# yhao-wang/DenseRetrievalToolkits

Hardware: AMD Instinct MI355X
Metric: queries/sec@top-1000, 10Mx768 corpus (BASELINE: passages encoded/sec + queries/sec@top-1000, 10Mx768 corpus, 1/2/4/8 GPU) (higher is better)
Workload: dtype bf16

## Files before the change

denseretrievaltoolkits_amd/_native.py:

```python
from __future__ import annotations

import ctypes
import os
import threading

import torch

from .build_native import LIB_PATH

DRT_OK = 0
DRT_EINVAL = -1
ROW_STATS_LEN = 34

_lock = threading.Lock()
_lib = None

c_i32 = ctypes.c_int32
c_i64 = ctypes.c_int64
c_sz = ctypes.c_size_t
c_vp = ctypes.c_void_p
c_f32 = ctypes.c_float
c_u64 = ctypes.c_uint64

_SIGNATURES = [
    ("drt_version", ctypes.c_char_p, []),
    ("drt_ip_topk_workspace", c_sz, [c_i64, c_i64, c_i32, c_i32]),
    ("drt_ip_topk_bf16", c_i32, [c_vp, c_i64, c_vp, c_i64, c_i32, c_i32, c_i64, c_vp, c_vp, c_vp, c_vp, c_sz, c_vp]),
    ("drt_ip_topk_resolve_workspace", c_sz, [c_i64, c_i64, c_i32]),
    ("drt_ip_topk_resolve", c_i32, [c_vp, c_i64, c_vp, c_i64, c_i32, c_i32, c_i64, c_vp, c_vp, c_vp, c_vp, c_sz,
                                    c_vp, c_vp]),
    ("drt_topk_merge", c_i32, [c_vp, c_vp, c_i64, c_i32, c_i32, c_i32, c_vp, c_vp, c_vp]),
    ("drt_ip_topk_sample_rank", c_i32, [c_i32]),
    ("drt_ip_topk_dist_workspace", c_sz, [c_i64, c_i64, c_i64, c_i32, c_i32]),
    ("drt_ip_topk_dist_sample", c_i32, [c_vp, c_i64, c_vp, c_i64, c_i64, c_i32, c_i32, c_vp, c_vp, c_sz, c_vp]),
    ("drt_ip_topk_dist_tau", c_i32, [c_vp, c_i64, c_i32, c_i32, c_vp, c_vp]),
    ("drt_ip_topk_dist_filter", c_i32, [c_vp, c_i64, c_vp, c_i64, c_i64, c_i32, c_i32, c_i64, c_vp, c_vp, c_vp,
                                        c_sz, c_vp]),
    ("drt_ip_topk_dist_filter_chunks", c_i32, [c_vp, c_i64, c_vp, c_i64, c_i64, c_i32, c_i32, c_i64, c_vp, c_vp,
                                               c_vp, c_i32, c_vp, c_sz, c_vp]),
    ("drt_ip_topk_tighten_rank", c_i32, [c_i64, c_i32, c_i32]),
    ("drt_ip_topk_filter_passes_workspace", c_sz, [c_i64, c_i64, c_i64, c_i32, c_i32]),
    ("drt_ip_topk_filter_passes", c_i32, [c_vp, c_i64, c_vp, c_i64, c_i64, c_i32, c_i32, c_i64, c_vp, c_vp,
                                          c_i32, c_i32, c_vp, c_vp, c_vp, c_sz, c_vp]),
    ("drt_ip_topk_dist_filter_lists", c_i32, [c_vp, c_i64, c_vp, c_i64, c_i64, c_i32, c_i32, c_i64, c_vp, c_i32,
                                              c_vp, c_vp, c_vp, c_sz, c_vp]),
    ("drt_ip_topk_dist_filter_lists_at", c_i32, [c_vp, c_i64, c_vp, c_i64, c_i64, c_i32, c_i32, c_i64, c_vp,
                                                 c_i32, c_i64, c_vp, c_vp, c_vp, c_sz, c_vp]),
    ("drt_topk_merge_packed", c_i32, [c_vp, c_i64, c_i32, c_i32, c_i64, c_vp, c_vp, c_vp, c_vp]),
    ("drt_topk_merge_packed_cert", c_i32, [c_vp, c_i64, c_i32, c_i32, c_i32, c_i64, c_vp, c_vp, c_vp, c_vp]),
    ("drt_topk_merge_packed_capped", c_i32, [c_vp, c_i64, c_i32, c_i32, c_i32, c_i32, c_i64, c_vp, c_vp, c_vp,
                                             c_vp]),
    ("drt_row_stats_bf16", c_i32, [c_vp, c_i64, c_i32, c_vp, c_i32, c_vp]),
    ("drt_refine_width", c_i32, [c_i32]),
    ("drt_ip_topk_exact_bf16", c_i32, [c_vp, c_i64, c_vp, c_i64, c_i32, c_i32, c_i64, c_vp, c_vp, c_vp, c_vp, c_vp,
                                       c_sz, c_vp]),
    ("drt_hit_metrics_i8", c_i32, [c_vp, c_i64, c_i64, c_vp, c_i32, c_vp, c_vp]),
    ("drt_answer_match_i32", c_i32, [c_vp, c_i32, c_vp, c_vp, c_i64, c_i64, c_i64, c_vp, c_vp, c_i32, c_i32, c_vp,
                                     c_vp, c_vp]),
    ("drt_ip_topk_resolve_exact", c_i32, [c_vp, c_i64, c_vp, c_i64, c_i32, c_i32, c_i64, c_vp, c_vp, c_vp, c_vp,
                                          c_vp, c_sz, c_vp, c_vp]),
    ("drt_ip_topk_resolve_wide_workspace", c_sz, [c_i64, c_i32]),
    ("drt_ip_topk_resolve_wide", c_i32, [c_vp, c_i64, c_vp, c_i64, c_i32, c_i32, c_i64, c_vp, c_vp, c_vp, c_vp,
                                         c_vp, c_sz, c_vp, c_vp]),
    ("drt_ip_topk_large_workspace", c_sz, [c_i32, c_i32]),
    ("drt_ip_topk_large", c_i32, [c_vp, c_i64, c_vp, c_i64, c_i32, c_i32, c_i64, c_vp, c_vp, c_vp, c_vp, c_vp, c_vp,
                                  c_sz, c_vp]),
    ("drt_ip_topk_large_keys", c_i32, [c_vp, c_i64, c_vp, c_i64, c_i32, c_i32, c_i64, c_vp, c_vp, c_vp, c_vp, c_vp,
                                       c_vp, c_vp, c_sz, c_vp]),
    ("drt_merge_exact", c_i32, [c_vp, c_vp, c_i64, c_i32, c_i32, c_vp, c_vp, c_vp]),
    ("drt_refine_delta_bf16", c_i32, [c_vp, c_i64, c_i32, c_vp, c_i64, c_i64, c_vp, c_vp, c_i32, c_i32, c_vp, c_vp,
                                      c_vp, c_vp, c_vp, c_vp]),
    ("drt_refine_delta_local_bf16", c_i32, [c_vp, c_i64, c_i32, c_vp, c_i64, c_i64, c_vp, c_vp, c_i32, c_i32, c_vp,
                                            c_vp, c_vp, c_vp, c_vp, c_vp]),
    ("drt_refine_sort", c_i32, [c_vp, c_vp, c_vp, c_vp, c_i64, c_i32, c_i32, c_vp, c_vp, c_vp]),
    ("drt_topk_exclude", c_i32, [c_vp, c_vp, c_i64, c_i32, c_vp, c_vp, c_vp, c_i32, c_i32, c_vp, c_vp, c_vp, c_vp]),
    ("drt_pair_scores_bf16", c_i32, [c_vp, c_i64, c_vp, c_i64, c_i32, c_vp, c_vp, c_i64, c_vp, c_vp]),
    ("drt_topk_collapse_workspace", c_sz, [c_i64, c_i32]),
    ("drt_topk_collapse", c_i32, [c_vp, c_vp, c_i64, c_i32, c_vp, c_i64, c_i32, c_vp, c_vp, c_vp, c_vp, c_vp, c_sz,
                                  c_vp]),
    ("drt_gemm_nt_bf16_f32", c_i32, [c_vp, c_vp, c_vp, c_i64, c_i64, c_i32, c_i64, c_vp]),
    ("drt_embed_ln", c_i32, [c_vp, c_vp, c_i64, c_i64, c_vp, c_vp, c_vp, c_vp, c_vp, c_f32, c_i32, c_vp, c_vp]),
    ("drt_linear_bf16", c_i32, [c_vp, c_vp, c_vp, c_vp, c_vp, c_i64, c_i64, c_i64, c_i32, c_vp]),
    ("drt_linear_workspace", c_sz, [c_i64, c_i64, c_i64]),
    ("drt_linear_bf16_ws", c_i32, [c_vp, c_vp, c_vp, c_vp, c_vp, c_i64, c_i64, c_i64, c_i32, c_vp, c_sz, c_vp]),
    ("drt_linear_ln_bf16_ws", c_i32, [c_vp, c_vp, c_vp, c_vp, c_vp, c_vp, c_f32, c_vp, c_vp, c_i64, c_i64, c_i64,
                                      c_vp, c_sz, c_vp]),
    ("drt_layernorm_f32_bf16", c_i32, [c_vp, c_i64, c_i32, c_vp, c_vp, c_f32, c_vp, c_vp]),
    ("drt_attention_fwd_lse_bf16", c_i32, [c_vp, c_vp, c_vp, c_vp, c_i64, c_i64, c_i32, c_i32, c_f32, c_vp]),
    ("drt_layernorm_bwd_workspace", c_sz, [c_i64, c_i32]),
    ("drt_layernorm_bwd_sum_bf16", c_i32, [c_vp, c_vp, c_vp, c_f32, c_i64, c_i32, c_vp, c_vp, c_vp, c_f32, c_u64,
                                           c_u64, c_vp, c_vp, c_vp, c_vp, c_sz, c_vp]),
    ("drt_linear_bf16_ex", c_i32, [c_vp, c_vp, c_vp, c_vp, c_vp, c_vp, c_vp, c_i64, c_i64, c_i64, c_i32, c_f32, c_u64,
                                   c_u64, c_vp, c_sz, c_vp]),
    ("drt_layernorm_bwd_bf16", c_i32, [c_vp, c_vp, c_vp, c_f32, c_i64, c_i32, c_vp, c_vp, c_vp, c_vp, c_vp, c_sz,
                                       c_vp]),
    ("drt_colsum_workspace", c_sz, [c_i64, c_i64]),
    ("drt_colsum_bf16", c_i32, [c_vp, c_i64, c_i64, c_vp, c_vp, c_sz, c_vp]),
    ("drt_colsum_f32", c_i32, [c_vp, c_i64, c_i64, c_vp, c_vp, c_sz, c_vp]),
    ("drt_linear_dgelu_bias_workspace", c_sz, [c_i64, c_i64, c_i64]),
    ("drt_linear_dgelu_bias_bf16", c_i32, [c_vp, c_vp, c_vp, c_vp, c_i64, c_i64, c_i64, c_vp, c_vp, c_sz, c_vp]),
    ("drt_gelu_bwd_bf16", c_i32, [c_vp, c_vp, c_i64, c_vp, c_vp]),
    ("drt_linear_wgrad_workspace", c_sz, [c_i64, c_i64, c_i64]),
    ("drt_linear_wgrad_bf16", c_i32, [c_vp, c_vp, c_vp, c_i64, c_i64, c_i64, c_vp, c_sz, c_vp]),
    ("drt_transpose_bf16", c_i32, [c_vp, c_i64, c_i64, c_vp, c_vp]),
    ("drt_transpose_bf16_ld", c_i32, [c_vp, c_i64, c_i64, c_vp, c_i64, c_vp]),
    ("drt_embed_ln_pre", c_i32, [c_vp, c_vp, c_i64, c_i64, c_vp, c_vp, c_vp, c_vp, c_vp, c_f32, c_i32, c_vp, c_vp,
                                 c_vp]),
    ("drt_gelu_bf16", c_i32, [c_vp, c_i64, c_vp, c_vp]),
    ("drt_embedding_bwd", c_i32, [c_vp, c_vp, c_i32, c_vp, c_i64, c_i64, c_i32, c_i64, c_vp, c_vp, c_vp, c_vp]),
    ("drt_dropout_add_bf16", c_i32, [c_vp, c_vp, c_i64, c_f32, ctypes.c_uint64, ctypes.c_uint64, c_vp, c_vp]),
    ("drt_attention_train_fwd_bits_bf16", c_i32, [c_vp, c_vp, c_vp, c_vp, c_vp, c_i64, c_i64, c_i32, c_i32, c_f32,
                                                  c_f32, c_u64, c_u64, c_vp]),
    ("drt_attention_train_bwd_bits_bf16", c_i32, [c_vp, c_vp, c_vp, c_vp, c_vp, c_vp, c_vp, c_i64, c_i64, c_i32,
                                                  c_i32, c_f32, c_f32, c_u64, c_u64, c_vp]),
    ("drt_attention_train_bwd_bias_workspace", c_sz, [c_i64, c_i32, c_i32]),
    ("drt_attention_train_bwd_bias_bf16", c_i32, [c_vp, c_vp, c_vp, c_vp, c_vp, c_vp, c_vp, c_i64, c_i64, c_i32,
                                                  c_i32, c_f32, c_f32, c_u64, c_u64, c_vp, c_vp, c_sz, c_vp]),
    ("drt_attention_bwd_bf16", c_i32, [c_vp, c_vp, c_vp, c_vp, c_vp, c_vp, c_i64, c_i64, c_i32, c_i32, c_f32, c_vp]),
    ("drt_layernorm_bf16", c_i32, [c_vp, c_i64, c_i32, c_vp, c_vp, c_f32, c_vp, c_vp]),
    ("drt_attention_bf16", c_i32, [c_vp, c_vp, c_vp, c_i64, c_i64, c_i32, c_i32, c_f32, c_vp]),
    ("drt_pool_bf16", c_i32, [c_vp, c_vp, c_i64, c_i64, c_i32, c_i32, c_vp, c_vp, c_vp]),
    ("drt_l2_normalize_f32", c_i32, [c_vp, c_i64, c_i32, c_vp, c_vp]),
    ("drt_t5_embed_bf16", c_i32, [c_vp, c_i64, c_i64, c_vp, c_i32, c_vp, c_vp]),
    ("drt_rmsnorm_bf16", c_i32, [c_vp, c_i64, c_i32, c_vp, c_f32, c_vp, c_vp]),
    ("drt_attention_relbias_bf16", c_i32, [c_vp, c_vp, c_vp, c_vp, c_i64, c_i64, c_i32, c_i32, c_f32, c_vp]),
    ("drt_gated_gelu_new_bf16", c_i32, [c_vp, c_i64, c_i64, c_vp, c_vp]),
    ("drt_attention_relbias_train_fwd_bits_bf16", c_i32, [c_vp, c_vp, c_vp, c_vp, c_vp, c_vp, c_i64, c_i64, c_i32,
                                                          c_i32, c_f32, c_f32, c_u64, c_u64, c_vp]),
    ("drt_attention_relbias_train_bwd_workspace", c_sz, [c_i64, c_i64, c_i32]),
    ("drt_attention_relbias_train_bwd_bf16", c_i32, [c_vp, c_vp, c_vp, c_vp, c_vp, c_vp, c_vp, c_vp, c_i64, c_i64,
                                                     c_i32, c_i32, c_f32, c_f32, c_u64, c_u64, c_vp, c_vp, c_sz,
                                                     c_vp]),
    ("drt_rmsnorm_bwd_workspace", c_sz, [c_i64, c_i32]),
    ("drt_rmsnorm_bwd_bf16", c_i32, [c_vp, c_vp, c_vp, c_f32, c_i64, c_i32, c_vp, c_vp, c_vp, c_vp, c_sz, c_vp]),
    ("drt_gated_gelu_new_bwd_bf16", c_i32, [c_vp, c_vp, c_i64, c_i64, c_f32, c_u64, c_u64, c_vp, c_vp]),
    ("drt_relu_bwd_bf16", c_i32, [c_vp, c_vp, c_i64, c_f32, c_u64, c_u64, c_vp, c_vp]),
    ("drt_t5_embedding_bwd", c_i32, [c_vp, c_vp, c_i64, c_i64, c_i32, c_i64, c_vp, c_vp]),
    ("drt_t5_head_expand_bf16",c_i32, [c_vp, c_vp, c_vp, c_i64, c_i32, c_i32, c_vp]),
    ("drt_t5_cross_pool_bf16", c_i32, [c_vp, c_vp, c_vp, c_vp, c_i64, c_i64, c_i32, c_i32, c_vp]),
    ("drt_t5_head_reduce_bf16", c_i32, [c_vp, c_vp, c_vp, c_i64, c_i32, c_i32, c_vp]),
    ("drt_gemm_nt_f32", c_i32, [c_vp, c_vp, c_vp, c_i64, c_i64, c_i64, c_i64, c_i64, c_i64, c_vp]),
    ("drt_gemm_f32", c_i32, [c_vp, c_vp, c_vp, c_i64, c_i64, c_i64, c_i64, c_i64, c_i64, c_i32, c_i32, c_i32, c_vp, c_vp]),
    ("drt_ce_fwd", c_i32, [c_vp, c_i64, c_i64, c_i64, c_f32, c_vp, c_vp, c_vp, c_vp]),
    ("drt_ce_bwd", c_i32, [c_vp, c_vp, c_i64, c_i64, c_i64, c_vp, c_f32, c_vp, c_vp]),
    ("drt_score_ce_workspace", c_sz, [c_i64, c_i64, c_i32]),
    ("drt_score_ce_fwd", c_i32, [c_vp, c_vp, c_i64, c_i64, c_i32, c_i64, c_f32, c_vp, c_vp, c_vp, c_vp, c_sz, c_vp]),
    ("drt_score_ce_bwd", c_i32, [c_vp, c_vp, c_vp, c_vp, c_i64, c_i64, c_i32, c_i64, c_vp, c_f32, c_vp, c_vp, c_vp,
                                 c_sz, c_vp]),
    ("drt_kd_fwd", c_i32, [c_vp, c_vp, c_i64, c_i64, c_i64, c_f32, c_f32, c_f32, c_f32, c_vp, c_vp, c_vp, c_vp, c_vp]),
    ("drt_kd_bwd", c_i32, [c_vp, c_vp, c_vp, c_vp, c_i64, c_i64, c_i64, c_f32, c_f32, c_f32, c_vp, c_f32, c_vp, c_vp]),
    ("drt_score_kd_workspace", c_sz, [c_i64, c_i64, c_i32]),
    ("drt_score_kd_fwd", c_i32, [c_vp, c_vp, c_vp, c_i64, c_i64, c_i32, c_i64, c_f32, c_f32, c_f32, c_f32, c_vp, c_vp,
                                 c_vp, c_vp, c_vp, c_sz, c_vp]),
    ("drt_score_kd_bwd", c_i32, [c_vp, c_vp, c_vp, c_vp, c_vp, c_vp, c_i64, c_i64, c_i32, c_i64, c_f32, c_f32, c_f32,
                                 c_vp, c_f32, c_vp, c_vp, c_vp, c_sz, c_vp]),
    ("drt_transpose_f32", c_i32, [c_vp, c_i64, c_i64, c_vp, c_vp]),
    ("drt_profile_enable", c_i32, [c_i32, c_i32]),
    ("drt_profile_read", c_i32, [c_i32, c_vp, c_vp]),
    ("drt_profile_read_each", c_i32, [c_i32, c_vp, c_i64, c_vp]),
]

PROF_SCAN, PROF_SAMPLE, PROF_SELECT, PROF_MERGE, PROF_GEMM = range(5)

EXPORTED = [n for n, _, _ in _SIGNATURES]


def lib_path() -> str:
    return os.environ.get("DRT_LIB", LIB_PATH)


def load():
    global _lib
    if _lib is not None:
        return _lib
    with _lock:
        if _lib is not None:
            return _lib
        path = lib_path()
        if not os.path.exists(path):
            raise RuntimeError(
                f"DRT native library not found at {path}; build it with "
                "`python -m denseretrievaltoolkits_amd.build_native` (no CPU fallback exists)")
        lib = ctypes.CDLL(path, mode=ctypes.RTLD_LOCAL)
        for name, res, args in _SIGNATURES:
            fn = getattr(lib, name)
            fn.restype = res
            fn.argtypes = args
        _lib = lib
    return _lib


def check(rc: int, what: str) -> None:
    if rc != DRT_OK:
        if rc == DRT_EINVAL:
            raise ValueError(f"{what}: invalid argument (DRT_EINVAL)")
        raise RuntimeError(f"{what}: HIP error {rc}")
# ... 5 lines not shown
```

denseretrievaltoolkits_amd/csrc/search.hip:

```cpp
#include <cmath>
#include <type_traits>

#include "profile.h"
#include "search_internal.h"

namespace drt {

constexpr int kHitCap = 1024;
constexpr int kTopRL = 4;

__host__ __device__ __forceinline__ int pass_tiles(int ntiles, int npass, int pass) {
  return npass <= 1 ? ntiles : (pass < ntiles ? (ntiles - 1 - pass) / npass + 1 : 0);
}

__device__ __forceinline__ void glds16(const void* gsrc, uint32_t lds_addr) {
  uint32_t keep;
  asm volatile(
      "s_mov_b32 %0, m0\n\t"
      "s_mov_b32 m0, %2\n\t"
      "s_nop 0\n\t"
      "global_load_lds_dwordx4 %1, off\n\t"
      "s_mov_b32 m0, %0"
      : "=&s"(keep)
      : "v"(gsrc), "s"(lds_addr)
// ... 1180 lines not shown
  rc = launch_scan(filter_scan_args(Q, nq, P, d, n, tau, cnt, w + p.off_keys, p.cap), d, SCAN_FILTER, s, PROF_SCAN);
  if (rc) return rc;

  sa.in = w + p.off_keys;
  sa.in_stride = p.cap;
  sa.counts = cnt;
  sa.cap = p.cap;
  sa.n_total = n;
  rc = launch_select(sa, SEL_KEYS64, SEL_TOPK, s);
  if (rc || !refine) return rc;
  ra.tau = tau;
  return launch_refine(ra, s);
}

int drt_ip_topk_bf16(const void* Q, int64_t nq, const void* P, int64_t n, int32_t d, int32_t k,
                     int64_t id_offset, float* out_scores, int64_t* out_ids, int32_t* status,
                     void* ws, size_t ws_bytes, void* stream) {
  return ip_topk_impl(Q, nq, P, n, d, k, id_offset, out_scores, out_ids, status, ws, ws_bytes, nullptr,
                      (hipStream_t)stream);
}

int drt_ip_topk_exact_bf16(const void* Q, int64_t nq, const void* P, int64_t n, int32_t d, int32_t k,
                           int64_t id_offset, const float* stats, float* out_scores, int64_t* out_ids,
                           int32_t* status, void* ws, size_t ws_bytes, void* stream) {
  DRT_REQUIRE(stats != nullptr);
  return ip_topk_impl(Q, nq, P, n, d, k, id_offset, out_scores, out_ids, status, ws, ws_bytes, stats,
                      (hipStream_t)stream);
}

static int64_t resolve_chunk(int64_t nbad, int64_t n) {
  const int64_t width = resolve_width(n);
  int64_t chunk = std::max<int64_t>(1, std::min<int64_t>(nbad, (2ll << 30) / (width * 4)));
  return std::min<int64_t>(chunk, kQueriesPerWG);
}

size_t drt_ip_topk_resolve_workspace(int64_t nbad, int64_t n, int32_t d) {
  if (nbad <= 0 || n < 0 || d <= 0 || d % 64 || d > 1024) return 0;
  return resolve_layout(resolve_chunk(nbad, n), n, d).total;
}

static int resolve_impl(const void* Q, int64_t nq, const void* P, int64_t n, int32_t d, int32_t k, int64_t id_offset,
                        float* out_scores, int64_t* out_ids, int32_t* status, void* ws, size_t ws_bytes,
                        int64_t* n_resolved, const float* stats, hipStream_t s) {
  DRT_REQUIRE(valid_dims(nq, n, d, k));
  if (n_resolved) *n_resolved = 0;
  if (nq == 0 || status == nullptr) return DRT_OK;
  std::vector<int32_t> bad;
  int rc = flagged_queries(status, nq, 1, 1, s, bad);
  if (rc || bad.empty()) return rc;
  if (n_resolved) *n_resolved = (int64_t)bad.size();

  const int64_t width = resolve_width(n);
  int64_t chunk = resolve_chunk((int64_t)bad.size(), n);
  while (chunk > 1 && resolve_layout(chunk, n, d).total > ws_bytes) chunk >>= 1;
  const bool refine = stats != nullptr && n > 0;
  const int64_t kc = refine_width(k);
  const ResolveLayout l = resolve_layout(chunk, n, d, kc);
  DRT_REQUIRE(ws != nullptr && l.total <= ws_bytes);
  char* wp = (char*)ws;
  void* qbuf = wp + l.qbuf;
  void* sbuf = wp + l.scores;
  void* mbuf = wp + l.qmap;
  float* rcs = (float*)(wp + l.cand_s);
  int64_t* rci = (int64_t*)(wp + l.cand_i);
  float* rdl = (float*)(wp + l.delta);
  int32_t* rcn = (int32_t*)(wp + l.cnt);
  for (size_t b0 = 0; b0 < bad.size(); b0 += chunk) {
    const int64_t nb = std::min<int64_t>(chunk, (int64_t)bad.size() - (int64_t)b0);
    if ((rc = gather_queries(Q, d, bad.data() + b0, nb, qbuf, mbuf, s))) return rc;
    ScanArgs a = scan_args(qbuf, nb, P, d);
    a.nrows = n;
    a.out = sbuf;
    a.cap = width;
    if ((rc = launch_scan(a, d, SCAN_DENSE, s, -1))) return rc;
    SelectArgs sa{};
    sa.in = sbuf;
    sa.in_stride = width;
    sa.n_in = n;
    sa.n_total = n;
    sa.k = k;
    sa.nq = nb;
    sa.out_scores = out_scores;
    sa.out_ids = out_ids;
    sa.ldo = k;
    sa.id_offset = id_offset;
    sa.status = status;
    sa.qmap = (const int32_t*)mbuf;
    if (refine) {
      sa.k = (int)kc;
      sa.k_cert = k;
      sa.out_scores = rcs;
      sa.out_ids = rci;
      sa.ldo = kc;
      sa.status = nullptr;
      sa.qmap = nullptr;
    }
    if ((rc = launch_select(sa, SEL_DENSE32, SEL_TOPK, s))) return rc;
    if (refine) {
      RefineArgs ra{};
      ra.Q = (const __bf16*)qbuf;
      ra.nq = nb;
      ra.d = d;
      ra.P = (const __bf16*)P;
      ra.n_local = n;
      ra.row_offset = id_offset;
      ra.cs = rcs;
      ra.ci = rci;
      ra.kc = (int32_t)kc;
      ra.k = k;
      ra.stats = stats;
      ra.tau = nullptr;
      ra.delta = rdl;
      ra.cnt = rcn;
      ra.status = status;
      ra.qmap = (const int32_t*)mbuf;
      ra.set_status = true;
      ra.out_s = out_scores;
      ra.out_i = out_ids;
      if ((rc = launch_refine(ra, s))) return rc;
    }
    DRT_CHECK_HIP(hipStreamSynchronize(s));
  }
  return DRT_OK;
}

int drt_ip_topk_resolve(const void* Q, int64_t nq, const void* P, int64_t n, int32_t d, int32_t k,
                        int64_t id_offset, float* out_scores, int64_t* out_ids, int32_t* status,
                        void* ws, size_t ws_bytes, int64_t* n_resolved, void* stream) {
  return resolve_impl(Q, nq, P, n, d, k, id_offset, out_scores, out_ids, status, ws, ws_bytes, n_resolved, nullptr,
                      (hipStream_t)stream);
}

int drt_ip_topk_resolve_exact(const void* Q, int64_t nq, const void* P, int64_t n, int32_t d, int32_t k,
                              int64_t id_offset, const float* stats, float* out_scores, int64_t* out_ids,
                              int32_t* status, void* ws, size_t ws_bytes, int64_t* n_resolved, void* stream) {
  DRT_REQUIRE(stats != nullptr);
  return resolve_impl(Q, nq, P, n, d, k, id_offset, out_scores, out_ids, status, ws, ws_bytes, n_resolved, stats,
                      (hipStream_t)stream);
}

int32_t drt_ip_topk_sample_rank(int32_t k) {
  if (k < 1 || k > kSelMaxK) return -1;
  const TopkPlan p = make_plan(1, (int64_t)0xFFFFFFFEll, k);
  return (int32_t)p.r;
}

size_t drt_ip_topk_dist_workspace(int64_t nq, int64_t n_local, int64_t n_global, int32_t d, int32_t k) {
  if (!valid_dist_dims(nq, n_local, n_global, d, k)) return 0;
  return make_dist_plan(nq, n_local, n_global, k).total;
}

int drt_ip_topk_dist_sample(const void* Q, int64_t nq, const void* P, int64_t n_local, int64_t n_global, int32_t d,
                            int32_t k, uint32_t* best, void* ws, size_t ws_bytes, void* stream) {
  DRT_REQUIRE(valid_dist_dims(nq, n_local, n_global, d, k));
  if (nq == 0) return DRT_OK;
  DRT_REQUIRE(Q && best && ws);
  const TopkPlan p = make_dist_plan(nq, n_local, n_global, k);
  DRT_REQUIRE(ws_bytes >= p.total);
  const int64_t r = drt_ip_topk_sample_rank(k);
  hipStream_t s = (hipStream_t)stream;
  if (!p.sample || n_local == 0) {
    DRT_CHECK_HIP(hipMemsetAsync(best, 0xFF, (size_t)nq * r * 4, s));
    return DRT_OK;
  }
  DRT_REQUIRE(P != nullptr);
  char* w = (char*)ws;
  ScanArgs a = scan_args(Q, nq, P, d);
  a.row0 = p.stride / 2;
  a.nrows = p.m;
  a.rstride = p.stride;
  a.out = w + p.off_sample;
  const int64_t nlists = 4 * (int64_t)scan16_grid(nq, p.m).x;
  if (nlists * kTopRL <= kKthChunk && nlists * kTopRL <= align_up(p.m, 4)) {
    a.cap = nlists * kTopRL;
    DRT_CHECK_HIP(hipMemsetAsync(a.out, 0xFF, (size_t)nq * a.cap * 4, s));
    int rc = launch_scan(a, d, SCAN_TOPR, s, PROF_SAMPLE);
    if (rc) return rc;
    const ProfPair pp = prof_begin(PROF_SELECT, s);
    launch_kth_final(nq, (const uint32_t*)a.out, (int)nlists, (int)r, (int64_t)kTopRL, (int64_t)a.cap, nullptr, best,
                     nullptr, kTopRL, s);
    prof_end(pp, s);
    return hip_status(hipGetLastError());
  }
  a.cap = align_up(p.m, 4);
  int rc = launch_scan(a, d, SCAN_DENSE, s, PROF_SAMPLE);
  if (rc) return rc;
  const ProfPair pp = prof_begin(PROF_SELECT, s);
  launch_kth_partial(p.nchunk, nq, (const uint32_t*)(w + p.off_sample), (int64_t)align_up(p.m, 4), p.m, (int)r,
                     (uint32_t*)(w + p.off_part), s);
  launch_kth_final(nq, (const uint32_t*)(w + p.off_part), (int)p.nchunk, (int)r, (int64_t)r, (int64_t)(p.nchunk * r),
                   nullptr, best, nullptr, (int)r, s);
  prof_end(pp, s);
  return hip_status(hipGetLastError());
}

int drt_ip_topk_dist_tau(const uint32_t* lists, int64_t nq, int32_t nlists, int32_t k, float* tau, void* stream) {
  const int32_t r = drt_ip_topk_sample_rank(k);
  DRT_REQUIRE(r > 0 && nq >= 0 && nlists >= 1 && (int64_t)nlists * r <= kKthChunk);
  if (nq == 0) return DRT_OK;
  DRT_REQUIRE(lists && tau);
  launch_kth_final(nq, lists, (int)nlists, (int)r, (int64_t)nq * r, (int64_t)r, tau, nullptr, nullptr, (int)r,
                   (hipStream_t)stream);
  return hip_status(hipGetLastError());
}

struct FilterRun {
  TopkPlan p;
  hipStream_t s;
  char* w;
  uint32_t* cnt;
  SelectArgs sel;
  ScanArgs scan;
};

static int filter_setup(FilterRun& f, const void* Q, int64_t nq, const void* P, int64_t n_local, int64_t n_global,
                        int32_t d, int32_t k, int64_t id_offset, const void* thr, uint64_t* packed, void* ws,
                        size_t ws_bytes, void* stream) {
  DRT_REQUIRE(valid_dist_dims(nq, n_local, n_global, d, k));
  DRT_REQUIRE(id_offset >= 0 && id_offset + n_local <= n_global);
  if (nq == 0) return DRT_OK;
  DRT_REQUIRE(Q && thr && packed && ws);
  f.p = make_dist_plan(nq, n_local, n_global, k);
  DRT_REQUIRE(ws_bytes >= f.p.total);
  f.s = (hipStream_t)stream;
  f.w = (char*)ws;
  f.cnt = (uint32_t*)(f.w + f.p.off_cnt);
  f.sel = SelectArgs{};
  f.sel.in = f.w + f.p.off_keys;
  f.sel.in_stride = f.p.cap;
  f.sel.k = k;
  f.sel.nq = nq;
  f.sel.id_offset = id_offset;
  f.sel.out_packed = packed;
  f.sel.global_tau = true;
  f.scan = filter_scan_args(Q, nq, P, d, n_local, nullptr, f.cnt, f.w + f.p.off_keys, f.p.cap);
  return DRT_OK;
}

static int filter_begin(const FilterRun& f, bool zero_counts) {
  DRT_REQUIRE(f.scan.P != nullptr);
  if (zero_counts) DRT_CHECK_HIP(hipMemsetAsync(f.cnt, 0, f.p.nq_pad * 4 * kCntStride, f.s));
  return DRT_OK;
}

static int filter_select(FilterRun& f) {
  if (f.p.n == 0) return launch_select(f.sel, SEL_DENSE32, SEL_TOPK, f.s);
  f.sel.counts = f.cnt;
  f.sel.cap = f.p.cap;
  f.sel.n_total = f.p.n;
  return launch_select(f.sel, SEL_KEYS64, SEL_TOPK, f.s);
}

int drt_ip_topk_dist_filter(const void* Q, int64_t nq, const void* P, int64_t n_local, int64_t n_global, int32_t d,
                            int32_t k, int64_t id_offset, const float* tau, uint64_t* packed, void* ws,
                            size_t ws_bytes, void* stream) {
  FilterRun f;
  int rc = filter_setup(f, Q, nq, P, n_local, n_global, d, k, id_offset, tau, packed, ws, ws_bytes, stream);
  if (rc || nq == 0) return rc;
  if (n_local > 0) {
    if ((rc = filter_begin(f, true))) return rc;
    ScanArgs a = f.scan;
    a.tau = tau;
    a.exp_hits = rows_exp_hits(f.p, n_local, n_global);
    if ((rc = launch_scan(a, d, SCAN_FILTER, f.s, PROF_SCAN))) return rc;
  }
  return filter_select(f);
}

int drt_ip_topk_dist_filter_chunks(const void* Q, int64_t nq, const void* P, int64_t n_local, int64_t n_global,
                                   int32_t d, int32_t k, int64_t id_offset, const float* tau, uint64_t* packed,
                                   const int64_t* starts, int32_t nchunks, void* ws, size_t ws_bytes, void* stream) {
  DRT_REQUIRE(d <= 768 && n_local < ((int64_t)1 << 32));
  DRT_REQUIRE(starts != nullptr && nchunks >= 1 && starts[0] == 0 && starts[nchunks] == n_local);
  for (int c = 0; c < nchunks; ++c) DRT_REQUIRE(starts[c] <= starts[c + 1]);
  FilterRun f;
  int rc = filter_setup(f, Q, nq, P, n_local, n_global, d, k, id_offset, tau, packed, ws, ws_bytes, stream);
  if (rc || nq == 0) return rc;
  if (n_local > 0) {
    if ((rc = filter_begin(f, true))) return rc;
    for (int c = 0; c < nchunks; ++c) {
      const int64_t r0 = starts[c], rows = starts[c + 1] - starts[c];
      if (rows == 0) continue;
      ScanArgs a = f.scan;
      a.P += r0 * d;
      a.nrows = rows;
      a.row_base = (uint32_t)r0;
      a.tau = tau;
      a.exp_hits = rows_exp_hits(f.p, rows, n_global);
      if ((rc = launch_scan(a, d, SCAN_FILTER, f.s, PROF_SCAN))) return rc;
    }
  }
  return filter_select(f);
}

int32_t drt_ip_topk_tighten_rank(int64_t n_local, int32_t npasses, int32_t k) {
  if (n_local <= 0 || npasses <= 1 || k < 1) return 0;
  const int64_t tall = (n_local + kT16 - 1) / kT16;
  const int64_t t0 = (tall + npasses - 1) / npasses;
  if (t0 >= tall) return 0;
  const double C = (double)tall / (double)t0;
  for (int64_t r = 1; r < ((int64_t)1 << 24); ++r) {
    const double sigma = std::sqrt(C * (C - 1.0) * (double)r + (C - 1.0) * (double)r);
    if (C * (double)r - 5.0 * sigma >= (double)k) return (int32_t)r;
  }
  return 0;
}

size_t drt_ip_topk_filter_passes_workspace(int64_t nq, int64_t n_local, int64_t n_global, int32_t d, int32_t k) {
  if (!valid_dist_dims(nq, n_local, n_global, d, k)) return 0;
  const TopkPlan p = make_dist_plan(nq, n_local, n_global, k);
  return passes_layout(p.total, p.nq_pad).total;
}

int drt_ip_topk_filter_passes(const void* Q, int64_t nq, const void* P, int64_t n_local, int64_t n_global,
                              int32_t d, int32_t k, int64_t id_offset, const float* tau, uint64_t* packed,
                              int32_t npasses, int32_t r, float* tau1_out, uint32_t* pass0_out, void* ws,
                              size_t ws_bytes, void* stream) {
  DRT_REQUIRE(d <= 768 && n_local < ((int64_t)1 << 32) && npasses >= 1 && npasses <= 1024);
  FilterRun f;
  int rc = filter_setup(f, Q, nq, P, n_local, n_global, d, k, id_offset, tau, packed, ws, ws_bytes, stream);
  if (rc || nq == 0) return rc;
  const PassesLayout pl = passes_layout(f.p.total, f.p.nq_pad);
  DRT_REQUIRE(ws_bytes >= pl.total);
  if (r < 0) r = drt_ip_topk_tighten_rank(n_local, npasses, k);
  const int tall = (int)((n_local + kT16 - 1) / kT16);
  const bool tighten = r > 0 && n_local > 0 && pass_tiles(tall, npasses, 0) < tall;
  if (!tighten) {
    if (tau1_out) DRT_CHECK_HIP(hipMemcpyAsync(tau1_out, tau, (size_t)nq * 4, hipMemcpyDeviceToDevice, f.s));
    if (pass0_out) DRT_CHECK_HIP(hipMemsetAsync(pass0_out, 0, (size_t)nq * 16, f.s));
  }
  float* tau1 = tau1_out ? tau1_out : (float*)(f.w + f.p.off_tau);
  uint32_t* pass0 = pass0_out ? pass0_out : (uint32_t*)(f.w + pl.off_pass0);
  if (n_local > 0) {
    if ((rc = filter_begin(f, true))) return rc;
    for (int ps = 0; ps < npasses; ++ps) {
      if (pass_tiles(tall, npasses, ps) == 0) continue;
      ScanArgs a = f.scan;
      a.npass = npasses;
      a.pass = ps;
      a.tau = (tighten && ps > 0) ? tau1 : tau;
      a.exp_hits = pass_exp_hits(f.p, npasses, n_global);
      if ((rc = launch_scan(a, d, SCAN_FILTER, f.s, PROF_SCAN))) return rc;
      if (tighten && ps == 0) {
        const ProfPair pp = prof_begin(PROF_SELECT, f.s);
        launch_tighten(nq, (const uint64_t*)f.scan.out, f.p.cap, f.cnt, tau, (int)r, tau1, pass0, f.s);
        prof_end(pp, f.s);
        DRT_CHECK_HIP(hipGetLastError());
      }
    }
  }
  f.sel.pass0 = tighten ? pass0 : nullptr;
  return filter_select(f);
}

int drt_ip_topk_dist_filter_lists(const void* Q, int64_t nq, const void* P, int64_t n_local, int64_t n_global,
                                  int32_t d, int32_t k, int64_t id_offset, const uint32_t* lists, int32_t nlists,
                                  float* tau_out, uint64_t* packed, void* ws, size_t ws_bytes, void* stream) {
  const int32_t r = drt_ip_topk_sample_rank(k);
  return drt_ip_topk_dist_filter_lists_at(Q, nq, P, n_local, n_global, d, k, id_offset, lists, nlists,
                                          r > 0 ? nq * r : 0, tau_out, packed, ws, ws_bytes, stream);
}

int drt_ip_topk_dist_filter_lists_at(const void* Q, int64_t nq, const void* P, int64_t n_local, int64_t n_global,
                                     int32_t d, int32_t k, int64_t id_offset, const uint32_t* lists, int32_t nlists,
                                     int64_t lists_stride, float* tau_out, uint64_t* packed, void* ws,
                                     size_t ws_bytes, void* stream) {
  const int32_t r = drt_ip_topk_sample_rank(k);
  DRT_REQUIRE(r > 0 && nlists >= 1 && (int64_t)nlists * r <= kKthChunk);
  DRT_REQUIRE(nlists == 1 || lists_stride >= nq * r);
  FilterRun f;
  int rc = filter_setup(f, Q, nq, P, n_local, n_global, d, k, id_offset, lists, packed, ws, ws_bytes, stream);
  if (rc || nq == 0) return rc;
  float* tau = tau_out ? tau_out : (float*)(f.w + f.p.off_tau);
  launch_kth_final(nq, lists, (int)nlists, (int)r, lists_stride, (int64_t)r, tau, nullptr,
                   n_local > 0 ? f.cnt : nullptr, (int)r, f.s);
  DRT_CHECK_HIP(hipGetLastError());
  if (n_local > 0) {
    if ((rc = filter_begin(f, false))) return rc;
    ScanArgs a = f.scan;
    a.tau = tau;
    a.exp_hits = rows_exp_hits(f.p, n_local, n_global);
    if ((rc = launch_scan(a, d, SCAN_FILTER, f.s, PROF_SCAN))) return rc;
  }
  return filter_select(f);
}

}
```

denseretrievaltoolkits_amd/csrc/search_internal.h:

```cpp
#pragma once

#include <algorithm>
#include <vector>

#include "drt_common.h"

#define DRT_INTERNAL __attribute__((visibility("hidden")))

namespace drt {

constexpr int kQueriesPerWG = 128;
constexpr int kCntStride = 32;
constexpr int kSelMaxK = 2048;
constexpr int kKthChunk = 4096;
constexpr int64_t kWideCap = 65536;

enum { SEL_KEYS64 = 0, SEL_DENSE32 = 1 };
enum { SEL_TOPK = 0, SEL_KTH = 1 };

struct SelectArgs {
  const void* in;
  int64_t in_stride;
  const uint32_t* counts;
  int64_t n_in;
  int64_t cap;
  int64_t n_total;
  int k;
  int64_t nq;
  float* out_scores;
  int64_t* out_ids;
  int64_t ldo;
  int64_t id_offset;
  int32_t* status;
  const int32_t* qmap;
  float* tau;
  uint64_t* out_packed;
  bool global_tau;
  int k_cert;
  const uint32_t* pass0;
};

DRT_INTERNAL int launch_select(const SelectArgs& a, int input, int output, hipStream_t s);
DRT_INTERNAL bool kth_rank_fits(int64_t m, int64_t r);
DRT_INTERNAL void launch_kth_rank(int64_t nq, const uint32_t* in, int64_t stride, int64_t n, int r, float* tau,
                                  uint32_t* zero, hipStream_t s);
DRT_INTERNAL void launch_kth_partial(int64_t nchunk, int64_t nq, const uint32_t* in, int64_t stride, int64_t n, int r,
                                     uint32_t* part, hipStream_t s);
DRT_INTERNAL void launch_kth_final(int64_t nq, const uint32_t* part, int nlists, int r, int64_t lstride,
                                   int64_t qstride, float* tau, uint32_t* best, uint32_t* zero, int len,
                                   hipStream_t s);
DRT_INTERNAL void launch_tighten(int64_t nq, const uint64_t* keys, int64_t cap, const uint32_t* counts,
                                 const float* tau0, int r, float* tau1, uint32_t* pass0, hipStream_t s);

enum { SCAN_FILTER = 0, SCAN_DENSE = 1, SCAN_TOPR = 2 };

struct ScanArgs {
  const __bf16* Q;
  int64_t nq;
  int64_t ldq;
  const __bf16* P;
  int64_t ldp;
  int64_t row0;
  int64_t nrows;
  int64_t rstride;
  const float* tau;
  uint32_t* counts;
  void* out;
  int64_t cap;
  int64_t exp_hits;
  uint32_t row_base;
  int32_t npass;
  int32_t pass;
};

static inline ScanArgs scan_args(const void* Q, int64_t nq, const void* P, int32_t d) {
  ScanArgs a{};
  a.Q = (const __bf16*)Q;
  a.nq = nq;
  a.ldq = d;
  a.P = (const __bf16*)P;
  a.ldp = d;
  a.row0 = 0;
  a.rstride = 1;
  return a;
}

static inline ScanArgs filter_scan_args(const void* Q, int64_t nq, const void* P, int32_t d, int64_t n,
                                        const float* tau, uint32_t* counts, void* out, int64_t cap) {
  ScanArgs a = scan_args(Q, nq, P, d);
  a.nrows = n;
  a.tau = tau;
  a.counts = counts;
  a.out = out;
  a.cap = cap;
  return a;
}

DRT_INTERNAL int launch_scan(const ScanArgs& a, int d, int mode, hipStream_t s, int family);

struct RefineArgs {
  const __bf16* Q;
  int64_t nq;
  int32_t d;
  const __bf16* P;
  int64_t n_local;
  int64_t row_offset;
  const float* cs;
  const int64_t* ci;
  int32_t kc, k;
  const float* stats;
  const float* tau;
  float* delta;
  int32_t* cnt;
  int32_t* status;
  const int32_t* qmap;
  bool set_status;
  int32_t slice;
  float* out_s;
  int64_t* out_i;
};

DRT_INTERNAL int launch_refine(RefineArgs& ra, hipStream_t s);
DRT_INTERNAL int flagged_queries(const int32_t* status, int64_t nq, int32_t mask, int32_t want, hipStream_t s,
                                 std::vector<int32_t>& out);
DRT_INTERNAL int gather_queries(const void* Q, int32_t d, const int32_t* idx, int64_t nb, void* qbuf, void* qmap,
                                hipStream_t s);

static inline size_t align_up(size_t x, size_t a) { return (x + a - 1) / a * a; }

static inline int64_t hit_target(int64_t k) { return std::max<int64_t>(4096, 4 * k); }

static inline int64_t refine_width(int64_t k) {
  return std::min<int64_t>(kSelMaxK, k + std::max<int64_t>(256, k / 4));
}

static inline bool valid_dims(int64_t nq, int64_t n, int32_t d, int32_t k) {
  return nq >= 0 && n >= 0 && d > 0 && d % 64 == 0 && d <= 1024 && k >= 1 && k <= kSelMaxK &&
         n < (int64_t)0xFFFFFFFFll;
}


struct WsBump {
  size_t o = 0;
  size_t take(size_t bytes) {
    const size_t at = o;
    o = align_up(o + bytes, 256);
    return at;
  }
};

struct PlanHead {
  size_t off_tau, off_cnt, off_keys, off_sample, off_part, head_end;
};
static inline PlanHead plan_head_layout(int64_t nq_pad, int64_t cap, int key_bytes, int64_t m, int64_t part_keys) {
  WsBump b;
  PlanHead h;
  h.off_tau = b.take((size_t)nq_pad * 4);
  h.off_cnt = b.take((size_t)nq_pad * 4 * kCntStride);
  h.off_keys = b.take((size_t)nq_pad * cap * key_bytes);
  h.off_sample = b.take((size_t)nq_pad * align_up(m, 4) * 4);
  h.off_part = b.take((size_t)nq_pad * part_keys * 4);
  h.head_end = b.o;
  return h;
}

struct PassesLayout {
  size_t off_pass0, total;
};
static inline PassesLayout passes_layout(size_t plan_total, int64_t nq_pad) {
  WsBump b;
  b.take(plan_total);
  PassesLayout l;
  l.off_pass0 = b.take((size_t)nq_pad * 16);
  l.total = b.o;
  return l;
}

static inline int64_t resolve_width(int64_t n) { return align_up(std::max<int64_t>(n, 4), 4); }

struct ResolveLayout {
  size_t qbuf, scores, qmap, cand_s, cand_i, delta, cnt, total;
};
static inline ResolveLayout resolve_layout(int64_t chunk, int64_t n, int32_t d, int64_t kc = kSelMaxK) {
  WsBump b;
  ResolveLayout l;
  l.qbuf = b.take((size_t)chunk * d * 2);
  l.scores = b.take((size_t)chunk * resolve_width(n) * 4);
  l.qmap = b.take((size_t)chunk * 4);
  l.cand_s = b.take((size_t)chunk * kSelMaxK * 16 + chunk * 8);
  l.cand_i = l.cand_s + (size_t)chunk * kc * 4;
  l.delta = l.cand_s + (size_t)chunk * kc * 12;
  l.cnt = l.cand_s + (size_t)chunk * kc * 16;
// ... 41 lines not shown
```

denseretrievaltoolkits_amd/csrc/select.hip:

```cpp
#include "profile.h"
#include "search_internal.h"

namespace drt {

constexpr int kSelThreads = 512;
constexpr int kSelWaves = kSelThreads / 64;
constexpr int kSelBins = 1024;
constexpr int kSelBuf = 4096;
constexpr int kSelKPT = 16;
constexpr int kSelRegCap = kSelKPT * kSelThreads;

template <int INPUT>
__device__ __forceinline__ uint64_t sel_load(const SelectArgs& a, int64_t q, int64_t j) {
  if (INPUT == SEL_KEYS64) return ((const uint64_t*)a.in)[q * a.in_stride + j];
  const uint32_t v = ((const uint32_t*)a.in)[q * a.in_stride + j];
  return ((uint64_t)v << 32) | (uint64_t)(uint32_t)j;
}

__device__ __forceinline__ float key_score(uint64_t x) { return desc_key_to_score((uint32_t)(x >> 32)); }

__device__ __forceinline__ int score_bin(float s, float smin, float scale) {
  if (scale == 0.0f) return 0;
  return hist_bin((s - smin) * scale, kSelBins, __builtin_signbit(s) ? 0 : kSelBins - 1);
}

template <typename T, typename Op>
__device__ __forceinline__ T block_reduce(T v, T* scratch, Op op) {
#pragma unroll
  for (int o = 32; o > 0; o >>= 1) v = op(v, __shfl_xor(v, o, 64));
  const int w = threadIdx.x >> 6;
  __syncthreads();
  if ((threadIdx.x & 63) == 0) scratch[w] = v;
  __syncthreads();
  T r = scratch[0];
#pragma unroll
  for (int i = 1; i < kSelWaves; ++i) r = op(r, scratch[i]);
  return r;
}

template <typename T, int NT, int E, int US>
__device__ __forceinline__ void sort_inthread(T (&v)[E], int size, int tid) {
#pragma unroll
  for (int u = 0; u < E; ++u) {
    if ((u & US) == 0 && (u | US) < E) {
      const int i = u * NT + tid;
      const bool up = (i & size) == 0;
      const T a = v[u], b = v[u | US];
      v[u] = up ? (a < b ? a : b) : (a < b ? b : a);
      v[u | US] = up ? (a < b ? b : a) : (a < b ? a : b);
    }
  }
}

template <typename T, int NT, int N>
__device__ __forceinline__ void block_sort_fixed(T* buf, int n) {
  constexpr int E = N / NT;
  const int tid = threadIdx.x;
  const T kMax = ~(T)0;
  T v[E];
#pragma unroll
  for (int u = 0; u < E; ++u) {
    const int i = u * NT + tid;
    v[u] = i < n ? buf[i] : kMax;
  }
  __syncthreads();
#pragma unroll
  for (int size = 2; size <= N; size <<= 1) {
#pragma unroll
    for (int stride = size >> 1; stride > 0; stride >>= 1) {
      if (stride >= NT) {
        if (E >= 2 && stride == NT) sort_inthread<T, NT, E, 1>(v, size, tid);
        else if (E >= 4 && stride == 2 * NT) sort_inthread<T, NT, E, 2>(v, size, tid);
        else if (E >= 8) sort_inthread<T, NT, E, 4>(v, size, tid);
      } else {
        T p[E];
        if (stride >= 64) {
#pragma unroll
          for (int u = 0; u < E; ++u) buf[u * NT + tid] = v[u];
          __syncthreads();
#pragma unroll
          for (int u = 0; u < E; ++u) p[u] = buf[(u * NT + tid) ^ stride];
          __syncthreads();
        } else {
#pragma unroll
          for (int u = 0; u < E; ++u) p[u] = __shfl_xor(v[u], stride, 64);
        }
#pragma unroll
        for (int u = 0; u < E; ++u) {
          const int i = u * NT + tid;
          const bool keep_min = ((i & stride) == 0) == ((i & size) == 0);
          const T a = v[u], b = p[u];
          v[u] = keep_min ? (a < b ? a : b) : (a < b ? b : a);
        }
      }
    }
  }
#pragma unroll
  for (int u = 0; u < E; ++u) {
    const int i = u * NT + tid;
    if (i < n) buf[i] = v[u];
  }
  __syncthreads();
}

template <typename T, int NT>
__device__ __forceinline__ void block_sort(T* buf, int n) {
  if (n <= 1) {
    __syncthreads();
    return;
  }
  if (n <= NT) block_sort_fixed<T, NT, NT>(buf, n);
  else if (n <= 2 * NT) block_sort_fixed<T, NT, 2 * NT>(buf, n);
  else if (n <= 4 * NT) block_sort_fixed<T, NT, 4 * NT>(buf, n);
  else block_sort_fixed<T, NT, 8 * NT>(buf, n);
}

__device__ __forceinline__ void block_bitonic(uint64_t* buf, int n2) { block_sort<uint64_t, kSelThreads>(buf, n2); }

template <int INPUT, int OUTPUT>
__global__ __launch_bounds__(kSelThreads) void select_kernel(SelectArgs a) {
  __shared__ uint32_t hist[kSelWaves][kSelBins];
  __shared__ uint32_t suffix[kSelBins];
  __shared__ float fscr[kSelWaves];
  __shared__ uint64_t uscr[kSelWaves];
  __shared__ uint64_t sh_prefix, sh_mask;
  __shared__ int64_t sh_kk;
  __shared__ int sh_done, sh_bin;
  __shared__ uint32_t sh_nsel, sh_nside;
  __shared__ __attribute__((aligned(16))) uint64_t buf[kSelBuf];

  const int tid = threadIdx.x;
  const int wave = tid >> 6;
  const int64_t q = blockIdx.x;
  int64_t c_raw, c;
  if (INPUT == SEL_KEYS64) {
    c_raw = a.counts[q * kCntStride];
    c = c_raw < a.cap ? c_raw : a.cap;
  } else {
    c_raw = a.n_in;
    c = a.n_in;
  }
  const int64_t kk_total = (int64_t)a.k < c ? (int64_t)a.k : c;

  if (OUTPUT == SEL_KTH && (c < (int64_t)a.k || c == 0)) {
    if (tid == 0) a.tau[q] = -__builtin_inff();
    return;
  }

  bool fast_done = false;
  int nsel = 0;
  if (c > (int64_t)a.k && c <= kSelRegCap) {
    uint64_t kr[kSelKPT];
    float sc[kSelKPT];
#pragma unroll
    for (int u = 0; u < kSelKPT; ++u) {
      const int64_t j = (int64_t)u * kSelThreads + tid;
      const uint64_t x = sel_load<INPUT>(a, q, j < c ? j : 0);
      kr[u] = j < c ? x : ~0ull;
    }
    float lo = __builtin_inff(), hi = -__builtin_inff();
#pragma unroll
    for (int u = 0; u < kSelKPT; ++u) {
      sc[u] = key_score(kr[u]);
      if ((int64_t)u * kSelThreads + tid < c) {
        lo = fminf(lo, sc[u]);
        hi = fmaxf(hi, sc[u]);
      }
    }
    lo = block_reduce(lo, fscr, [](float x, float y) { return fminf(x, y); });
    hi = block_reduce(hi, fscr, [](float x, float y) { return fmaxf(x, y); });
    const float range = hi - lo;
    const float scale = hist_scale((float)kSelBins, range);
    for (int i = tid; i < kSelWaves * kSelBins; i += kSelThreads) (&hist[0][0])[i] = 0;
    __syncthreads();
    int bn[kSelKPT];
#pragma unroll
    for (int u = 0; u < kSelKPT; ++u) {
      bn[u] = -1;
      if ((int64_t)u * kSelThreads + tid < c) {
        bn[u] = score_bin(sc[u], lo, scale);
        atomicAdd(&hist[wave][bn[u]], 1u);
      }
    }
    __syncthreads();
    for (int i = tid; i < kSelBins; i += kSelThreads) {
      uint32_t t = 0;
#pragma unroll
      for (int w = 0; w < kSelWaves; ++w) t += hist[w][i];
      suffix[i] = t;
    }
    __syncthreads();
    for (int off = 1; off < kSelBins; off <<= 1) {
      uint32_t v[kSelBins / kSelThreads];
#pragma unroll
      for (int u = 0; u < kSelBins / kSelThreads; ++u) {
        const int i = tid + u * kSelThreads;
        v[u] = suffix[i] + (i + off < kSelBins ? suffix[i + off] : 0u);
      }
      __syncthreads();
#pragma unroll
      for (int u = 0; u < kSelBins / kSelThreads; ++u) suffix[tid + u * kSelThreads] = v[u];
      __syncthreads();
    }
    if (tid == 0) sh_bin = 0;
    __syncthreads();
    for (int i = tid; i < kSelBins; i += kSelThreads) {
      const bool ok = (int64_t)suffix[i] >= kk_total;
      const bool next_ok = (i + 1 < kSelBins) && (int64_t)suffix[i + 1] >= kk_total;
      if (ok && !next_ok) sh_bin = i;
    }
    __syncthreads();
    const int b = sh_bin;
    if (OUTPUT == SEL_KTH) {
      float t = __builtin_inff();
#pragma unroll
      for (int u = 0; u < kSelKPT; ++u)
        if (bn[u] >= b) t = fminf(t, sc[u]);
      t = block_reduce(t, fscr, [](float x, float y) { return fminf(x, y); });
      if (tid == 0) a.tau[q] = t;
      return;
    }
    const uint32_t cnt_sel = suffix[b];
    const uint32_t c_above = (b + 1 < kSelBins) ? suffix[b + 1] : 0u;
    const uint32_t cnt_b = cnt_sel - c_above;
    if (cnt_b <= (uint32_t)(kSelBuf / 2) && kk_total <= kSelBuf / 2) {
      uint64_t* side = buf + kSelBuf / 2;
      if (tid == 0) {
        sh_nsel = 0;
        sh_nside = 0;
      }
      __syncthreads();
#pragma unroll
      for (int u = 0; u < kSelKPT; ++u) {
        if (bn[u] > b) buf[atomicAdd(&sh_nsel, 1u)] = kr[u];
        else if (bn[u] == b) side[atomicAdd(&sh_nside, 1u)] = kr[u];
      }
      __syncthreads();
      const int ns = (int)sh_nside;
      int m2 = 1;
      while (m2 < ns) m2 <<= 1;
      for (int i = ns + tid; i < m2; i += kSelThreads) side[i] = ~0ull;
      __syncthreads();
      block_bitonic(side, m2);
      const int need = (int)kk_total - (int)c_above;
      for (int i = tid; i < need; i += kSelThreads) buf[c_above + i] = side[i];
      __syncthreads();
      nsel = (int)kk_total;
      fast_done = true;
    } else if (cnt_sel <= (uint32_t)kSelBuf) {
      if (tid == 0) sh_nsel = 0;
      __syncthreads();
#pragma unroll
      for (int u = 0; u < kSelKPT; ++u)
        if (bn[u] >= b) buf[atomicAdd(&sh_nsel, 1u)] = kr[u];
      __syncthreads();
      nsel = (int)sh_nsel;
      fast_done = true;
    }
  } else if (c > (int64_t)a.k) {
    float lo = __builtin_inff(), hi = -__builtin_inff();
    for (int64_t j = tid; j < c; j += kSelThreads) {
      const float s = key_score(sel_load<INPUT>(a, q, j));
      lo = fminf(lo, s);
      hi = fmaxf(hi, s);
    }
    lo = block_reduce(lo, fscr, [](float x, float y) { return fminf(x, y); });
    hi = block_reduce(hi, fscr, [](float x, float y) { return fmaxf(x, y); });
    const float range = hi - lo;
    const float scale = hist_scale((float)kSelBins, range);
    for (int i = tid; i < kSelWaves * kSelBins; i += kSelThreads) (&hist[0][0])[i] = 0;
    __syncthreads();
    for (int64_t j = tid; j < c; j += kSelThreads) {
      const float s = key_score(sel_load<INPUT>(a, q, j));
      atomicAdd(&hist[wave][score_bin(s, lo, scale)], 1u);
    }
    __syncthreads();
    for (int i = tid; i < kSelBins; i += kSelThreads) {
      uint32_t t = 0;
#pragma unroll
      for (int w = 0; w < kSelWaves; ++w) t += hist[w][i];
      suffix[i] = t;
    }
    __syncthreads();
    for (int off = 1; off < kSelBins; off <<= 1) {
      uint32_t v[kSelBins / kSelThreads];
#pragma unroll
      for (int u = 0; u < kSelBins / kSelThreads; ++u) {
        const int i = tid + u * kSelThreads;
        v[u] = suffix[i] + (i + off < kSelBins ? suffix[i + off] : 0u);
      }
      __syncthreads();
#pragma unroll
      for (int u = 0; u < kSelBins / kSelThreads; ++u) suffix[tid + u * kSelThreads] = v[u];
      __syncthreads();
    }
    if (tid == 0) sh_bin = 0;
    __syncthreads();
    for (int i = tid; i < kSelBins; i += kSelThreads) {
      const bool ok = (int64_t)suffix[i] >= kk_total;
      const bool next_ok = (i + 1 < kSelBins) && (int64_t)suffix[i + 1] >= kk_total;
      if (ok && !next_ok) sh_bin = i;
    }
    __syncthreads();
    const int b = sh_bin;
    const uint32_t cnt_sel = suffix[b];
    if (OUTPUT == SEL_KTH) {
      float t = __builtin_inff();
      for (int64_t j = tid; j < c; j += kSelThreads) {
        const float s = key_score(sel_load<INPUT>(a, q, j));
        if (score_bin(s, lo, scale) >= b) t = fminf(t, s);
      }
      t = block_reduce(t, fscr, [](float x, float y) { return fminf(x, y); });
      if (tid == 0) a.tau[q] = t;
      return;
    }
    const uint32_t c_above = (b + 1 < kSelBins) ? suffix[b + 1] : 0u;
    const uint32_t cnt_b = cnt_sel - c_above;
    if (cnt_b <= (uint32_t)(kSelBuf / 2) && kk_total <= kSelBuf / 2) {
      uint64_t* side = buf + kSelBuf / 2;
      if (tid == 0) {
        sh_nsel = 0;
        sh_nside = 0;
      }
      __syncthreads();
      for (int64_t j = tid; j < c; j += kSelThreads) {
        const uint64_t x = sel_load<INPUT>(a, q, j);
        const int bx = score_bin(key_score(x), lo, scale);
        if (bx > b) buf[atomicAdd(&sh_nsel, 1u)] = x;
        else if (bx == b) side[atomicAdd(&sh_nside, 1u)] = x;
      }
      __syncthreads();
      const int ns = (int)sh_nside;
      int m2 = 1;
      while (m2 < ns) m2 <<= 1;
      for (int i = ns + tid; i < m2; i += kSelThreads) side[i] = ~0ull;
      __syncthreads();
      block_bitonic(side, m2);
      const int need = (int)kk_total - (int)c_above;
      for (int i = tid; i < need; i += kSelThreads) buf[c_above + i] = side[i];
      __syncthreads();
      nsel = (int)kk_total;
      fast_done = true;
    } else if (cnt_sel <= (uint32_t)kSelBuf) {
      if (tid == 0) sh_nsel = 0;
      __syncthreads();
      for (int64_t j = tid; j < c; j += kSelThreads) {
        const uint64_t x = sel_load<INPUT>(a, q, j);
        if (score_bin(key_score(x), lo, scale) >= b) {
          const uint32_t p = atomicAdd(&sh_nsel, 1u);
          if (p < (uint32_t)kSelBuf) buf[p] = x;
        }
      }
      __syncthreads();
      nsel = (int)sh_nsel;
      fast_done = true;
    }
  }

  if (!fast_done) {
    if (tid == 0) {
      sh_prefix = 0;
      sh_mask = 0;
      sh_kk = kk_total;
      sh_done = (c <= (int64_t)a.k) ? 1 : 0;
      if (c <= (int64_t)a.k) {
        sh_prefix = ~0ull;
        sh_mask = ~0ull;
      }
    }
    __syncthreads();
    uint32_t* h0 = &hist[0][0];
    for (int shift = 56; shift >= 0 && !sh_done; shift -= 8) {
      for (int i = tid; i < 256; i += kSelThreads) h0[i] = 0;
      __syncthreads();
      const uint64_t prefix = sh_prefix, mask = sh_mask;
      for (int64_t j = tid; j < c; j += kSelThreads) {
        const uint64_t x = sel_load<INPUT>(a, q, j);
        if ((x & mask) == prefix) atomicAdd(&h0[(x >> shift) & 255], 1u);
      }
      __syncthreads();
      if (tid < 64) {
        const uint32_t b0 = h0[4 * tid], b1 = h0[4 * tid + 1], b2 = h0[4 * tid + 2], b3 = h0[4 * tid + 3];
        const uint32_t s4 = b0 + b1 + b2 + b3;
        uint32_t incl = s4;
#pragma unroll
        for (int o = 1; o < 64; o <<= 1) {
          const uint32_t v = __shfl_up(incl, o, 64);
          if (tid >= o) incl += v;
        }
        const uint32_t excl = incl - s4;
        const int64_t kk = sh_kk;
        if ((int64_t)excl < kk && kk <= (int64_t)incl) {
          uint32_t run = excl;
          const uint32_t bb[4] = {b0, b1, b2, b3};
          int d = 0;
          uint32_t cnt = 0;
#pragma unroll
          for (int t = 0; t < 4; ++t) {
            if ((int64_t)(run + bb[t]) >= kk) {
              d = 4 * tid + t;
              cnt = bb[t];
              break;
            }
            run += bb[t];
          }
          const int64_t rem = kk - run;
          sh_prefix = prefix | ((uint64_t)d << shift);
          sh_mask = mask | (255ull << shift);
          sh_kk = rem;
          if ((int64_t)cnt == rem) sh_done = 1;
        }
      }
      __syncthreads();
    }
    const uint64_t thr = sh_prefix | ~sh_mask;
    if (tid == 0) sh_nsel = 0;
    __syncthreads();
    for (int64_t j = tid; j < c; j += kSelThreads) {
      const uint64_t x = sel_load<INPUT>(a, q, j);
      if (x <= thr) {
        const uint32_t p = atomicAdd(&sh_nsel, 1u);
        if (p < (uint32_t)kSelBuf) buf[p] = x;
      }
    }
    __syncthreads();
    nsel = (int)sh_nsel;
  }

  nsel = nsel < kSelBuf ? nsel : kSelBuf;
  int n2 = 1;
  while (n2 < nsel) n2 <<= 1;
  for (int i = nsel + tid; i < n2; i += kSelThreads) buf[i] = ~0ull;
  __syncthreads();
  block_bitonic(buf, n2);

  const int64_t orow = a.qmap ? (int64_t)a.qmap[q] : q;
  if (a.out_packed) {
    uint64_t* op = a.out_packed + orow * (int64_t)(a.k + 1);
    for (int j = tid; j < a.k; j += kSelThreads) {
      if (j < kk_total) {
        const uint64_t x = buf[j];
        op[j] = (x & 0xFFFFFFFF00000000ull) | (uint64_t)(uint32_t)(a.id_offset + (int64_t)(x & 0xFFFFFFFFull));
      } else {
        op[j] = ~0ull;
      }
    }
    if (tid == 0) {
      const uint64_t nval = (uint64_t)(kk_total < a.k ? kk_total : a.k);
      bool bad = INPUT == SEL_KEYS64 && c_raw > a.cap;
      if (INPUT == SEL_KEYS64 && a.pass0) {
        const uint32_t* t = a.pass0 + q * 4;
        if (t[2] && (int64_t)t[1] + (c_raw - (int64_t)t[0]) < (int64_t)a.k) bad = true;
      }
      op[a.k] = (nval << 32) | (bad ? 1ull : 0ull) | (c_raw > (int64_t)a.k ? 2ull : 0ull);
    }
    return;
  }
  float* os = a.out_scores + orow * a.ldo;
  int64_t* oi = a.out_ids + orow * a.ldo;
  for (int j = tid; j < a.k; j += kSelThreads) {
    if (j < kk_total) {
      const uint64_t x = buf[j];
      os[j] = key_score(x);
      oi[j] = a.id_offset + (int64_t)(x & 0xFFFFFFFFull);
    } else {
      os[j] = kPadScore;
      oi[j] = -1;
    }
  }
  if (a.status && tid == 0) {
    int st = 0;
    if (INPUT == SEL_KEYS64) {
      if (c_raw > a.cap) st = 1;
      const int64_t kq = a.k_cert > 0 ? a.k_cert : a.k;
      if (!a.global_tau && c_raw < kq && c_raw < a.n_total) st = 1;
    }
    a.status[orow] = st;
  }
}

constexpr int kTightThreads = 256;

__global__ __launch_bounds__(kTightThreads) void tighten_kernel(const uint64_t* keys, int64_t cap,
                                                                const uint32_t* counts, const float* tau0, int r,
                                                                float* tau1, uint32_t* pass0) {
  __shared__ uint32_t hist[256];
  __shared__ uint32_t sh_prefix, sh_rem;
  __shared__ uint32_t red[kTightThreads / 64];
  const int tid = threadIdx.x;
  const int64_t q = blockIdx.x;
  const uint32_t c = counts[q * kCntStride];
  const float t0 = tau0[q];
  if (!((int64_t)c <= cap && c >= (uint32_t)r && t0 == t0)) {
    if (tid == 0) {
      tau1[q] = t0;
      pass0[q * 4 + 0] = c;
      pass0[q * 4 + 1] = c;
      pass0[q * 4 + 2] = 0;
      pass0[q * 4 + 3] = 0;
    }
    return;
  }
  const uint64_t* kq = keys + q * cap;
  uint32_t prefix = 0, mask = 0, rem = (uint32_t)r;
  for (int shift = 24; shift >= 0; shift -= 8) {
    hist[tid] = 0;
    __syncthreads();
    for (uint32_t j = tid; j < c; j += kTightThreads) {
      const uint32_t key = (uint32_t)(kq[j] >> 32);
      if ((key & mask) == prefix) atomicAdd(&hist[(key >> shift) & 255], 1u);
    }
    __syncthreads();
    if (tid < 64) {
      const uint32_t bb[4] = {hist[4 * tid], hist[4 * tid + 1], hist[4 * tid + 2], hist[4 * tid + 3]};
      const uint32_t s4 = bb[0] + bb[1] + bb[2] + bb[3];
      uint32_t incl = s4;
#pragma unroll
      for (int o = 1; o < 64; o <<= 1) {
        const uint32_t v = __shfl_up(incl, o, 64);
        if (tid >= o) incl += v;
      }
      uint32_t run = incl - s4;
      if (run < rem && rem <= incl) {
        int dgt = 4 * tid;
#pragma unroll
        for (int t = 0; t < 3; ++t) {
          if (dgt == 4 * tid + t && run + bb[t] < rem) {
            run += bb[t];
            ++dgt;
          }
        }
        sh_prefix = prefix | ((uint32_t)dgt << shift);
        sh_rem = rem - run;
      }
    }
    __syncthreads();
    prefix = sh_prefix;
    rem = sh_rem;
    mask |= 255u << shift;
  }
  const float t1 = desc_key_to_score(prefix);
  uint32_t n = 0;
  for (uint32_t j = tid; j < c; j += kTightThreads) n += key_score(kq[j]) >= t1 ? 1u : 0u;
#pragma unroll
  for (int o = 32; o > 0; o >>= 1) n += __shfl_xor(n, o, 64);
  if ((tid & 63) == 0) red[tid >> 6] = n;
  __syncthreads();
  if (tid == 0) {
    uint32_t tot = 0;
    for (int w = 0; w < kTightThreads / 64; ++w) tot += red[w];
    tau1[q] = t1;
    pass0[q * 4 + 0] = c;
    pass0[q * 4 + 1] = tot;
    pass0[q * 4 + 2] = t1 > t0 ? 1u : 0u;
    pass0[q * 4 + 3] = 0;
  }
}

constexpr int kKthThreads = 512;

__device__ __forceinline__ void block_bitonic_u32(uint32_t* buf, int n2) { block_sort<uint32_t, kKthThreads>(buf, n2); }

constexpr int kKthPer = kKthChunk / kKthThreads;
constexpr int kKthBins = 256;
constexpr int kKthSel = 1024;

__global__ __launch_bounds__(kKthThreads) void kth_partial_kernel(const uint32_t* in, int64_t stride, int64_t n,
                                                                  int r, uint32_t* part) {
  __shared__ __attribute__((aligned(16))) uint32_t buf[kKthChunk];
  __shared__ uint32_t hist[kKthThreads / 64][kKthBins];
  __shared__ float red[2][kKthThreads / 64];
  __shared__ uint32_t sh_n;
  __shared__ int sh_bin;
  const int tid = threadIdx.x, wave = tid >> 6, lane = tid & 63;
  const int64_t q = blockIdx.y;
  const int nchunk = gridDim.x;
  const int64_t j0 = (int64_t)blockIdx.x * kKthChunk;
  const int cnt = (int)(n - j0 < kKthChunk ? n - j0 : kKthChunk);
  const uint32_t* src = in + q * stride + j0;

  uint32_t key[kKthPer];
#pragma unroll
  for (int v = 0; v < 2; ++v) {
    const int base = v * (kKthChunk / 2) + 4 * tid;
    if (base + 3 < cnt) {
      const u32x4 x = *(const u32x4*)(src + base);
#pragma unroll
      for (int u = 0; u < 4; ++u) key[4 * v + u] = x[u];
    } else {
#pragma unroll
      for (int u = 0; u < 4; ++u) key[4 * v + u] = base + u < cnt ? src[base + u] : 0xFFFFFFFFu;
    }
  }
  float hi = -__builtin_inff(), lo = __builtin_inff();
#pragma unroll
  for (int e = 0; e < kKthPer; ++e) {
    if (key[e] != 0xFFFFFFFFu) {
      const float sc = desc_key_to_score(key[e]);
      hi = fmaxf(hi, sc);
      lo = fminf(lo, sc);
    }
  }
#pragma unroll
  for (int o = 32; o > 0; o >>= 1) {
    hi = fmaxf(hi, __shfl_xor(hi, o, 64));
    lo = fminf(lo, __shfl_xor(lo, o, 64));
  }
  if (lane == 0) {
    red[0][wave] = hi;
    red[1][wave] = lo;
  }
  for (int i = tid; i < (kKthThreads / 64) * kKthBins; i += kKthThreads) (&hist[0][0])[i] = 0;
  __syncthreads();
#pragma unroll
  for (int w = 0; w < kKthThreads / 64; ++w) {
    hi = fmaxf(hi, red[0][w]);
    lo = fminf(lo, red[1][w]);
  }
  const float range = hi - lo;
  const float scale = hist_scale((float)kKthBins, range);
  int bins[kKthPer];
#pragma unroll
  for (int e = 0; e < kKthPer; ++e) {
    int bb = kKthBins;
    if (key[e] != 0xFFFFFFFFu) {
// ... 300 lines not shown
```

denseretrievaltoolkits_amd/csrc/torch_ops.cpp:

```cpp
#include <vector>

#include <torch/library.h>
#include <ATen/ATen.h>
#include <c10/core/DeviceGuard.h>
#include <ATen/hip/impl/HIPStreamMasqueradingAsCUDA.h>

#include "drt.h"

namespace {

using at::Tensor;

void* stream_of(const Tensor& t) {
  return (void*)at::hip::getCurrentHIPStreamMasqueradingAsCUDA(t.device().index()).stream();
}

void check_rc(int rc, const char* what) {
  TORCH_CHECK_VALUE(rc != DRT_EINVAL, what, ": invalid argument (DRT_EINVAL)");
  TORCH_CHECK(rc == DRT_OK, what, ": HIP error ", rc);
}

void need_gpu(const Tensor& t, const char* name) {
  TORCH_CHECK(t.is_cuda(), "drt ops run on the GPU only (", name, " is on ", t.device(),
              "; no CPU fallback exists)");
// ... 144 lines not shown
  TORCH_CHECK_VALUE(wsb > 0, "unsupported ip_topk_large shape d=", d, " k=", k, " (d % 64 == 0, d <= 1024, k <= 32768)");
  const float* sp = stats_ptr(stats, q);
  Tensor scores = at::empty({nq, k}, q.options().dtype(at::kFloat));
  Tensor ids = at::empty({nq, k}, q.options().dtype(at::kLong));
  Tensor status = at::empty({nq}, q.options().dtype(at::kInt));
  Tensor keys = at::empty({want_keys ? nq : 0, k}, q.options().dtype(at::kLong));
  if (nq == 0) return {scores, ids, status, keys};
  Tensor ws = workspace(q, wsb);
  check_rc(drt_ip_topk_large_keys(q.data_ptr(), nq, n ? p.data_ptr() : nullptr, n, (int32_t)d, (int32_t)k, id_offset,
                                  sp, tau.data_ptr<float>(), scores.data_ptr<float>(), ids.data_ptr<int64_t>(),
                                  want_keys ? (uint64_t*)keys.data_ptr<int64_t>() : nullptr,
                                  status.data_ptr<int32_t>(), ws.data_ptr(), wsb, stream_of(q)),
           "drt_ip_topk_large_keys");
  return {scores, ids, status, keys};
}

std::tuple<Tensor, Tensor, Tensor> ip_topk_large(const Tensor& q, const Tensor& p, int64_t k, int64_t id_offset,
                                                 const Tensor& stats, const Tensor& tau) {
  auto r = ip_topk_large_impl(q, p, k, id_offset, stats, tau, false);
  return {std::get<0>(r), std::get<1>(r), std::get<2>(r)};
}

std::tuple<Tensor, Tensor, Tensor, Tensor> ip_topk_large_keys(const Tensor& q, const Tensor& p, int64_t k,
                                                              int64_t id_offset, const Tensor& stats,
                                                              const Tensor& tau) {
  return ip_topk_large_impl(q, p, k, id_offset, stats, tau, true);
}

std::tuple<Tensor, Tensor> merge_exact(const Tensor& keys_, const Tensor& ids_, int64_t k) {
  need(keys_, "keys", at::kLong, 3);
  need(ids_, "ids", at::kLong, 3);
  TORCH_CHECK_VALUE(keys_.sizes() == ids_.sizes() && keys_.device() == ids_.device(),
                    "merge_exact: keys and ids differ in shape or device");
  TORCH_CHECK_VALUE(keys_.size(2) == k, "merge_exact: lists of ", keys_.size(2), " entries, k = ", k);
  const c10::DeviceGuard g(keys_.device());
  const Tensor keys = keys_.contiguous(), ids = ids_.contiguous();
  const int64_t nq = keys.size(1);
  Tensor s = at::empty({nq, k}, keys.options().dtype(at::kFloat));
  Tensor i = at::empty({nq, k}, keys.options().dtype(at::kLong));
  check_rc(drt_merge_exact((const uint64_t*)keys.data_ptr<int64_t>(), ids.data_ptr<int64_t>(), nq,
                           (int32_t)keys.size(0), (int32_t)k, s.data_ptr<float>(), i.data_ptr<int64_t>(),
                           stream_of(keys)),
           "drt_merge_exact");
  return {s, i};
}

Tensor row_stats(const Tensor& p_, const c10::optional<Tensor>& prev) {
  need(p_, "p", at::kBFloat16, 2);
  const c10::DeviceGuard g(p_.device());
  const Tensor p = p_.contiguous();
  Tensor st;
  if (prev.has_value()) {
    stats_ptr(prev, p);
    st = prev->clone();
  } else {
    st = at::empty({DRT_ROW_STATS_LEN}, p.options().dtype(at::kFloat));
  }
  check_rc(drt_row_stats_bf16(p.size(0) ? p.data_ptr() : nullptr, p.size(0), (int32_t)p.size(1),
                              st.data_ptr<float>(), prev.has_value() ? 1 : 0, stream_of(p)),
           "drt_row_stats_bf16");
  return st;
}

std::tuple<Tensor, Tensor> refine_delta(const Tensor& q_, const Tensor& p_, int64_t row_offset, const Tensor& cs_,
                                        const Tensor& ci_, int64_t k, const Tensor& stats,
                                        const c10::optional<Tensor>& tau_, Tensor& status, bool local) {
  need(q_, "q", at::kBFloat16, 2);
  need(p_, "p", at::kBFloat16, 2);
  need(cs_, "cand_scores", at::kFloat, 2);
  need(ci_, "cand_ids", at::kLong, 2);
  need(status, "status", at::kInt, 1);
  const c10::DeviceGuard g(q_.device());
  const Tensor q = q_.contiguous(), p = p_.contiguous(), cs = cs_.contiguous(), ci = ci_.contiguous();
  const int64_t nq = q.size(0), kc = cs.size(1);
  TORCH_CHECK_VALUE(ci.sizes() == cs.sizes() && cs.size(0) == nq, "candidates must be [nq, kc] like q");
  TORCH_CHECK_VALUE(status.is_contiguous() && status.size(0) == nq, "status must be a contiguous [nq] tensor");
  Tensor tau;
  if (tau_.has_value()) {
    need(*tau_, "tau", at::kFloat, 1);
    tau = tau_->contiguous();
    TORCH_CHECK_VALUE(tau.size(0) == nq, "tau must hold one threshold per query");
  }
  Tensor delta = at::empty({nq, kc}, cs.options());
  Tensor cnt = at::empty({nq, 2}, cs.options().dtype(at::kInt));
  check_rc((local ? drt_refine_delta_local_bf16 : drt_refine_delta_bf16)(
               q.data_ptr(), nq, (int32_t)q.size(1), p.size(0) ? p.data_ptr() : nullptr, p.size(0), row_offset,
               cs.data_ptr<float>(), ci.data_ptr<int64_t>(), (int32_t)kc, (int32_t)k, stats_ptr(stats, q),
               tau.defined() ? tau.data_ptr<float>() : nullptr, delta.data_ptr<float>(), cnt.data_ptr<int32_t>(),
               status.data_ptr<int32_t>(), stream_of(q)),
           "drt_refine_delta_bf16");
  return {delta, cnt};
}

std::tuple<Tensor, Tensor> refine_sort(const Tensor& cs_, const Tensor& ci_, const Tensor& delta_, const Tensor& cnt_,
                                       int64_t k) {
  need(cs_, "cand_scores", at::kFloat, 2);
  need(ci_, "cand_ids", at::kLong, 2);
  need(delta_, "delta", at::kFloat, 2);
  need(cnt_, "cnt", at::kInt, 2);
  const c10::DeviceGuard g(cs_.device());
  const Tensor cs = cs_.contiguous(), ci = ci_.contiguous(), delta = delta_.contiguous(), cnt = cnt_.contiguous();
  const int64_t nq = cs.size(0), kc = cs.size(1);
  TORCH_CHECK_VALUE(ci.sizes() == cs.sizes() && delta.sizes() == cs.sizes() && cnt.size(0) == nq,
                    "refine_sort: candidate, delta and cnt shapes disagree");
  Tensor os = at::empty({nq, k}, cs.options());
  Tensor oi = at::empty({nq, k}, ci.options());
  check_rc(drt_refine_sort(cs.data_ptr<float>(), ci.data_ptr<int64_t>(), delta.data_ptr<float>(),
                           cnt.data_ptr<int32_t>(), nq, (int32_t)kc, (int32_t)k, os.data_ptr<float>(),
                           oi.data_ptr<int64_t>(), stream_of(cs)),
           "drt_refine_sort");
  return {os, oi};
}

std::tuple<Tensor, Tensor> topk_merge(const Tensor& scores_, const Tensor& ids_, int64_t k_out) {
  need(scores_, "scores", at::kFloat, 3);
  need(ids_, "ids", at::kLong, 3);
  TORCH_CHECK_VALUE(scores_.sizes() == ids_.sizes(), "topk_merge: scores and ids differ in shape");
  const c10::DeviceGuard g(scores_.device());
  const Tensor s = scores_.contiguous(), i = ids_.contiguous();
  const int64_t nparts = s.size(0), nq = s.size(1), k_in = s.size(2);
  Tensor os = at::empty({nq, k_out}, s.options());
  Tensor oi = at::empty({nq, k_out}, i.options());
  check_rc(drt_topk_merge(s.data_ptr<float>(), i.data_ptr<int64_t>(), nq, (int32_t)nparts, (int32_t)k_in,
                          (int32_t)k_out, os.data_ptr<float>(), oi.data_ptr<int64_t>(), stream_of(s)),
           "drt_topk_merge");
  return {os, oi};
}

Tensor dist_ws(const Tensor& q, int64_t n_local, int64_t n_global, int64_t k, size_t* wsb, bool passes = false) {
  *wsb = (passes ? drt_ip_topk_filter_passes_workspace
                 : drt_ip_topk_dist_workspace)(q.size(0), n_local, n_global, (int32_t)q.size(1), (int32_t)k);
  TORCH_CHECK_VALUE(*wsb > 0 || q.size(0) == 0, "unsupported dist shape nq=", q.size(0), " n_local=", n_local,
              " n_global=", n_global, " d=", q.size(1), " k=", k);
  return workspace(q, *wsb);
}

Tensor dist_sample(const Tensor& q_, const Tensor& p_, int64_t n_global, int64_t k) {
  need(q_, "q", at::kBFloat16, 2);
  need(p_, "p", at::kBFloat16, 2);
  const c10::DeviceGuard g(q_.device());
  const Tensor q = q_.contiguous(), p = p_.contiguous();
  const int32_t r = drt_ip_topk_sample_rank((int32_t)k);
  TORCH_CHECK_VALUE(r > 0, "unsupported k=", k);
  Tensor best = at::empty({q.size(0), r}, q.options().dtype(at::kInt));
  size_t wsb = 0;
  Tensor ws = dist_ws(q, p.size(0), n_global, k, &wsb);
  check_rc(drt_ip_topk_dist_sample(q.data_ptr(), q.size(0), p.size(0) ? p.data_ptr() : nullptr, p.size(0), n_global,
                                   (int32_t)q.size(1), (int32_t)k, (uint32_t*)best.data_ptr<int32_t>(), ws.data_ptr(),
                                   wsb, stream_of(q)),
           "drt_ip_topk_dist_sample");
  return best;
}

Tensor dist_tau(const Tensor& lists_, int64_t k) {
  need(lists_, "lists", at::kInt, 3);
  const c10::DeviceGuard g(lists_.device());
  const Tensor lists = lists_.contiguous();
  Tensor tau = at::empty({lists.size(1)}, lists.options().dtype(at::kFloat));
  check_rc(drt_ip_topk_dist_tau((const uint32_t*)lists.data_ptr<int32_t>(), lists.size(1), (int32_t)lists.size(0),
                                (int32_t)k, tau.data_ptr<float>(), stream_of(lists)),
           "drt_ip_topk_dist_tau");
  return tau;
}

struct FilterPrelude {
  c10::OptionalDeviceGuard guard;
  Tensor q, p, thr, ws;
  size_t wsb = 0;
  int64_t n_global, k;

  FilterPrelude(const Tensor& q_, const Tensor& p_, const Tensor& thr_, bool thr_is_lists, const Tensor& packed,
                int64_t n_global_, int64_t k_, bool passes_ws = false)
      : n_global(n_global_), k(k_) {
    need(q_, "q", at::kBFloat16, 2);
    need(p_, "p", at::kBFloat16, 2);
    if (thr_is_lists) need(thr_, "lists", at::kInt, 3);
    else need(thr_, "tau", at::kFloat, 1);
    need(packed, "packed", at::kLong, 2);
    guard.reset_device(q_.device());
    q = q_.contiguous();
    p = p_.contiguous();
    thr = thr_is_lists ? thr_ : thr_.contiguous();
    TORCH_CHECK_VALUE(thr_is_lists || thr.size(0) == q.size(0), "tau must hold one threshold per query");
    TORCH_CHECK_VALUE(packed.is_contiguous() && packed.size(0) == q.size(0) && packed.size(1) == k + 1,
                      "packed must be a contiguous [nq, k + 1] tensor");
    ws = dist_ws(q, p.size(0), n_global, k, &wsb, passes_ws);
  }
  template <class Fn, class... Mid>
  void call(Fn fn, const char* what, int64_t id_offset, Mid... mid) const {
    check_rc(fn(q.data_ptr(), q.size(0), p.size(0) ? p.data_ptr() : nullptr, p.size(0), n_global, (int32_t)q.size(1),
                (int32_t)k, id_offset, mid..., ws.data_ptr(), wsb, stream_of(q)),
             what);
  }
};

void dist_filter_into(const Tensor& q_, const Tensor& p_, int64_t n_global, int64_t k, int64_t id_offset,
                      const Tensor& tau_, Tensor& packed) {
  const FilterPrelude f(q_, p_, tau_, false, packed, n_global, k);
  f.call(drt_ip_topk_dist_filter, "drt_ip_topk_dist_filter", id_offset, f.thr.data_ptr<float>(),
         (uint64_t*)packed.data_ptr<int64_t>());
}

Tensor dist_filter(const Tensor& q, const Tensor& p, int64_t n_global, int64_t k, int64_t id_offset,
                   const Tensor& tau) {
  need(q, "q", at::kBFloat16, 2);
  Tensor packed = at::empty({q.size(0), k + 1}, q.options().dtype(at::kLong));
  dist_filter_into(q, p, n_global, k, id_offset, tau, packed);
  return packed;
}

void dist_filter_chunks_into(const Tensor& q_, const Tensor& p_, int64_t n_global, int64_t k, int64_t id_offset,
                             const Tensor& tau_, at::IntArrayRef starts, Tensor& packed) {
  const FilterPrelude f(q_, p_, tau_, false, packed, n_global, k);
  TORCH_CHECK_VALUE(starts.size() >= 2 && starts.front() == 0 && starts.back() == f.p.size(0),
                    "starts must run from 0 to the shard's row count");
  for (size_t c = 1; c < starts.size(); ++c) TORCH_CHECK_VALUE(starts[c - 1] <= starts[c], "starts must not decrease");
  TORCH_CHECK_VALUE(f.q.size(1) <= 768, "chunked filtering takes d <= 768");
  const std::vector<int64_t> st(starts.begin(), starts.end());
  f.call(drt_ip_topk_dist_filter_chunks, "drt_ip_topk_dist_filter_chunks", id_offset, f.thr.data_ptr<float>(),
         (uint64_t*)packed.data_ptr<int64_t>(), st.data(), (int32_t)st.size() - 1);
}

void filter_passes_into(const Tensor& q_, const Tensor& p_, int64_t n_global, int64_t k, int64_t id_offset,
                        const Tensor& tau_, int64_t npasses, int64_t r, Tensor& packed,
                        const c10::optional<Tensor>& tau1, const c10::optional<Tensor>& pass0) {
  const FilterPrelude f(q_, p_, tau_, false, packed, n_global, k, true);
  TORCH_CHECK_VALUE(f.q.size(1) <= 768, "interleaved filter passes take d <= 768");
  TORCH_CHECK_VALUE(npasses >= 1 && npasses <= 1024, "npasses must be in [1, 1024]");
  if (tau1.has_value()) {
    need(*tau1, "tau1", at::kFloat, 1);
    TORCH_CHECK_VALUE(tau1->is_contiguous() && tau1->size(0) == f.q.size(0), "tau1 must be a contiguous [nq] tensor");
  }
  if (pass0.has_value()) {
    need(*pass0, "pass0", at::kInt, 2);
    TORCH_CHECK_VALUE(pass0->is_contiguous() && pass0->size(0) == f.q.size(0) && pass0->size(1) == 4,
                      "pass0 must be a contiguous [nq, 4] tensor");
  }
  f.call(drt_ip_topk_filter_passes, "drt_ip_topk_filter_passes", id_offset, f.thr.data_ptr<float>(),
         (uint64_t*)packed.data_ptr<int64_t>(), (int32_t)npasses, (int32_t)r,
         tau1.has_value() ? tau1->data_ptr<float>() : nullptr,
         pass0.has_value() ? (uint32_t*)pass0->data_ptr<int32_t>() : nullptr);
}

void filter_lists_into(const Tensor& q_, const Tensor& p_, int64_t n_global, int64_t k, int64_t id_offset,
                       const Tensor& lists, int64_t q0, Tensor& packed, const char* what) {
  const FilterPrelude f(q_, p_, lists, true, packed, n_global, k);
  TORCH_CHECK_VALUE(lists.is_contiguous(), "lists must be a contiguous [nlists, NQ, r] tensor");
  TORCH_CHECK_VALUE(q0 >= 0 && q0 + f.q.size(0) <= lists.size(1), "query rows [", q0, ", ", q0 + f.q.size(0),
                    ") outside the lists' ", lists.size(1), " rows");
  const int64_t r = lists.size(2);
  TORCH_CHECK_VALUE(r == drt_ip_topk_sample_rank((int32_t)k), "lists hold ", r, " keys per query, k=", k, " needs ",
                    drt_ip_topk_sample_rank((int32_t)k));
  f.call(drt_ip_topk_dist_filter_lists_at, what, id_offset, (const uint32_t*)lists.data_ptr<int32_t>() + q0 * r,
         (int32_t)lists.size(0), lists.size(1) * r, (float*)nullptr, (uint64_t*)packed.data_ptr<int64_t>());
}

void dist_filter_lists_into(const Tensor& q, const Tensor& p, int64_t n_global, int64_t k, int64_t id_offset,
                            const Tensor& lists, int64_t q0, Tensor& packed) {
  filter_lists_into(q, p, n_global, k, id_offset, lists, q0, packed, "drt_ip_topk_dist_filter_lists_at");
}

Tensor dist_filter_lists(const Tensor& q, const Tensor& p, int64_t n_global, int64_t k, int64_t id_offset,
                         const Tensor& lists_) {
  need(q, "q", at::kBFloat16, 2);
  need(p, "p", at::kBFloat16, 2);
  need(lists_, "lists", at::kInt, 3);
  TORCH_CHECK_VALUE(lists_.size(1) == q.size(0), "lists must be [nlists, nq, r]");
  Tensor packed = at::empty({q.size(0), k + 1}, q.options().dtype(at::kLong));
  filter_lists_into(q, p, n_global, k, id_offset, lists_.contiguous(), 0, packed, "drt_ip_topk_dist_filter_lists");
  return packed;
}

std::tuple<Tensor, Tensor, Tensor> merge_packed(const Tensor& parts_, int64_t k, int64_t n_global, int64_t k_cert) {
  need(parts_, "parts", at::kLong, 3);
  TORCH_CHECK_VALUE(parts_.size(2) >= 2 && parts_.size(2) <= k + 1,
                    "merge_packed expects [nparts, nq, lcap + 1] lists with lcap <= k");
  const c10::DeviceGuard g(parts_.device());
  const Tensor parts = parts_.contiguous();
  const int64_t nq = parts.size(1), lcap = parts.size(2) - 1;
  Tensor s = at::empty({nq, k}, parts.options().dtype(at::kFloat));
  Tensor i = at::empty({nq, k}, parts.options().dtype(at::kLong));
  Tensor st = at::empty({nq}, parts.options().dtype(at::kInt));
  if (lcap < k) {
    check_rc(drt_topk_merge_packed_capped((const uint64_t*)parts.data_ptr<int64_t>(), nq, (int32_t)parts.size(0),
                                          (int32_t)lcap, (int32_t)k, (int32_t)(k_cert > 0 ? k_cert : k), n_global,
                                          s.data_ptr<float>(), i.data_ptr<int64_t>(), st.data_ptr<int32_t>(),
                                          stream_of(parts)),
             "drt_topk_merge_packed_capped");
    return {s, i, st};
  }
  check_rc(drt_topk_merge_packed_cert((const uint64_t*)parts.data_ptr<int64_t>(), nq, (int32_t)parts.size(0),
                                      (int32_t)k, (int32_t)(k_cert > 0 ? k_cert : k), n_global, s.data_ptr<float>(),
                                      i.data_ptr<int64_t>(), st.data_ptr<int32_t>(), stream_of(parts)),
           "drt_topk_merge_packed_cert");
  return {s, i, st};
}

std::tuple<Tensor, Tensor, Tensor> topk_exclude(const Tensor& scores_, const Tensor& ids_, const Tensor& excl_,
                                                const Tensor& excl_off_, const c10::optional<Tensor>& ceiling_,
                                                int64_t skip, int64_t k_out) {
  need(scores_, "scores", at::kFloat, 2);
  need(ids_, "ids", at::kLong, 2);
  need(excl_, "excl", at::kLong, 1);
  need(excl_off_, "excl_off", at::kLong, 1);
  TORCH_CHECK_VALUE(scores_.sizes() == ids_.sizes(), "topk_exclude: scores ", scores_.sizes(), " and ids ",
                    ids_.sizes(), " differ in shape");
  TORCH_CHECK_VALUE(ids_.device() == scores_.device() && excl_.device() == scores_.device() &&
                        excl_off_.device() == scores_.device(),
                    "topk_exclude: every tensor must be on the scores' device ", scores_.device());
  const int64_t nq = scores_.size(0), k_in = scores_.size(1);
  TORCH_CHECK_VALUE(excl_off_.numel() == nq + 1, "excl_off: expected ", nq + 1, " offsets (nq + 1), got ",
                    excl_off_.numel());
  TORCH_CHECK_VALUE(k_out >= 1 && skip >= 0 && skip <= 0x7FFFFFFF && k_out <= 0x7FFFFFFF,
                    "topk_exclude: unsupported skip=", skip, " k_out=", k_out, " (skip >= 0, k_out >= 1)");
  TORCH_CHECK_VALUE(k_in >= 1 && k_in <= 32768, "topk_exclude: unsupported list length k_in=", k_in,
                    " (1 <= k_in <= 32768)");
  const c10::DeviceGuard g(scores_.device());
  const Tensor scores = scores_.contiguous(), ids = ids_.contiguous(), excl = excl_.contiguous(),
               excl_off = excl_off_.contiguous();
  Tensor ceiling;
  if (ceiling_.has_value()) {
    need(*ceiling_, "ceiling", at::kFloat, 1);
    TORCH_CHECK_VALUE(ceiling_->device() == scores.device() && ceiling_->numel() == nq,
                      "ceiling: expected a float [", nq, "] tensor on ", scores.device());
    ceiling = ceiling_->contiguous();
  }
  Tensor os = at::empty({nq, k_out}, scores.options());
  Tensor oi = at::empty({nq, k_out}, ids.options());
  Tensor cnt = at::empty({nq}, scores.options().dtype(at::kInt));
  if (nq == 0) return {os, oi, cnt};
  check_rc(drt_topk_exclude(scores.data_ptr<float>(), ids.data_ptr<int64_t>(), nq, (int32_t)k_in,
                            excl.numel() ? excl.data_ptr<int64_t>() : nullptr, excl_off.data_ptr<int64_t>(),
                            ceiling.defined() ? ceiling.data_ptr<float>() : nullptr, (int32_t)skip, (int32_t)k_out,
                            os.data_ptr<float>(), oi.data_ptr<int64_t>(), cnt.data_ptr<int32_t>(), stream_of(scores)),
           "drt_topk_exclude");
  return {os, oi, cnt};
}

Tensor pair_scores(const Tensor& q_, const Tensor& p_, const Tensor& qidx_, const Tensor& rows_) {
  need(q_, "q", at::kBFloat16, 2);
  need(p_, "p", at::kBFloat16, 2);
  need(qidx_, "qidx", at::kInt, 1);
  need(rows_, "rows", at::kLong, 1);
  TORCH_CHECK_VALUE(q_.size(1) == p_.size(1), "q and p differ in dimension: ", q_.sizes(), " vs ", p_.sizes());
  TORCH_CHECK_VALUE(p_.device() == q_.device() && qidx_.device() == q_.device() && rows_.device() == q_.device(),
                    "pair_scores: every tensor must be on the queries' device ", q_.device());
  TORCH_CHECK_VALUE(qidx_.numel() == rows_.numel(), "pair_scores: ", qidx_.numel(), " query indices for ",
                    rows_.numel(), " rows");
  const int64_t d = q_.size(1);
  TORCH_CHECK_VALUE(d >= 8 && d % 8 == 0 && d <= 1024, "pair_scores: unsupported d=", d, " (d % 8 == 0, d <= 1024)");
  const c10::DeviceGuard g(q_.device());
  const Tensor q = q_.contiguous(), p = p_.contiguous(), qidx = qidx_.contiguous(), rows = rows_.contiguous();
  const int64_t npairs = rows.numel();
  Tensor out = at::empty({npairs}, q.options().dtype(at::kFloat));
  if (npairs == 0) return out;
  check_rc(drt_pair_scores_bf16(q.size(0) ? q.data_ptr() : nullptr, q.size(0), p.size(0) ? p.data_ptr() : nullptr,
                                p.size(0), (int32_t)d, qidx.data_ptr<int32_t>(), rows.data_ptr<int64_t>(), npairs,
                                out.data_ptr<float>(), stream_of(q)),
           "drt_pair_scores_bf16");
  return out;
}

std::tuple<Tensor, Tensor, Tensor, Tensor> topk_collapse(const Tensor& scores_, const Tensor& ids_,
                                                         const Tensor& groups_, int64_t k_out) {
  need(scores_, "scores", at::kFloat, 2);
  need(ids_, "ids", at::kLong, 2);
  need(groups_, "groups", at::kInt, 1);
  TORCH_CHECK_VALUE(scores_.sizes() == ids_.sizes(), "topk_collapse: scores ", scores_.sizes(), " and ids ",
                    ids_.sizes(), " differ in shape");
  TORCH_CHECK_VALUE(ids_.device() == scores_.device() && groups_.device() == scores_.device(),
                    "topk_collapse: every tensor must be on the scores' device ", scores_.device());
  const int64_t nq = scores_.size(0), k_in = scores_.size(1);
  TORCH_CHECK_VALUE(k_out >= 1 && k_out <= 0x7FFFFFFF, "topk_collapse: unsupported k_out=", k_out, " (k_out >= 1)");
  TORCH_CHECK_VALUE(k_in >= 1 && k_in <= 32768, "topk_collapse: unsupported list length k_in=", k_in,
                    " (1 <= k_in <= 32768)");
  const c10::DeviceGuard g(scores_.device());
  const Tensor scores = scores_.contiguous(), ids = ids_.contiguous(), groups = groups_.contiguous();
  Tensor os = at::empty({nq, k_out}, scores.options());
  Tensor og = at::empty({nq, k_out}, groups.options());
  Tensor oi = at::empty({nq, k_out}, ids.options());
  Tensor cnt = at::empty({nq}, scores.options().dtype(at::kInt));
  if (nq == 0) return {os, og, oi, cnt};
  const size_t wsb = drt_topk_collapse_workspace(nq, (int32_t)k_in);
  TORCH_CHECK_VALUE(wsb > 0, "unsupported topk_collapse shape nq=", nq, " k_in=", k_in);
  Tensor ws = workspace(scores, wsb);
  check_rc(drt_topk_collapse(scores.data_ptr<float>(), ids.data_ptr<int64_t>(), nq, (int32_t)k_in,
                             groups.numel() ? groups.data_ptr<int32_t>() : nullptr, groups.numel(), (int32_t)k_out,
                             os.data_ptr<float>(), og.data_ptr<int32_t>(), oi.data_ptr<int64_t>(),
                             cnt.data_ptr<int32_t>(), ws.data_ptr(), wsb, stream_of(scores)),
           "drt_topk_collapse");
  return {os, og, oi, cnt};
}

std::tuple<Tensor, Tensor, Tensor> score_ce_fwd(const Tensor& q_, const Tensor& p_, int64_t target_stride,
// ... 69 lines not shown
}

std::tuple<Tensor, Tensor> score_kd_bwd(const Tensor& grad_, const Tensor& q_, const Tensor& p_,
                                        const Tensor& teacher_, const Tensor& S_, const Tensor& lse_,
                                        const Tensor& aux_, int64_t group, double temperature, double w_ce,
                                        double w_kd, double scale) {
  need_kd(q_, p_, teacher_, group);
  need(S_, "scores", at::kFloat, 2);
  need(lse_, "lse", at::kFloat, 1);
  need(aux_, "aux", at::kFloat, 2);
  const int64_t m = q_.size(0), n = p_.size(0), d = q_.size(1);
  TORCH_CHECK_VALUE(S_.size(0) == m && S_.size(1) == n && lse_.size(0) == m && aux_.size(0) == m && aux_.size(1) == 2,
                    "scores ", S_.sizes(), ", lse ", lse_.sizes(), ", aux ", aux_.sizes(), ": expected [", m, ", ", n,
                    "], [", m, "], [", m, ", 2]");
  const c10::DeviceGuard g(q_.device());
  const Tensor q = q_.contiguous(), p = p_.contiguous(), teacher = teacher_.contiguous(), S = S_.contiguous(),
               lse = lse_.contiguous(), aux = aux_.contiguous();
  const Tensor grad = grad_.to(at::kFloat).contiguous().reshape({1});
  Tensor dq = at::empty({m, d}, q.options());
  Tensor dp = at::empty({n, d}, q.options());
  const size_t wsb = drt_score_kd_workspace(m, n, (int32_t)d);
  Tensor ws = workspace(q, wsb);
  check_rc(drt_score_kd_bwd(q.data_ptr<float>(), p.data_ptr<float>(), teacher.data_ptr<float>(), S.data_ptr<float>(),
                            lse.data_ptr<float>(), aux.data_ptr<float>(), m, n, (int32_t)d, group, (float)temperature,
                            (float)w_ce, (float)w_kd, grad.data_ptr<float>(), (float)scale, dq.data_ptr<float>(),
                            dp.data_ptr<float>(), ws.data_ptr(), wsb, stream_of(q)),
           "drt_score_kd_bwd");
  return {dq, dp};
}

Tensor embed_ln(const Tensor& ids_, const c10::optional<Tensor>& type_ids, const Tensor& word, const Tensor& pos,
                const Tensor& type, const Tensor& gamma, const Tensor& beta, double eps) {
  need(ids_, "input_ids", at::kLong, 2);
  const c10::DeviceGuard g(ids_.device());
  const Tensor ids = ids_.contiguous();
  const int64_t B = ids.size(0), L = ids.size(1), H = word.size(1);
  TORCH_CHECK(L <= pos.size(0), "sequence length ", L, " exceeds max_position_embeddings ", pos.size(0));
  c10::optional<Tensor> tt;
  if (type_ids.has_value()) tt = type_ids->contiguous();
  Tensor out = at::empty({B, L, H}, ids.options().dtype(at::kBFloat16));
  check_rc(drt_embed_ln(ids.data_ptr<int64_t>(), tt.has_value() ? tt->data_ptr<int64_t>() : nullptr, B, L,
                        word.data_ptr<float>(), pos.data_ptr<float>(), type.data_ptr<float>(), gamma.data_ptr<float>(),
                        beta.data_ptr<float>(), (float)eps, (int32_t)H, out.data_ptr(), stream_of(ids)),
           "drt_embed_ln");
  return out;
}

Tensor linear(const Tensor& x_, const Tensor& w_, const c10::optional<Tensor>& bias,
              const c10::optional<Tensor>& residual, bool gelu, bool fp32_out) {
  need(x_, "x", at::kBFloat16, 2);
  need(w_, "w", at::kBFloat16, 2);
  TORCH_CHECK(x_.size(1) == w_.size(1), "linear: x ", x_.sizes(), " and w ", w_.sizes(), " differ in K");
  const c10::DeviceGuard g(x_.device());
  const Tensor x = x_.contiguous(), w = w_.contiguous();
  const int64_t M = x.size(0), K = x.size(1), N = w.size(0);
  if (bias.has_value()) TORCH_CHECK(bias->scalar_type() == at::kFloat && bias->numel() == N, "bias: float [N]");
  c10::optional<Tensor> res;
  if (residual.has_value()) {
    TORCH_CHECK(residual->scalar_type() == at::kBFloat16 && residual->numel() == M * N, "residual: bf16 [M, N]");
    res = residual->contiguous();
  }
  Tensor y = at::empty({M, N}, x.options().dtype(fp32_out ? at::kFloat : at::kBFloat16));
  const int32_t flags = (gelu ? 1 : 0) | (fp32_out ? 2 : 0);
  const size_t wsb = drt_linear_workspace(M, N, K);
  Tensor ws = workspace(x, wsb);
  check_rc(drt_linear_bf16_ws(x.data_ptr(), w.data_ptr(), bias.has_value() ? bias->data_ptr<float>() : nullptr,
                              res.has_value() ? res->data_ptr() : nullptr, y.data_ptr(), M, N, K, flags,
                              wsb ? ws.data_ptr() : nullptr, wsb, stream_of(x)),
           "drt_linear_bf16_ws");
  return y;
}

Tensor attention(const Tensor& qkv_, const c10::optional<Tensor>& mask, int64_t B, int64_t heads, double scale) {
  need(qkv_, "qkv", at::kBFloat16, 2);
  const c10::DeviceGuard g(qkv_.device());
  const Tensor qkv = qkv_.contiguous();
  const int64_t T = qkv.size(0), H3 = qkv.size(1);
  TORCH_CHECK(B > 0 && T % B == 0 && H3 % (3 * heads) == 0, "attention: qkv must be [B*L, 3*heads*64]");
  const int64_t L = T / B, hd = H3 / (3 * heads);
  c10::optional<Tensor> m;
  if (mask.has_value()) {
    TORCH_CHECK(mask->numel() == B * L, "attention: mask must be [B, L]");
    m = mask->to(at::kLong).contiguous();
  }
  Tensor ctx = at::empty({T, heads * hd}, qkv.options());
  check_rc(drt_attention_bf16(qkv.data_ptr(), m.has_value() ? m->data_ptr<int64_t>() : nullptr, ctx.data_ptr(), B, L,
                              (int32_t)heads, (int32_t)hd, (float)scale, stream_of(qkv)),
           "drt_attention_bf16");
  return ctx;
}

Tensor layernorm(const Tensor& x_, const Tensor& gamma, const Tensor& beta, double eps) {
  need_gpu(x_, "x");
  const c10::DeviceGuard g(x_.device());
  const Tensor x = x_.contiguous();
  const int64_t H = x.size(-1), M = x.numel() / H;
  Tensor out = at::empty(x.sizes(), x.options().dtype(at::kBFloat16));
  int rc;
  if (x.scalar_type() == at::kFloat)
    rc = drt_layernorm_f32_bf16(x.data_ptr<float>(), M, (int32_t)H, gamma.data_ptr<float>(), beta.data_ptr<float>(),
                                (float)eps, out.data_ptr(), stream_of(x));
  else {
    TORCH_CHECK(x.scalar_type() == at::kBFloat16, "layernorm: x must be float or bfloat16");
    rc = drt_layernorm_bf16(x.data_ptr(), M, (int32_t)H, gamma.data_ptr<float>(), beta.data_ptr<float>(), (float)eps,
                            out.data_ptr(), stream_of(x));
  }
  check_rc(rc, "drt_layernorm");
  return out;
}

Tensor pool(const Tensor& hidden_, const c10::optional<Tensor>& mask, int64_t mode) {
  need(hidden_, "hidden", at::kBFloat16, 3);
  const c10::DeviceGuard g(hidden_.device());
  const Tensor hidden = hidden_.contiguous();
  const int64_t B = hidden.size(0), L = hidden.size(1), H = hidden.size(2);
  c10::optional<Tensor> m;
  if (mask.has_value()) m = mask->to(at::kLong).contiguous();
  Tensor reps = at::empty({B, H}, hidden.options().dtype(at::kFloat));
  check_rc(drt_pool_bf16(hidden.data_ptr(), m.has_value() ? m->data_ptr<int64_t>() : nullptr, B, L, (int32_t)H,
                         (int32_t)mode, reps.data_ptr<float>(), nullptr, stream_of(hidden)),
           "drt_pool_bf16");
  return reps;
}

Tensor l2_normalize(const Tensor& x_) {
  need(x_, "x", at::kFloat, 2);
  const c10::DeviceGuard g(x_.device());
  Tensor x = x_.clone(at::MemoryFormat::Contiguous);
  check_rc(drt_l2_normalize_f32(x.data_ptr<float>(), x.size(0), (int32_t)x.size(1), nullptr, stream_of(x)),
           "drt_l2_normalize_f32");
  return x;
}

}

TORCH_LIBRARY(drt, m) {
  m.def("ip_topk(Tensor q, Tensor p, int k, int id_offset=0, Tensor? stats=None) -> (Tensor, Tensor, Tensor)");
  m.def("ip_topk.out(Tensor q, Tensor p, int k, int id_offset, Tensor? stats=None, *, Tensor(a!) scores, "
        "Tensor(b!) ids, Tensor(c!) status) -> ()");
  m.def("ip_topk_resolve(Tensor q, Tensor p, int k, int id_offset, Tensor(a!) scores, Tensor(b!) ids, "
        "Tensor(c!) status, Tensor? stats=None) -> int");
  m.def("ip_topk_resolve_wide(Tensor q, Tensor p, int k, int id_offset, Tensor(a!) scores, Tensor(b!) ids, "
        "Tensor(c!) status, Tensor stats) -> int");
  m.def("ip_topk_large(Tensor q, Tensor p, int k, int id_offset, Tensor stats, Tensor tau) -> (Tensor, Tensor, Tensor)");
  m.def("ip_topk_large_keys(Tensor q, Tensor p, int k, int id_offset, Tensor stats, Tensor tau) -> "
        "(Tensor, Tensor, Tensor, Tensor)");
  m.def("merge_exact(Tensor keys, Tensor ids, int k) -> (Tensor, Tensor)");
  m.def("row_stats(Tensor p, Tensor? prev=None) -> Tensor");
  m.def("refine_delta(Tensor q, Tensor p, int row_offset, Tensor cand_scores, Tensor cand_ids, int k, Tensor stats, "
        "Tensor? tau, Tensor(a!) status, bool local=False) -> (Tensor, Tensor)");
  m.def("refine_sort(Tensor cand_scores, Tensor cand_ids, Tensor delta, Tensor cnt, int k) -> (Tensor, Tensor)");
  m.def("topk_merge(Tensor scores, Tensor ids, int k_out) -> (Tensor, Tensor)");
  m.def("dist_sample(Tensor q, Tensor p, int n_global, int k) -> Tensor");
  m.def("dist_tau(Tensor lists, int k) -> Tensor");
  m.def("dist_filter(Tensor q, Tensor p, int n_global, int k, int id_offset, Tensor tau) -> Tensor");
  m.def("dist_filter_lists(Tensor q, Tensor p, int n_global, int k, int id_offset, Tensor lists) -> Tensor");
  m.def("dist_filter_lists_into(Tensor q, Tensor p, int n_global, int k, int id_offset, Tensor lists, int q0, "
        "Tensor(a!) packed) -> ()");
  m.def("dist_filter_into(Tensor q, Tensor p, int n_global, int k, int id_offset, Tensor tau, Tensor(a!) packed) -> ()");
  m.def("dist_filter_chunks_into(Tensor q, Tensor p, int n_global, int k, int id_offset, Tensor tau, int[] starts, "
        "Tensor(a!) packed) -> ()");
  m.def("filter_passes_into(Tensor q, Tensor p, int n_global, int k, int id_offset, Tensor tau, int npasses, int r, "
        "Tensor(a!) packed, Tensor(b!)? tau1=None, Tensor(c!)? pass0=None) -> ()");
  m.def("merge_packed(Tensor parts, int k, int n_global, int k_cert=-1) -> (Tensor, Tensor, Tensor)");
  m.def("topk_exclude(Tensor scores, Tensor ids, Tensor excl, Tensor excl_off, Tensor? ceiling, int skip, int k_out) -> "
        "(Tensor, Tensor, Tensor)");
  m.def("pair_scores(Tensor q, Tensor p, Tensor qidx, Tensor rows) -> Tensor");
  m.def("topk_collapse(Tensor scores, Tensor ids, Tensor groups, int k_out) -> (Tensor, Tensor, Tensor, Tensor)");
  m.def("score_ce_fwd(Tensor q, Tensor p, int target_stride, float scale) -> (Tensor, Tensor, Tensor)");
  m.def("score_ce_bwd(Tensor grad, Tensor q, Tensor p, Tensor scores, Tensor lse, int target_stride, "
        "float scale) -> (Tensor, Tensor)");
  m.def("score_kd_fwd(Tensor q, Tensor p, Tensor teacher, int group, float temperature, float w_ce, float w_kd, "
        "float scale) -> (Tensor, Tensor, Tensor, Tensor)");
  m.def("score_kd_bwd(Tensor grad, Tensor q, Tensor p, Tensor teacher, Tensor scores, Tensor lse, Tensor aux, "
        "int group, float temperature, float w_ce, float w_kd, float scale) -> (Tensor, Tensor)");
  m.def("embed_ln(Tensor input_ids, Tensor? token_type_ids, Tensor word, Tensor pos, Tensor type, Tensor gamma, "
        "Tensor beta, float eps) -> Tensor");
  m.def("linear(Tensor x, Tensor w, Tensor? bias, Tensor? residual, bool gelu=False, bool fp32_out=False) -> Tensor");
  m.def("attention(Tensor qkv, Tensor? mask, int batch, int heads, float scale) -> Tensor");
  m.def("layernorm(Tensor x, Tensor gamma, Tensor beta, float eps) -> Tensor");
  m.def("pool(Tensor hidden, Tensor? mask, int mode) -> Tensor");
  m.def("l2_normalize(Tensor x) -> Tensor");
}

TORCH_LIBRARY_IMPL(drt, CUDA, m) {
  m.impl("ip_topk", &ip_topk);
  m.impl("ip_topk.out", &ip_topk_out);
  m.impl("dist_filter_chunks_into", &dist_filter_chunks_into);
  m.impl("filter_passes_into", &filter_passes_into);
  m.impl("ip_topk_resolve", &ip_topk_resolve);
  m.impl("ip_topk_resolve_wide", &ip_topk_resolve_wide);
  m.impl("ip_topk_large", &ip_topk_large);
  m.impl("ip_topk_large_keys", &ip_topk_large_keys);
  m.impl("merge_exact", &merge_exact);
  m.impl("row_stats", &row_stats);
  m.impl("refine_delta", &refine_delta);
  m.impl("refine_sort", &refine_sort);
  m.impl("topk_merge", &topk_merge);
  m.impl("dist_sample", &dist_sample);
  m.impl("dist_tau", &dist_tau);
  m.impl("dist_filter", &dist_filter);
  m.impl("dist_filter_lists", &dist_filter_lists);
  m.impl("dist_filter_lists_into", &dist_filter_lists_into);
  m.impl("dist_filter_into", &dist_filter_into);
  m.impl("merge_packed", &merge_packed);
  m.impl("topk_exclude", &topk_exclude);
  m.impl("pair_scores", &pair_scores);
  m.impl("topk_collapse", &topk_collapse);
  m.impl("score_ce_fwd", &score_ce_fwd);
  m.impl("score_ce_bwd", &score_ce_bwd);
  m.impl("score_kd_fwd", &score_kd_fwd);
  m.impl("score_kd_bwd", &score_kd_bwd);
  m.impl("embed_ln", &embed_ln);
  m.impl("linear", &linear);
  m.impl("attention", &attention);
  m.impl("layernorm", &layernorm);
  m.impl("pool", &pool);
  m.impl("l2_normalize", &l2_normalize);
}
```

denseretrievaltoolkits_amd/kernels.py:

```python
from __future__ import annotations

from typing import Optional, Tuple

import torch

from . import _native, ops


def _require_device(*ts: torch.Tensor) -> None:
    for t in ts:
        if not t.is_cuda:
            raise ValueError("DRT kernels run on the GPU only (got a CPU tensor; no CPU fallback exists)")


def ip_topk_workspace_bytes(nq: int, n: int, d: int, k: int) -> int:
    return int(_native.load().drt_ip_topk_workspace(nq, n, d, k))


def ip_topk(q: torch.Tensor, p: torch.Tensor, k: int, id_offset: int = 0, resolve: bool = True,
            out: Optional[Tuple[torch.Tensor, torch.Tensor]] = None,
            status: Optional[torch.Tensor] = None,
            stats: Optional[torch.Tensor] = None) -> Tuple[torch.Tensor, torch.Tensor, torch.Tensor]:
    drt = ops.load()
    _require_device(q, p)
# ... 62 lines not shown
        st.index_copy_(0, bad, st2)
        if keys is not None:
            keys.index_copy_(0, bad, k2)
        still = torch.nonzero(st2 != 0).flatten()
        if still.numel():
            qs = qb.index_select(0, still).contiguous()
            s3, i3, k3 = exact_by_ranges(qs, p, k, id_offset, stats, want_keys=True)
            rows = bad.index_select(0, still)
            scores.index_copy_(0, rows, s3)
            ids.index_copy_(0, rows, i3)
            st.index_fill_(0, rows, 0)
            if keys is not None:
                keys.index_copy_(0, rows, k3)
    if out is not None:
        out[0].copy_(scores)
        out[1].copy_(ids)
        scores, ids = out
    if status is not None:
        status.copy_(st)
        st = status
    if want_keys:
        return scores, ids, st, keys
    return scores, ids, st


def ip_topk_exact_keys(q: torch.Tensor, p: torch.Tensor, k: int, id_offset: int = 0,
                       stats: Optional[torch.Tensor] = None) -> Tuple[torch.Tensor, torch.Tensor]:
    drt = ops.load()
    _require_device(q, p)
    if k > MAX_K_LARGE or k < 1:
        raise ValueError(f"unsupported k={k} (1 <= k <= {MAX_K_LARGE})")
    if q.shape[0] == 0:
        z = torch.empty((0, k), dtype=torch.int64, device=q.device)
        return z, z.clone()
    _, ids, _, keys = _ip_topk_large(q, p, k, id_offset, None, None, stats, want_keys=True)
    return keys, ids


def merge_exact(keys: torch.Tensor, ids: torch.Tensor, k: int) -> Tuple[torch.Tensor, torch.Tensor]:
    _require_device(keys, ids)
    if keys.dim() != 3 or keys.shape != ids.shape:
        raise ValueError("merge_exact expects [nparts, nq, k] keys and ids")
    return ops.load().merge_exact(keys, ids, k)


def exact_by_ranges(q: torch.Tensor, p: torch.Tensor, k: int, id_offset: int = 0,
                    stats: Optional[torch.Tensor] = None, want_keys: bool = False):
    drt = ops.load()
    _require_device(q, p)
    nq, n = q.shape[0], p.shape[0]
    if k > MAX_K_LARGE or k < 1:
        raise ValueError(f"unsupported k={k} (1 <= k <= {MAX_K_LARGE})")
    ranges = [(a, min(n, a + _WIDE_CAP)) for a in range(0, n, _WIDE_CAP)] or [(0, 0)]
    if len(ranges) > 1024:
        raise ValueError(f"exact_by_ranges: {n} rows exceed 1024 ranges of {_WIDE_CAP}")
    if stats is None:
        stats = row_stats(p)
    tau = torch.full((nq,), float("-inf"), dtype=torch.float32, device=q.device)
    keys = torch.full((len(ranges), nq, k), -1, dtype=torch.int64, device=q.device)
    ids = torch.full((len(ranges), nq, k), -1, dtype=torch.int64, device=q.device)
    for r, (a, b) in enumerate(ranges):
        kk = min(k, b - a)
        if kk <= 0:
            continue
        _, i_, st_, k_ = drt.ip_topk_large_keys(q, p[a:b], kk, id_offset + a, stats, tau)
        if bool((st_ != 0).any()):
            raise RuntimeError("exact_by_ranges: a range of at most _WIDE_CAP rows overflowed")
        keys[r, :, :kk] = k_
        ids[r, :, :kk] = i_
    so, io = merge_exact(keys, ids, k)
    if not want_keys:
        return so, io
    cid = ids.permute(1, 0, 2).reshape(nq, -1)
    ckey = keys.permute(1, 0, 2).reshape(nq, -1)
    sid, order = torch.sort(cid, dim=1)
    pos = torch.searchsorted(sid, io.contiguous()).clamp_(max=sid.shape[1] - 1)
    ko = torch.gather(ckey, 1, torch.gather(order, 1, pos))
    ko = torch.where(io >= 0, ko, torch.full_like(ko, -1))
    return so, io, ko


_KTH_ROWS = 1 << 20


def _kth_bound(q: torch.Tensor, p: torch.Tensor, k: int, stats: torch.Tensor) -> torch.Tensor:
    nq, d = q.shape
    best = None
    for a in range(0, p.shape[0], _KTH_ROWS):
        g = gemm_nt_f32(q, p[a: a + _KTH_ROWS])
        cand = g if best is None else torch.cat([best, g], dim=1)
        best = torch.topk(cand, min(k, cand.shape[1]), dim=1, sorted=False).values
        del g, cand
    gk = best.min(dim=1).values if best.shape[1] >= k else torch.full((nq,), float("-inf"), device=q.device)
    qn = q.float().pow(2).sum(1).sqrt()
    eps = 1.1 * d * 2.0 ** -24 * qn * stats[0].clamp_min(0).sqrt()
    return (gk - eps).contiguous()


def resolve_failed(q, p, k, id_offset, scores, ids, status, n_failed: Optional[int] = None,
                   stats: Optional[torch.Tensor] = None) -> int:
    if n_failed == 0 or q.shape[0] == 0:
        return 0
    return int(ops.load().ip_topk_resolve(q, p, k, id_offset, scores, ids, status, stats))


def resolve_wide(q, p, k, id_offset, scores, ids, status, stats: torch.Tensor, n_wide: Optional[int] = None) -> int:
    if n_wide == 0 or q.shape[0] == 0:
        return 0
    _require_device(q, p, stats)
    return int(ops.load().ip_topk_resolve_wide(q, p, k, id_offset, scores, ids, status, stats))


def row_stats(p: torch.Tensor, prev: Optional[torch.Tensor] = None) -> torch.Tensor:
    _require_device(p)
    return ops.load().row_stats(p, prev)


def refine_width(k: int) -> int:
    w = int(_native.load().drt_refine_width(k))
    if w <= 0:
        raise ValueError(f"unsupported k={k}")
    return w


def refine(q: torch.Tensor, p: torch.Tensor, row_offset: int, cand_s: torch.Tensor, cand_i: torch.Tensor, k: int,
           stats: torch.Tensor, tau: Optional[torch.Tensor], status: torch.Tensor, all_reduce_sum=None):
    _require_device(q, p, cand_s, cand_i, stats, status)
    drt = ops.load()
    delta, cnt = drt.refine_delta(q, p, row_offset, cand_s, cand_i, k, stats, tau, status, all_reduce_sum is None)
    if all_reduce_sum is not None:
        all_reduce_sum(delta)
    return drt.refine_sort(cand_s, cand_i, delta, cnt, k)


def topk_merge(scores: torch.Tensor, ids: torch.Tensor, k_out: int) -> Tuple[torch.Tensor, torch.Tensor]:
    _require_device(scores, ids)
    if scores.dim() != 3 or scores.shape != ids.shape:
        raise ValueError("topk_merge expects [nparts, nq, k] scores and ids")
    return ops.load().topk_merge(scores.float(), ids.long(), k_out)


def sample_rank(k: int) -> int:
    r = int(_native.load().drt_ip_topk_sample_rank(k))
    if r <= 0:
        raise ValueError(f"unsupported k={k}")
    return r


def dist_sample(q: torch.Tensor, p: torch.Tensor, n_global: int, k: int) -> torch.Tensor:
    _require_device(q, p)
    return ops.load().dist_sample(q, p, n_global, k)


def dist_tau(lists: torch.Tensor, k: int) -> torch.Tensor:
    _require_device(lists)
    return ops.load().dist_tau(lists, k)


def dist_filter(q: torch.Tensor, p: torch.Tensor, n_global: int, k: int, id_offset: int,
                tau: torch.Tensor) -> torch.Tensor:
    _require_device(q, p, tau)
    return ops.load().dist_filter(q, p, n_global, k, id_offset, tau)


def dist_filter_lists(q: torch.Tensor, p: torch.Tensor, n_global: int, k: int, id_offset: int,
                      lists: torch.Tensor) -> torch.Tensor:
    _require_device(q, p, lists)
    return ops.load().dist_filter_lists(q, p, n_global, k, id_offset, lists)


def dist_filter_into(q: torch.Tensor, p: torch.Tensor, n_global: int, k: int, id_offset: int, tau: torch.Tensor,
                     packed: torch.Tensor) -> None:
    _require_device(q, p, tau, packed)
    ops.load().dist_filter_into(q, p, n_global, k, id_offset, tau, packed)


def dist_filter_chunks_into(q: torch.Tensor, p: torch.Tensor, n_global: int, k: int, id_offset: int,
                            tau: torch.Tensor, starts, packed: torch.Tensor) -> None:
    _require_device(q, p, tau, packed)
    ops.load().dist_filter_chunks_into(q, p, n_global, k, id_offset, tau, [int(x) for x in starts], packed)


def tighten_rank(n_local: int, npasses: int, k: int) -> int:
    return int(_native.load().drt_ip_topk_tighten_rank(n_local, npasses, k))


def filter_passes_into(q: torch.Tensor, p: torch.Tensor, n_global: int, k: int, id_offset: int, tau: torch.Tensor,
                       npasses: int, packed: torch.Tensor, r: int = -1, tau1: Optional[torch.Tensor] = None,
                       pass0: Optional[torch.Tensor] = None) -> None:
    _require_device(q, p, tau, packed)
    ops.load().filter_passes_into(q, p, n_global, k, id_offset, tau, npasses, r, packed, tau1, pass0)


def dist_filter_lists_into(q: torch.Tensor, p: torch.Tensor, n_global: int, k: int, id_offset: int,
                           lists: torch.Tensor, q0: int, packed: torch.Tensor) -> None:
    _require_device(q, p, lists, packed)
    ops.load().dist_filter_lists_into(q, p, n_global, k, id_offset, lists, q0, packed)


def merge_packed(parts: torch.Tensor, k: int, n_global: int, k_cert: int = -1):
    _require_device(parts)
    if parts.dim() != 3 or not 2 <= parts.shape[2] <= k + 1:
        raise ValueError("merge_packed expects [nparts, nq, lcap + 1] with lcap <= k")
    return ops.load().merge_packed(parts, k, n_global, k_cert)


def exchange_cap(kc: int, nparts: int) -> int:
    if nparts <= 1 or nparts > 8:
        return kc
    cap = -(-5 * kc // (4 * nparts)) + 32
    cap = -(-cap // 64) * 64
    return kc if cap * 10 >= kc * 9 else cap


def filtered_depth(k: int, skip: int, max_excluded: int) -> int:
    if k < 1 or skip < 0 or max_excluded < 0:
        raise ValueError(f"filtered search needs k >= 1, skip >= 0 (k={k}, skip={skip})")
    depth = skip + k + max_excluded
    if depth > MAX_K_LARGE:
        raise ValueError(f"filtered search depth skip + k + max exclusions = {skip} + {k} + {max_excluded} = {depth} "
                         f"exceeds the limit {MAX_K_LARGE} (MAX_K_LARGE)")
    return depth


def topk_exclude(scores: torch.Tensor, ids: torch.Tensor, excl: torch.Tensor, excl_off: torch.Tensor,
                 k_out: int, skip: int = 0,
                 ceiling: Optional[torch.Tensor] = None) -> Tuple[torch.Tensor, torch.Tensor, torch.Tensor]:
    _require_device(scores, ids, excl, excl_off)
    if ceiling is not None:
        _require_device(ceiling)
    if scores.dim() != 2 or scores.shape != ids.shape:
        raise ValueError("topk_exclude expects [nq, k_in] scores and ids")
    return ops.load().topk_exclude(scores, ids, excl, excl_off, ceiling, skip, k_out)


def pair_scores(q: torch.Tensor, p: torch.Tensor, qidx: torch.Tensor, rows: torch.Tensor) -> torch.Tensor:
    _require_device(q, p, qidx, rows)
    if q.dtype != torch.bfloat16 or p.dtype != torch.bfloat16:
        raise ValueError("pair_scores expects bf16 queries and corpus")
    return ops.load().pair_scores(q, p, qidx.to(torch.int32), rows.to(torch.int64))


COLLAPSE_LDS_K = 2048
COLLAPSE_LDS_GROUPS = 1024
COLLAPSE_REGIONS = 128


def grouped_depths(k: int, p_max: int, ntotal: int) -> Tuple[int, Optional[int]]:
    if k < 1 or p_max < 1 or ntotal < 0:
        raise ValueError(f"grouped search needs k >= 1, p_max >= 1, ntotal >= 0 (k={k}, p_max={p_max}, "
                         f"ntotal={ntotal})")
    full = max(1, min(k * p_max, int(ntotal)))
    d1 = max(1, min(full, MAX_K))
    d2 = max(1, min(full, MAX_K_LARGE)) if full > d1 else None
    return d1, d2


def topk_collapse(scores: torch.Tensor, ids: torch.Tensor, groups: torch.Tensor,
                  k_out: int) -> Tuple[torch.Tensor, torch.Tensor, torch.Tensor, torch.Tensor]:
    _require_device(scores, ids, groups)
    if scores.dim() != 2 or scores.shape != ids.shape:
        raise ValueError("topk_collapse expects [nq, k_in] scores and ids")
    return ops.load().topk_collapse(scores, ids, groups, k_out)


def gemm_nt_f32(a: torch.Tensor, b: torch.Tensor, out: Optional[torch.Tensor] = None) -> torch.Tensor:
    lib = _native.load()
    _require_device(a, b)
    if a.dtype != torch.bfloat16 or b.dtype != torch.bfloat16:
        raise ValueError("gemm_nt_f32 expects bf16 operands")
    a = a.contiguous()
    b = b.contiguous()
    m, d = a.shape
    n = b.shape[0]
    if out is None:
        out = torch.empty((m, n), dtype=torch.float32, device=a.device)
    _native.check(lib.drt_gemm_nt_bf16_f32(a.data_ptr(), b.data_ptr(), out.data_ptr(), m, n, d, out.stride(0),
                                           _native.stream_ptr(a.device)), "drt_gemm_nt_bf16_f32")
    return out
```

denseretrievaltoolkits_amd/ops.py:

```python
from __future__ import annotations

import os
import threading

import torch

from . import _native
from ._native import ROW_STATS_LEN
from .build_native import OPS_LIB_PATH

_lock = threading.Lock()
_loaded = False


def load():
    global _loaded
    if _loaded:
        return torch.ops.drt
    with _lock:
        if _loaded:
            return torch.ops.drt
        _native.load()
        if not os.path.exists(OPS_LIB_PATH):
            raise RuntimeError(f"torch custom-op library not found at {OPS_LIB_PATH}; build it with "
                               "`python -m denseretrievaltoolkits_amd.build_native` (no CPU fallback exists)")
        torch.ops.load_library(OPS_LIB_PATH)
        _register_python_parts()
        _loaded = True
    return torch.ops.drt


def _register_python_parts():
    lib = torch.library

    @lib.register_fake("drt::ip_topk")
    def _(q, p, k, id_offset=0, stats=None):
        nq = q.shape[0]
        return (q.new_empty((nq, k), dtype=torch.float32), q.new_empty((nq, k), dtype=torch.int64),
                q.new_empty((nq,), dtype=torch.int32))

    @lib.register_fake("drt::ip_topk.out")
    def _(q, p, k, id_offset, stats=None, *, scores, ids, status):
        return None

    @lib.register_fake("drt::ip_topk_resolve")
    def _(q, p, k, id_offset, scores, ids, status, stats=None):
        return torch.library.get_ctx().new_dynamic_size()

    @lib.register_fake("drt::ip_topk_resolve_wide")
    def _(q, p, k, id_offset, scores, ids, status, stats):
        return torch.library.get_ctx().new_dynamic_size()

    @lib.register_fake("drt::ip_topk_large")
    def _(q, p, k, id_offset, stats, tau):
        nq = q.shape[0]
        return (q.new_empty((nq, k), dtype=torch.float32), q.new_empty((nq, k), dtype=torch.int64),
                q.new_empty((nq,), dtype=torch.int32))

    @lib.register_fake("drt::ip_topk_large_keys")
    def _(q, p, k, id_offset, stats, tau):
        nq = q.shape[0]
        return (q.new_empty((nq, k), dtype=torch.float32), q.new_empty((nq, k), dtype=torch.int64),
                q.new_empty((nq,), dtype=torch.int32), q.new_empty((nq, k), dtype=torch.int64))

    @lib.register_fake("drt::merge_exact")
    def _(keys, ids, k):
        nq = keys.shape[1]
        return keys.new_empty((nq, k), dtype=torch.float32), ids.new_empty((nq, k))

    @lib.register_fake("drt::row_stats")
    def _(p, prev=None):
        return p.new_empty((ROW_STATS_LEN,), dtype=torch.float32)

    @lib.register_fake("drt::refine_delta")
    def _(q, p, row_offset, cand_scores, cand_ids, k, stats, tau, status, local=False):
        return cand_scores.new_empty(cand_scores.shape), cand_scores.new_empty((cand_scores.shape[0], 2),
                                                                                 dtype=torch.int32)

    @lib.register_fake("drt::refine_sort")
    def _(cand_scores, cand_ids, delta, cnt, k):
        nq = cand_scores.shape[0]
        return cand_scores.new_empty((nq, k)), cand_ids.new_empty((nq, k))

    @lib.register_fake("drt::topk_merge")
    def _(scores, ids, k_out):
        nq = scores.shape[1]
        return scores.new_empty((nq, k_out)), ids.new_empty((nq, k_out))

    @lib.register_fake("drt::dist_sample")
    def _(q, p, n_global, k):
        r = int(_native.load().drt_ip_topk_sample_rank(k))
        return q.new_empty((q.shape[0], r), dtype=torch.int32)

    @lib.register_fake("drt::dist_tau")
    def _(lists, k):
        return lists.new_empty((lists.shape[1],), dtype=torch.float32)

    @lib.register_fake("drt::dist_filter")
    def _(q, p, n_global, k, id_offset, tau):
        return q.new_empty((q.shape[0], k + 1), dtype=torch.int64)

    @lib.register_fake("drt::dist_filter_lists")
    def _(q, p, n_global, k, id_offset, lists):
        return q.new_empty((q.shape[0], k + 1), dtype=torch.int64)

    @lib.register_fake("drt::dist_filter_into")
    def _(q, p, n_global, k, id_offset, tau, packed):
        return None

    @lib.register_fake("drt::dist_filter_chunks_into")
    def _(q, p, n_global, k, id_offset, tau, starts, packed):
        return None

    @lib.register_fake("drt::filter_passes_into")
    def _(q, p, n_global, k, id_offset, tau, npasses, r, packed, tau1=None, pass0=None):
        return None

    @lib.register_fake("drt::dist_filter_lists_into")
    def _(q, p, n_global, k, id_offset, lists, q0, packed):
        return None

    @lib.register_fake("drt::merge_packed")
    def _(parts, k, n_global, k_cert=-1):
        nq = parts.shape[1]
        return (parts.new_empty((nq, k), dtype=torch.float32), parts.new_empty((nq, k), dtype=torch.int64),
                parts.new_empty((nq,), dtype=torch.int32))

    @lib.register_fake("drt::topk_exclude")
    def _(scores, ids, excl, excl_off, ceiling, skip, k_out):
        nq = scores.shape[0]
        return (scores.new_empty((nq, k_out), dtype=torch.float32), ids.new_empty((nq, k_out), dtype=torch.int64),
                scores.new_empty((nq,), dtype=torch.int32))

    @lib.register_fake("drt::pair_scores")
    def _(q, p, qidx, rows):
        return q.new_empty((rows.shape[0],), dtype=torch.float32)

    @lib.register_fake("drt::topk_collapse")
    def _(scores, ids, groups, k_out):
        nq = scores.shape[0]
        return (scores.new_empty((nq, k_out), dtype=torch.float32), groups.new_empty((nq, k_out), dtype=torch.int32),
                ids.new_empty((nq, k_out), dtype=torch.int64), scores.new_empty((nq,), dtype=torch.int32))

    @lib.register_fake("drt::score_ce_fwd")
    def _(q, p, target_stride, scale):
        return q.new_empty(()), q.new_empty((q.shape[0], p.shape[0])), q.new_empty((q.shape[0],))

    @lib.register_fake("drt::score_ce_bwd")
    def _(grad, q, p, scores, lse, target_stride, scale):
        return q.new_empty(q.shape), p.new_empty(p.shape)

    @lib.register_fake("drt::score_kd_fwd")
    def _(q, p, teacher, group, temperature, w_ce, w_kd, scale):
        m = q.shape[0]
        return q.new_empty(()), q.new_empty((m, p.shape[0])), q.new_empty((m,)), q.new_empty((m, 2))

    @lib.register_fake("drt::score_kd_bwd")
    def _(grad, q, p, teacher, scores, lse, aux, group, temperature, w_ce, w_kd, scale):
        return q.new_empty(q.shape), p.new_empty(p.shape)

    @lib.register_fake("drt::embed_ln")
    def _(input_ids, token_type_ids, word, pos, type, gamma, beta, eps):
        return input_ids.new_empty(tuple(input_ids.shape) + (word.shape[1],), dtype=torch.bfloat16)

    @lib.register_fake("drt::linear")
    def _(x, w, bias, residual, gelu=False, fp32_out=False):
        return x.new_empty((x.shape[0], w.shape[0]), dtype=torch.float32 if fp32_out else torch.bfloat16)

    @lib.register_fake("drt::attention")
    def _(qkv, mask, batch, heads, scale):
        return qkv.new_empty((qkv.shape[0], qkv.shape[1] // 3))

    @lib.register_fake("drt::layernorm")
    def _(x, gamma, beta, eps):
        return x.new_empty(x.shape, dtype=torch.bfloat16)

    @lib.register_fake("drt::pool")
    def _(hidden, mask, mode):
        return hidden.new_empty((hidden.shape[0], hidden.shape[2]), dtype=torch.float32)

    @lib.register_fake("drt::l2_normalize")
    def _(x):
        return x.new_empty(x.shape)

    def setup_context(ctx, inputs, output):
        q, p, target_stride, scale = inputs
        _, scores, lse = output
        ctx.save_for_backward(q, p, scores, lse)
        ctx.target_stride = int(target_stride)
        ctx.scale = float(scale)
        ctx.mark_non_differentiable(scores, lse)

    def backward(ctx, g_loss, g_scores, g_lse):
        q, p, scores, lse = ctx.saved_tensors
        dq, dp = torch.ops.drt.score_ce_bwd(g_loss, q, p, scores, lse, ctx.target_stride, ctx.scale)
        return dq, dp, None, None

    lib.register_autograd("drt::score_ce_fwd", backward, setup_context=setup_context)

    def kd_setup_context(ctx, inputs, output):
        q, p, teacher, group, temperature, w_ce, w_kd, scale = inputs
        _, scores, lse, aux = output
        ctx.save_for_backward(q, p, teacher, scores, lse, aux)
        ctx.kd_args = (int(group), float(temperature), float(w_ce), float(w_kd), float(scale))
        ctx.mark_non_differentiable(scores, lse, aux)

    def kd_backward(ctx, g_loss, g_scores, g_lse, g_aux):
        q, p, teacher, scores, lse, aux = ctx.saved_tensors
        dq, dp = torch.ops.drt.score_kd_bwd(g_loss, q, p, teacher, scores, lse, aux, *ctx.kd_args)
        return dq, dp, None, None, None, None, None, None

    lib.register_autograd("drt::score_kd_fwd", kd_backward, setup_context=kd_setup_context)
```

denseretrievaltoolkits_amd/search.py:

```python
from __future__ import annotations

from typing import Optional, Tuple

import numpy as np
import torch

from . import _native, comm, kernels, shards


def _as_device_bf16(x, device) -> torch.Tensor:
    if isinstance(x, np.ndarray):
        x = torch.from_numpy(np.ascontiguousarray(x))
    if not isinstance(x, torch.Tensor):
        raise TypeError(f"expected np.ndarray or torch.Tensor, got {type(x)}")
    return x.detach().to(device=device, dtype=torch.bfloat16).contiguous()


def _stage_host(*ts: torch.Tensor):
    dev = ts[0].device
    hs = [torch.empty(t.shape, dtype=t.dtype, pin_memory=True) for t in ts]
    with torch.cuda.device(dev):
        stream = torch.cuda.current_stream(dev)
        for h, t in zip(hs, ts):
            h.copy_(t, non_blocking=True)
        ev = torch.cuda.Event()
        ev.record(stream)
    return hs, ev


def _stage_status(st: torch.Tensor):
    if not st.is_cuda:
        return st, None
    (h,), ev = _stage_host(st)
    return h, ev


def _status_failed(h: torch.Tensor, ev) -> int:
    if ev is not None:
        ev.synchronize()
    return int(((h & 1) != 0).sum().item())


def _order_uncertified(h: torch.Tensor) -> int:
    return int(((h & 2) != 0).sum().item())


EXACT_ORDER = True


class _HostResult:
    __slots__ = ("hs", "ev")

    def __init__(self, s: torch.Tensor, i: torch.Tensor):
        self.hs, self.ev = _stage_host(s, i)

    def get(self, s: torch.Tensor, i: torch.Tensor, redone: bool):
        if redone:
            return s.cpu().numpy(), i.cpu().numpy()
        self.ev.synchronize()
        return self.hs[0].numpy(), self.hs[1].numpy()


def _pipeline(batches, enqueue, finish):
    pend = None
    for j, q in enumerate(batches):
        cur = enqueue(j, q)
        if pend is not None:
            yield finish(pend)
        pend = cur
    if pend is not None:
        yield finish(pend)


GROUP_QUERIES = 2048
GROUP_MIN_ROWS = 500_000
GROUP_CHUNK_ROWS = 1_250_000
TIGHTEN_AFTER_FIRST_PASS = True


def group_chunks(nrows: int, chunk_rows: int = None, nch: int = None):
    chunk_rows = GROUP_CHUNK_ROWS if chunk_rows is None else chunk_rows
    if nch is None:
        if chunk_rows <= 0 or nrows <= chunk_rows:
            return [(0, nrows)]
        nch = -(-nrows // chunk_rows)
    if nch <= 1:
        return [(0, nrows)]
    per = -(-nrows // nch)
    return [(min(nrows, c * per), min(nrows, (c + 1) * per)) for c in range(nch)]


def _groups(batches, cap=None):
    cap = GROUP_QUERIES if cap is None else cap
    grp, n = [], 0
    for q in batches:
        if grp and n + q.shape[0] > cap:
            yield grp
            grp, n = [], 0
        grp.append(q)
        n += q.shape[0]
    if grp:
        yield grp


def _reserve_group_memory(local, k: int, n_global: int, chunks=None):
    key = (k, n_global, GROUP_QUERIES)
    if getattr(local, "_group_reserved", None) == key or local.ntotal == 0:
        return
    kc = kernels.refine_width(k)
    nq = GROUP_QUERIES
    ws = int(_native.load().drt_ip_topk_dist_workspace(nq, local.ntotal, n_global, local.dp, kc))
    nparts = max(1, len(chunks or [0]))
    lists = nq * (kc + 1) * 8 * (nparts + 1)
    outs = nq * kc * (4 + 8 + 4) + nq * k * (4 + 8) * 2
    need = ws + lists + outs + (64 << 20)
    with torch.cuda.device(local.device):
        blk = torch.empty(need, dtype=torch.uint8, device=local.device)
        del blk
    local._group_reserved = key


class _SideChannel:
    __slots__ = ("stream", "group")

    def __init__(self, stream, group):
        self.stream, self.group = stream, group

    def gather(self, t: torch.Tensor) -> torch.Tensor:
        return comm.all_gather_stacked(t, self.group)

    def all_reduce_sum(self, t: torch.Tensor) -> torch.Tensor:
        return comm.all_reduce_sum_(t, self.group)


def _gtau_enqueue_group(local, qs, k: int, n_global: int, offset: int, gather, to_host: bool = False,
                        stats=None, all_reduce_sum=None, id_shift: int = 0, chunks=None, world: int = 1,
                        side: _SideChannel = None):
    sizes = [q.shape[0] for q in qs]
    qg = qs[0] if len(qs) == 1 else torch.cat(qs)
    best = local.dist_sample(qg, n_global, k)
    lists = gather(best).contiguous()
    tau = kernels.dist_tau(lists, k)
    kc = kernels.refine_width(k) if stats is not None else k
    lc = kernels.exchange_cap(kc, world) if world > 1 and getattr(local, "exchange_capped", True) else kc
    if chunks is not None and len(chunks) > 1 and qg.shape[1] <= 768:
        lists = torch.empty((qg.shape[0], lc + 1), dtype=torch.int64, device=qg.device)
        if TIGHTEN_AFTER_FIRST_PASS and world == 1 and offset == 0 and n_global == local.rows.shape[0]:
            kernels.filter_passes_into(qg, local.rows, n_global, lc, offset, tau, len(chunks), lists)
        else:
            starts = [a for a, _ in chunks] + [chunks[-1][1]]
            kernels.dist_filter_chunks_into(qg, local.rows, n_global, lc, offset, tau, starts, lists)
    elif chunks is not None and len(chunks) > 1:
        lists = torch.empty((len(chunks), qg.shape[0], kc + 1), dtype=torch.int64, device=qg.device)
        for c, (a, b) in enumerate(chunks):
            kernels.dist_filter_into(qg, local.rows[a:b], n_global, kc, offset + a, tau, lists[c])
    else:
        lists = torch.empty((qg.shape[0], lc + 1), dtype=torch.int64, device=qg.device)
        kernels.dist_filter_into(qg, local.rows, n_global, lc, offset, tau, lists)

    def exchange(gather, all_reduce_sum):
        allp = gather(lists)
        if lists.dim() == 3:
            allp = allp.reshape(-1, qg.shape[0], kc + 1)
        s, i, st = kernels.merge_packed(allp, kc, n_global, k_cert=k)
        if stats is not None:
            s, i = kernels.refine(qg, local.rows, offset, s, i, k, stats, tau, st, all_reduce_sum)
        if id_shift:
            i = torch.where(i >= 0, i + id_shift, i)
        h, ev = _stage_status(st)
        host = _HostResult(s, i) if to_host else None
        return s, i, st, h, ev, host

    if side is None:
        return (qs, sizes) + exchange(gather, all_reduce_sum)
    compute = torch.cuda.current_stream(qg.device)
    scanned = torch.cuda.Event()
    scanned.record(compute)
    with torch.cuda.stream(side.stream):
        side.stream.wait_event(scanned)
        for t in (lists, qg, tau):
            t.record_stream(side.stream)
        s, i, st, h, ev, host = exchange(side.gather, side.all_reduce_sum)
    for t in (s, i, st):
        t.record_stream(compute)
    return qs, sizes, s, i, st, h, ev, host


def _gtau_finish_group(pend, redo, wide=None):
    qs, sizes, s, i, st, h, ev, host = pend
    if ev is not None:
        ev.synchronize()
    bad = (h & 1) != 0
    wid = (h & 3) == 2
    res, o, nredo, nunc = [], 0, 0, 0
    hs = hi = None
    for q, nb in zip(qs, sizes):
        nw = int(wid[o:o + nb].sum()) if not bool(bad[o:o + nb].any()) else 0
        if nw and wide is not None:
            nunc += nw - wide(q, s[o:o + nb], i[o:o + nb], st[o:o + nb])
            res.append((s[o:o + nb].cpu().numpy(), i[o:o + nb].cpu().numpy()) if host is not None
                       else (s[o:o + nb], i[o:o + nb]))
        elif bool(bad[o:o + nb].any()):
            rs, ri = redo(q)
            res.append((rs.cpu().numpy(), ri.cpu().numpy()) if host is not None else (rs, ri))
            nredo += 1
        elif host is not None:
            nunc += nw
            if hs is None:
                hs, hi = host.get(s, i, False)
            res.append((hs[o:o + nb], hi[o:o + nb]))
        else:
            nunc += nw
            res.append((s[o:o + nb], i[o:o + nb]))
        o += nb
    return res, nredo, nunc


def filtered_depth(k: int, skip: int, excl_off: torch.Tensor, ntotal: int, depth: Optional[int] = None) -> int:
    if excl_off.dim() != 1 or excl_off.numel() < 1:
        raise ValueError("excl_off must be a 1-d tensor of nq + 1 offsets")
    longest = int((excl_off[1:] - excl_off[:-1]).max().item()) if excl_off.numel() > 1 else 0
    need = kernels.filtered_depth(k, skip, max(0, longest))
    if depth is not None:
        if depth > kernels.MAX_K_LARGE:
            raise ValueError(f"filtered search depth {depth} exceeds the limit {kernels.MAX_K_LARGE} (MAX_K_LARGE)")
        need = max(need, int(depth))
    return max(1, min(need, int(ntotal)))


def _filtered_iter(index, batches, k: int, excl: torch.Tensor, excl_off: torch.Tensor, skip: int, ceiling,
                   to_host: bool, depth):
    batches = list(batches)
    nq = sum(int(q.shape[0]) for q in batches)
    if excl_off.numel() != nq + 1:
        raise ValueError(f"excl_off holds {excl_off.numel()} offsets for {nq} queries (expected nq + 1)")
    if ceiling is not None and ceiling.numel() != nq:
        raise ValueError(f"ceiling holds {ceiling.numel()} values for {nq} queries")
    if not batches:
        return
    K = filtered_depth(k, skip, excl_off, index.ntotal, depth)
    o = 0
    for s, i in index.search_batches_iter(batches, K):
        b = s.shape[0]
        fs, fi, cnt = kernels.topk_exclude(s, i, excl, excl_off[o: o + b + 1], k, skip=skip,
                                           ceiling=None if ceiling is None else ceiling[o: o + b])
        o += b
        yield (fs.cpu().numpy(), fi.cpu().numpy(), cnt.cpu().numpy()) if to_host else (fs, fi, cnt)


def prepare_groups(groups, device) -> Tuple[torch.Tensor, int]:
    g = groups if isinstance(groups, torch.Tensor) else torch.as_tensor(np.asarray(groups))
    if g.dim() != 1 or g.dtype not in (torch.int8, torch.int16, torch.int32, torch.int64, torch.uint8):
        raise ValueError(f"groups must be a 1-d integer array (got {tuple(g.shape)} {g.dtype})")
    g = g.to(device)
    if g.numel():
        lo, hi = int(g.min().item()), int(g.max().item())
        if lo < 0 or hi >= 2 ** 31:
            raise ValueError(f"group ids must lie in [0, 2^31) (got {lo} .. {hi})")
    g = g.to(torch.int32).contiguous()
    p_max = int(torch.unique(g, return_counts=True)[1].max().item()) if g.numel() else 1
    return g, p_max


def _grouped_iter(index, prep, batches, k: int, groups: Optional[torch.Tensor], p_max: int, to_host: bool):
    batches = list(batches)
    if groups is None:
        raise ValueError("grouped search needs a row -> group map: call set_groups first")
    if groups.numel() != index.ntotal:
        raise ValueError(f"groups maps {groups.numel()} rows, the index holds {index.ntotal} (set_groups again "
                         "after adding rows)")
    d1, d2 = kernels.grouped_depths(k, p_max, index.ntotal)
    full = max(1, min(k * p_max, int(index.ntotal)))
    batches = [prep(q) for q in batches]
    for q, (s, i) in zip(batches, index.search_batches_iter(batches, d1)):
        gs, gg, gi, cnt = kernels.topk_collapse(s, i, groups, k)
        if d2 is not None:
            short = torch.nonzero((cnt < k) & (i[:, -1] >= 0)).flatten()
            if short.numel():
                s2, i2 = next(iter(index.search_batches_iter([q.index_select(0, short).contiguous()], d2)))
                gs2, gg2, gi2, cnt2 = kernels.topk_collapse(s2, i2, groups, k)
                if d2 < full:
                    still = int(((cnt2 < k) & (i2[:, -1] >= 0)).sum().item())
                    if still:
                        raise ValueError(f"grouped search: {still} queries show fewer than k={k} groups in their top "
                                         f"{d2} rows (MAX_K_LARGE); an exact answer would need depth {full} = "
                                         f"min(k * P_max, ntotal) with P_max={p_max}")
                gs.index_copy_(0, short, gs2)
                gg.index_copy_(0, short, gg2)
                gi.index_copy_(0, short, gi2)
                cnt.index_copy_(0, short, cnt2)
        yield tuple(t.cpu().numpy() for t in (gs, gg, gi, cnt)) if to_host else (gs, gg, gi, cnt)


class _GroupPend:
    __slots__ = ("pend", "k", "id_offset", "res")

    def __init__(self, pend, k, id_offset):
        self.pend, self.k, self.id_offset, self.res = pend, k, id_offset, None


class _GroupMember:
    __slots__ = ("group", "j")

    def __init__(self, group, j):
        self.group, self.j = group, j


class FlatIPIndex:

    def __init__(self, d: int, device=None, capacity: int = 0):
        if d <= 0 or d > 1024:
            raise ValueError(f"dimension {d} unsupported: the HIP scan needs 0 < d <= 1024")
        self.d = int(d)
        self.dp = (self.d + 63) // 64 * 64
        self.device = torch.device(device) if device is not None else torch.device("cuda", torch.cuda.current_device())
        self._buf = torch.zeros((max(0, capacity), self.dp), dtype=torch.bfloat16, device=self.device)
        self.ntotal = 0
# ... 502 lines not shown
```

include/drt.h:

```cpp
#ifndef DRT_H_
#define DRT_H_

#include <stddef.h>
#include <stdint.h>

#ifdef __cplusplus
extern "C" {
#endif

#define DRT_OK 0
#define DRT_EINVAL (-1)
#define DRT_ROW_STATS_LEN 34

const char* drt_version(void);

size_t drt_ip_topk_workspace(int64_t nq, int64_t n, int32_t d, int32_t k);
int drt_ip_topk_bf16(const void* Q, int64_t nq, const void* P, int64_t n, int32_t d,
                     int32_t k, int64_t id_offset, float* out_scores, int64_t* out_ids,
                     int32_t* status, void* workspace, size_t workspace_bytes,
                     void* stream);

size_t drt_ip_topk_resolve_workspace(int64_t n_failed, int64_t n, int32_t d);
int drt_ip_topk_resolve(const void* Q, int64_t nq, const void* P, int64_t n, int32_t d,
                        int32_t k, int64_t id_offset, float* out_scores, int64_t* out_ids,
                        int32_t* status, void* workspace, size_t workspace_bytes,
                        int64_t* n_resolved, void* stream);

int drt_row_stats_bf16(const void* P, int64_t n, int32_t d, float* stats, int32_t accumulate, void* stream);
int32_t drt_refine_width(int32_t k);
int drt_ip_topk_exact_bf16(const void* Q, int64_t nq, const void* P, int64_t n, int32_t d, int32_t k,
                           int64_t id_offset, const float* stats, float* out_scores, int64_t* out_ids,
                           int32_t* status, void* workspace, size_t workspace_bytes, void* stream);
int drt_ip_topk_resolve_exact(const void* Q, int64_t nq, const void* P, int64_t n, int32_t d, int32_t k,
                              int64_t id_offset, const float* stats, float* out_scores, int64_t* out_ids,
                              int32_t* status, void* workspace, size_t workspace_bytes, int64_t* n_resolved,
                              void* stream);
size_t drt_ip_topk_resolve_wide_workspace(int64_t n, int32_t d);
int drt_ip_topk_resolve_wide(const void* Q, int64_t nq, const void* P, int64_t n, int32_t d, int32_t k,
                             int64_t id_offset, const float* stats, float* out_scores, int64_t* out_ids,
                             int32_t* status, void* workspace, size_t workspace_bytes, int64_t* n_resolved,
                             void* stream);
size_t drt_ip_topk_large_workspace(int32_t d, int32_t k);
int drt_ip_topk_large(const void* Q, int64_t nq, const void* P, int64_t n, int32_t d, int32_t k, int64_t id_offset,
                      const float* stats, const float* tau, float* out_scores, int64_t* out_ids, int32_t* status,
                      void* workspace, size_t workspace_bytes, void* stream);
int drt_ip_topk_large_keys(const void* Q, int64_t nq, const void* P, int64_t n, int32_t d, int32_t k,
                           int64_t id_offset, const float* stats, const float* tau, float* out_scores,
                           int64_t* out_ids, uint64_t* out_keys, int32_t* status, void* workspace,
                           size_t workspace_bytes, void* stream);
int drt_merge_exact(const uint64_t* keys, const int64_t* ids, int64_t nq, int32_t nparts, int32_t k,
                    float* out_scores, int64_t* out_ids, void* stream);
int drt_refine_delta_bf16(const void* Q, int64_t nq, int32_t d, const void* P, int64_t n_local,
                          int64_t row_offset, const float* cand_s, const int64_t* cand_i, int32_t kc,
                          int32_t k, const float* stats, const float* tau, float* delta, int32_t* cnt,
                          int32_t* status, void* stream);
int drt_refine_delta_local_bf16(const void* Q, int64_t nq, int32_t d, const void* P, int64_t n_local,
                                int64_t row_offset, const float* cand_s, const int64_t* cand_i, int32_t kc,
                                int32_t k, const float* stats, const float* tau, float* delta, int32_t* cnt,
                                int32_t* status, void* stream);
int drt_refine_sort(const float* cand_s, const int64_t* cand_i, const float* delta, const int32_t* cnt,
                    int64_t nq, int32_t kc, int32_t k, float* out_scores, int64_t* out_ids, void* stream);

int drt_answer_match_i32(const int32_t* tok, int32_t W, const int64_t* rows, const int64_t* slot_of, int64_t n_rows,
                         int64_t B, int64_t k, const int32_t* ans, const int32_t* alen, int32_t A, int32_t n_max,
                         const uint8_t* every, int8_t* hit, void* stream);

int drt_hit_metrics_i8(const int8_t* hit, int64_t B, int64_t k, const int32_t* topk, int32_t T, double* acc,
                       void* stream);

int drt_topk_merge(const float* scores, const int64_t* ids, int64_t nq, int32_t nparts,
                   int32_t k_in, int32_t k_out, float* out_scores, int64_t* out_ids,
                   void* stream);

int drt_topk_exclude(const float* scores, const int64_t* ids, int64_t nq, int32_t k_in, const int64_t* excl,
                     const int64_t* excl_off, const float* ceiling, int32_t skip, int32_t k_out,
                     float* out_scores, int64_t* out_ids, int32_t* out_count, void* stream);
int drt_pair_scores_bf16(const void* Q, int64_t nq, const void* P, int64_t n, int32_t d, const int32_t* qidx,
                         const int64_t* rows, int64_t npairs, float* out, void* stream);

size_t drt_topk_collapse_workspace(int64_t nq, int32_t k_in);
int drt_topk_collapse(const float* scores, const int64_t* ids, int64_t nq, int32_t k_in, const int32_t* groups,
                      int64_t n_rows, int32_t k_out, float* out_scores, int32_t* out_groups, int64_t* out_ids,
                      int32_t* out_count, void* workspace, size_t workspace_bytes, void* stream);

int32_t drt_ip_topk_sample_rank(int32_t k);
size_t drt_ip_topk_dist_workspace(int64_t nq, int64_t n_local, int64_t n_global, int32_t d,
                                  int32_t k);
int drt_ip_topk_dist_sample(const void* Q, int64_t nq, const void* P, int64_t n_local,
                            int64_t n_global, int32_t d, int32_t k, uint32_t* best, void* ws,
                            size_t ws_bytes, void* stream);
int drt_ip_topk_dist_tau(const uint32_t* lists, int64_t nq, int32_t nlists, int32_t k, float* tau,
                         void* stream);
int drt_ip_topk_dist_filter(const void* Q, int64_t nq, const void* P, int64_t n_local,
                            int64_t n_global, int32_t d, int32_t k, int64_t id_offset,
                            const float* tau, uint64_t* packed, void* ws, size_t ws_bytes,
                            void* stream);
int drt_ip_topk_dist_filter_chunks(const void* Q, int64_t nq, const void* P, int64_t n_local,
                                   int64_t n_global, int32_t d, int32_t k, int64_t id_offset,
                                   const float* tau, uint64_t* packed, const int64_t* starts,
                                   int32_t nchunks, void* ws, size_t ws_bytes, void* stream);
int32_t drt_ip_topk_tighten_rank(int64_t n_local, int32_t npasses, int32_t k);
size_t drt_ip_topk_filter_passes_workspace(int64_t nq, int64_t n_local, int64_t n_global, int32_t d,
                                           int32_t k);
int drt_ip_topk_filter_passes(const void* Q, int64_t nq, const void* P, int64_t n_local,
                              int64_t n_global, int32_t d, int32_t k, int64_t id_offset,
                              const float* tau, uint64_t* packed, int32_t npasses, int32_t r,
                              float* tau1_out, uint32_t* pass0_out, void* ws, size_t ws_bytes,
                              void* stream);
int drt_ip_topk_dist_filter_lists(const void* Q, int64_t nq, const void* P, int64_t n_local,
                                  int64_t n_global, int32_t d, int32_t k, int64_t id_offset,
                                  const uint32_t* lists, int32_t nlists, float* tau_out,
                                  uint64_t* packed, void* ws, size_t ws_bytes, void* stream);
int drt_ip_topk_dist_filter_lists_at(const void* Q, int64_t nq, const void* P, int64_t n_local,
                                     int64_t n_global, int32_t d, int32_t k, int64_t id_offset,
                                     const uint32_t* lists, int32_t nlists, int64_t lists_stride,
                                     float* tau_out, uint64_t* packed, void* ws, size_t ws_bytes,
                                     void* stream);
int drt_topk_merge_packed(const uint64_t* parts, int64_t nq, int32_t nparts, int32_t k,
                          int64_t n_global, float* out_scores, int64_t* out_ids, int32_t* status,
                          void* stream);
int drt_topk_merge_packed_capped(const uint64_t* parts, int64_t nq, int32_t nparts, int32_t lcap, int32_t k,
                                 int32_t k_cert, int64_t n_global, float* out_scores, int64_t* out_ids,
                                 int32_t* status, void* stream);
int drt_topk_merge_packed_cert(const uint64_t* parts, int64_t nq, int32_t nparts, int32_t k,
                               int32_t k_cert, int64_t n_global, float* out_scores, int64_t* out_ids,
                               int32_t* status, void* stream);
int drt_gemm_nt_bf16_f32(const void* A, const void* B, float* C, int64_t m, int64_t n,
                         int32_t d, int64_t ldc, void* stream);

int drt_embed_ln(const int64_t* ids, const int64_t* type_ids, int64_t B, int64_t L,
                 const float* word_emb, const float* pos_emb, const float* type_emb,
                 const float* gamma, const float* beta, float eps, int32_t H, void* out,
                 void* stream);
int drt_linear_bf16(const void* X, const void* W, const float* bias, const void* residual,
                    void* Y, int64_t M, int64_t N, int64_t K, int32_t flags, void* stream);
size_t drt_linear_workspace(int64_t M, int64_t N, int64_t K);
int drt_linear_bf16_ws(const void* X, const void* W, const float* bias, const void* residual,
                       void* Y, int64_t M, int64_t N, int64_t K, int32_t flags, void* ws,
                       size_t ws_bytes, void* stream);
int drt_linear_ln_bf16_ws(const void* X, const void* W, const float* bias, const void* residual,
                          const float* gamma, const float* beta, float eps, void* presum, void* out,
                          int64_t M, int64_t N, int64_t K, void* ws, size_t ws_bytes, void* stream);
size_t drt_linear_dgelu_bias_workspace(int64_t M, int64_t N, int64_t K);
int drt_linear_dgelu_bias_bf16(const void* dY, const void* Wt, const void* gelu_pre, void* dX, int64_t M,
                               int64_t N, int64_t K, float* dbias, void* ws, size_t ws_bytes, void* stream);
int drt_linear_bf16_ex(const void* X, const void* W, const float* bias, const void* residual,
                       const void* gelu_pre, void* Y, void* Y_pre, int64_t M, int64_t N, int64_t K,
                       int32_t flags, float drop_p, uint64_t seed, uint64_t site, void* ws,
                       size_t ws_bytes, void* stream);
int drt_layernorm_f32_bf16(const float* X, int64_t M, int32_t H, const float* gamma,
                           const float* beta, float eps, void* out, void* stream);
int drt_layernorm_bf16(const void* X, int64_t M, int32_t H, const float* gamma,
                       const float* beta, float eps, void* out, void* stream);
int drt_attention_bf16(const void* qkv, const int64_t* mask, void* ctx, int64_t B, int64_t L,
                       int32_t heads, int32_t head_dim, float scale, void* stream);
int drt_attention_fwd_lse_bf16(const void* qkv, const int64_t* mask, void* ctx, float* lse, int64_t B,
                               int64_t L, int32_t heads, int32_t head_dim, float scale, void* stream);

size_t drt_layernorm_bwd_workspace(int64_t M, int32_t H);
int drt_layernorm_bwd_bf16(const void* dy, const void* x, const float* gamma, float eps, int64_t M,
                           int32_t H, const void* dres, void* dx, float* dgamma, float* dbeta,
                           void* ws, size_t ws_bytes, void* stream);
int drt_layernorm_bwd_sum_bf16(const void* dy, const void* x, const float* gamma, float eps,
                               int64_t M, int32_t H, const void* dres, void* dx, void* dx_drop,
                               float drop_p, uint64_t seed, uint64_t site, float* dgamma,
                               float* dbeta, float* dsum, void* ws, size_t ws_bytes, void* stream);
size_t drt_colsum_workspace(int64_t M, int64_t N);
int drt_colsum_bf16(const void* x, int64_t M, int64_t N, float* out, void* ws, size_t ws_bytes,
                    void* stream);
int drt_colsum_f32(const float* x, int64_t M, int64_t N, float* out, void* ws, size_t ws_bytes,
                   void* stream);
int drt_gelu_bwd_bf16(const void* dy, const void* pre, int64_t n, void* dx, void* stream);
int drt_transpose_bf16(const void* x, int64_t R, int64_t C, void* y, void* stream);
int drt_transpose_bf16_ld(const void* x, int64_t R, int64_t C, void* y, int64_t ldy, void* stream);
size_t drt_linear_wgrad_workspace(int64_t T, int64_t N, int64_t K);
int drt_linear_wgrad_bf16(const void* dY, const void* X, float* dW, int64_t T, int64_t N, int64_t K, void* ws,
                          size_t ws_bytes, void* stream);
int drt_embed_ln_pre(const int64_t* ids, const int64_t* type_ids, int64_t B, int64_t L,
                     const float* word_emb, const float* pos_emb, const float* type_emb,
                     const float* gamma, const float* beta, float eps, int32_t H, void* out, void* pre,
                     void* stream);
int drt_gelu_bf16(const void* x, int64_t n, void* y, void* stream);
int drt_embedding_bwd(const int64_t* ids, const int64_t* type_ids, int32_t ntypes, const void* d,
                      int64_t B, int64_t L, int32_t H, int64_t padding_idx, float* dword, float* dpos,
                      float* dtype, void* stream);
int drt_attention_bwd_bf16(const void* qkv, const void* ctx, const void* dctx, const float* lse,
                           const int64_t* mask, void* dqkv, int64_t B, int64_t L, int32_t heads,
                           int32_t head_dim, float scale, void* stream);
int drt_dropout_add_bf16(const void* y, const void* resid, int64_t n, float p, uint64_t seed, uint64_t site,
                         void* out, void* stream);
int drt_attention_train_fwd_bits_bf16(const void* qkv, const int64_t* mask, void* ctx, float* lse,
                                      uint32_t* drop_bits, int64_t B, int64_t L, int32_t heads,
                                      int32_t head_dim, float scale, float drop_p, uint64_t seed,
                                      uint64_t site, void* stream);
int drt_attention_train_bwd_bits_bf16(const void* qkv, const void* ctx, const void* dctx, const float* lse,
                                      const int64_t* mask, const uint32_t* drop_bits, void* dqkv, int64_t B,
                                      int64_t L, int32_t heads, int32_t head_dim, float scale, float drop_p,
                                      uint64_t seed, uint64_t site, void* stream);
size_t drt_attention_train_bwd_bias_workspace(int64_t B, int32_t heads, int32_t head_dim);
int drt_attention_train_bwd_bias_bf16(const void* qkv, const void* ctx, const void* dctx, const float* lse,
                                      const int64_t* mask, const uint32_t* drop_bits, void* dqkv, int64_t B,
                                      int64_t L, int32_t heads, int32_t head_dim, float scale, float drop_p,
                                      uint64_t seed, uint64_t site, float* dbias, void* ws, size_t ws_bytes,
                                      void* stream);
int drt_pool_bf16(const void* hidden, const int64_t* mask, int64_t B, int64_t L, int32_t H,
                  int32_t mode, float* out, void* out_bf16, void* stream);
int drt_l2_normalize_f32(float* x, int64_t B, int32_t H, void* out_bf16, void* stream);
int drt_t5_embed_bf16(const int64_t* ids, int64_t B, int64_t L, const float* table, int32_t H,
                      void* out, void* stream);
int drt_rmsnorm_bf16(const void* X, int64_t M, int32_t H, const float* weight, float eps,
                     void* out, void* stream);
int drt_attention_relbias_bf16(const void* qkv, const int64_t* mask, const float* relbias, void* ctx,
                               int64_t B, int64_t L, int32_t heads, int32_t head_dim, float scale,
                               void* stream);
int drt_gated_gelu_new_bf16(const void* X, int64_t M, int64_t F, void* out, void* stream);
int drt_attention_relbias_train_fwd_bits_bf16(const void* qkv, const int64_t* mask, const float* relbias,
                                              void* ctx, float* lse, uint32_t* drop_bits, int64_t B,
                                              int64_t L, int32_t heads, int32_t head_dim, float scale,
                                              float drop_p, uint64_t seed, uint64_t site, void* stream);
size_t drt_attention_relbias_train_bwd_workspace(int64_t B, int64_t L, int32_t heads);
int drt_attention_relbias_train_bwd_bf16(const void* qkv, const void* ctx, const void* dctx,
                                         const float* lse, const int64_t* mask, const float* relbias,
                                         const uint32_t* drop_bits, void* dqkv, int64_t B, int64_t L,
                                         int32_t heads, int32_t head_dim, float scale, float drop_p,
                                         uint64_t seed, uint64_t site, float* dtable, void* ws,
                                         size_t ws_bytes, void* stream);
size_t drt_rmsnorm_bwd_workspace(int64_t M, int32_t H);
int drt_rmsnorm_bwd_bf16(const void* dy, const void* x, const float* gamma, float eps, int64_t M,
                         int32_t H, const void* dres, void* dx, float* dgamma, void* ws,
                         size_t ws_bytes, void* stream);
int drt_gated_gelu_new_bwd_bf16(const void* dy, const void* X, int64_t M, int64_t F, float drop_p,
                                uint64_t seed, uint64_t site, void* dX, void* stream);
int drt_relu_bwd_bf16(const void* dy, const void* f, int64_t n, float drop_p, uint64_t seed,
                      uint64_t site, void* dx, void* stream);
int drt_t5_embedding_bwd(const int64_t* ids, const void* d, int64_t B, int64_t L, int32_t H,
                         int64_t vocab, float* dshared, void* stream);
int drt_t5_head_expand_bf16(const void* q, const void* Wk, void* qt, int64_t B, int32_t heads,
                            int32_t D, void* stream);
int drt_t5_cross_pool_bf16(const void* qt, const void* enc, const int64_t* mask, void* pooled,
                           int64_t B, int64_t L, int32_t heads, int32_t D, void* stream);
int drt_t5_head_reduce_bf16(const void* pooled, const void* Wv, void* ctx, int64_t B, int32_t heads,
                            int32_t D, void* stream);
int drt_gemm_nt_f32(const float* A, const float* B, float* C, int64_t m, int64_t n, int64_t k,
                    int64_t lda, int64_t ldb, int64_t ldc, void* stream);
int drt_gemm_f32(const float* A, const float* B, float* C, int64_t m, int64_t n, int64_t k, int64_t lda,
                 int64_t ldb, int64_t ldc, int32_t a_kc, int32_t b_kc, int32_t splits, float* ws, void* stream);
int drt_ce_fwd(const float* S, int64_t m, int64_t n, int64_t target_stride, float scale,
               float* lse, float* row_loss, float* loss, void* stream);
int drt_ce_bwd(const float* S, const float* lse, int64_t m, int64_t n, int64_t target_stride,
               const float* grad, float scale, float* dS, void* stream);
int drt_transpose_f32(const float* X, int64_t rows, int64_t cols, float* Y, void* stream);
size_t drt_score_ce_workspace(int64_t m, int64_t n, int32_t d);
int drt_score_ce_fwd(const float* q, const float* p, int64_t m, int64_t n, int32_t d, int64_t target_stride,
                     float scale, float* S, float* lse, float* loss, void* ws, size_t ws_bytes, void* stream);
int drt_score_ce_bwd(const float* q, const float* p, const float* S, const float* lse, int64_t m, int64_t n,
                     int32_t d, int64_t target_stride, const float* grad, float scale, float* dq, float* dp,
                     void* ws, size_t ws_bytes, void* stream);
int drt_kd_fwd(const float* S, const float* teacher, int64_t m, int64_t n, int64_t group, float temperature,
               float w_ce, float w_kd, float scale, float* lse, float* aux, float* row_loss, float* loss,
               void* stream);
int drt_kd_bwd(const float* S, const float* teacher, const float* lse, const float* aux, int64_t m, int64_t n,
// ... 21 lines not shown
```

Measured before the change: 91140.

## Fuse single-GPU sample/tau and write final top-k directly from filter select

For the single-process path, the sample kernel now computes tau in its final kth selection, removing the separate gather and dist_tau launch. The filter-passes select writes scores, ids and status directly instead of packed per-partition lists, so the merge_packed kernel is skipped. The register-path selection now uses smaller per-thread register arrays when the candidate count allows, and it uses wave-aggregated atomics for LDS slot allocation. A memset of the sample buffer was also dropped. Together these reduce launches and memory traffic per query batch, but they add more template instantiations and a new status-certification rule for the one-part output.

Result: no change. 91330, median of 6 (+0.2%).

```diff
diff --git a/denseretrievaltoolkits_amd/_native.py b/denseretrievaltoolkits_amd/_native.py
--- a/denseretrievaltoolkits_amd/_native.py
+++ b/denseretrievaltoolkits_amd/_native.py
@@ -33,6 +33,8 @@
     ("drt_ip_topk_sample_rank", c_i32, [c_i32]),
     ("drt_ip_topk_dist_workspace", c_sz, [c_i64, c_i64, c_i64, c_i32, c_i32]),
     ("drt_ip_topk_dist_sample", c_i32, [c_vp, c_i64, c_vp, c_i64, c_i64, c_i32, c_i32, c_vp, c_vp, c_sz, c_vp]),
+    ("drt_ip_topk_dist_sample_tau", c_i32, [c_vp, c_i64, c_vp, c_i64, c_i64, c_i32, c_i32, c_vp, c_vp, c_vp, c_sz,
+                                            c_vp]),
     ("drt_ip_topk_dist_tau", c_i32, [c_vp, c_i64, c_i32, c_i32, c_vp, c_vp]),
     ("drt_ip_topk_dist_filter", c_i32, [c_vp, c_i64, c_vp, c_i64, c_i64, c_i32, c_i32, c_i64, c_vp, c_vp, c_vp,
                                         c_sz, c_vp]),
@@ -42,6 +44,8 @@
     ("drt_ip_topk_filter_passes_workspace", c_sz, [c_i64, c_i64, c_i64, c_i32, c_i32]),
     ("drt_ip_topk_filter_passes", c_i32, [c_vp, c_i64, c_vp, c_i64, c_i64, c_i32, c_i32, c_i64, c_vp, c_vp,
                                           c_i32, c_i32, c_vp, c_vp, c_vp, c_sz, c_vp]),
+    ("drt_ip_topk_filter_passes_onepart", c_i32, [c_vp, c_i64, c_vp, c_i64, c_i64, c_i32, c_i32, c_i32, c_i64, c_vp,
+                                                  c_vp, c_vp, c_vp, c_i32, c_i32, c_vp, c_vp, c_vp, c_sz, c_vp]),
     ("drt_ip_topk_dist_filter_lists", c_i32, [c_vp, c_i64, c_vp, c_i64, c_i64, c_i32, c_i32, c_i64, c_vp, c_i32,
                                               c_vp, c_vp, c_vp, c_sz, c_vp]),
     ("drt_ip_topk_dist_filter_lists_at", c_i32, [c_vp, c_i64, c_vp, c_i64, c_i64, c_i32, c_i32, c_i64, c_vp,
diff --git a/denseretrievaltoolkits_amd/csrc/search.hip b/denseretrievaltoolkits_amd/csrc/search.hip
--- a/denseretrievaltoolkits_amd/csrc/search.hip
+++ b/denseretrievaltoolkits_amd/csrc/search.hip
@@ -1356,6 +1356,12 @@
 
 int drt_ip_topk_dist_sample(const void* Q, int64_t nq, const void* P, int64_t n_local, int64_t n_global, int32_t d,
                             int32_t k, uint32_t* best, void* ws, size_t ws_bytes, void* stream) {
+  return drt_ip_topk_dist_sample_tau(Q, nq, P, n_local, n_global, d, k, best, nullptr, ws, ws_bytes, stream);
+}
+
+int drt_ip_topk_dist_sample_tau(const void* Q, int64_t nq, const void* P, int64_t n_local, int64_t n_global,
+                                int32_t d, int32_t k, uint32_t* best, float* tau, void* ws, size_t ws_bytes,
+                                void* stream) {
   DRT_REQUIRE(valid_dist_dims(nq, n_local, n_global, d, k));
   if (nq == 0) return DRT_OK;
   DRT_REQUIRE(Q && best && ws);
@@ -1365,6 +1371,10 @@
   hipStream_t s = (hipStream_t)stream;
   if (!p.sample || n_local == 0) {
     DRT_CHECK_HIP(hipMemsetAsync(best, 0xFF, (size_t)nq * r * 4, s));
+    if (tau) {
+      launch_kth_final(nq, best, 1, (int)r, (int64_t)nq * r, (int64_t)r, tau, nullptr, nullptr, (int)r, s);
+      return hip_status(hipGetLastError());
+    }
     return DRT_OK;
   }
   DRT_REQUIRE(P != nullptr);
@@ -1377,11 +1387,10 @@
   const int64_t nlists = 4 * (int64_t)scan16_grid(nq, p.m).x;
   if (nlists * kTopRL <= kKthChunk && nlists * kTopRL <= align_up(p.m, 4)) {
     a.cap = nlists * kTopRL;
-    DRT_CHECK_HIP(hipMemsetAsync(a.out, 0xFF, (size_t)nq * a.cap * 4, s));
     int rc = launch_scan(a, d, SCAN_TOPR, s, PROF_SAMPLE);
     if (rc) return rc;
     const ProfPair pp = prof_begin(PROF_SELECT, s);
-    launch_kth_final(nq, (const uint32_t*)a.out, (int)nlists, (int)r, (int64_t)kTopRL, (int64_t)a.cap, nullptr, best,
+    launch_kth_final(nq, (const uint32_t*)a.out, (int)nlists, (int)r, (int64_t)kTopRL, (int64_t)a.cap, tau, best,
                      nullptr, kTopRL, s);
     prof_end(pp, s);
     return hip_status(hipGetLastError());
@@ -1393,7 +1402,7 @@
   launch_kth_partial(p.nchunk, nq, (const uint32_t*)(w + p.off_sample), (int64_t)align_up(p.m, 4), p.m, (int)r,
                      (uint32_t*)(w + p.off_part), s);
   launch_kth_final(nq, (const uint32_t*)(w + p.off_part), (int)p.nchunk, (int)r, (int64_t)r, (int64_t)(p.nchunk * r),
-                   nullptr, best, nullptr, (int)r, s);
+                   tau, best, nullptr, (int)r, s);
   prof_end(pp, s);
   return hip_status(hipGetLastError());
 }
@@ -1408,6 +1417,14 @@
   return hip_status(hipGetLastError());
 }
 
+struct SelectOut {
+  uint64_t* packed;
+  float* scores = nullptr;
+  int64_t* ids = nullptr;
+  int32_t* status = nullptr;
+  int32_t k_cert = 0;
+};
+
 struct FilterRun {
   TopkPlan p;
   hipStream_t s;
@@ -1418,12 +1435,13 @@
 };
 
 static int filter_setup(FilterRun& f, const void* Q, int64_t nq, const void* P, int64_t n_local, int64_t n_global,
-                        int32_t d, int32_t k, int64_t id_offset, const void* thr, uint64_t* packed, void* ws,
+                        int32_t d, int32_t k, int64_t id_offset, const void* thr, const SelectOut& out, void* ws,
                         size_t ws_bytes, void* stream) {
   DRT_REQUIRE(valid_dist_dims(nq, n_local, n_global, d, k));
   DRT_REQUIRE(id_offset >= 0 && id_offset + n_local <= n_global);
   if (nq == 0) return DRT_OK;
-  DRT_REQUIRE(Q && thr && packed && ws);
+  DRT_REQUIRE(Q && thr && ws);
+  DRT_REQUIRE(out.packed || (out.scores && out.ids && out.status && out.k_cert >= 1 && out.k_cert <= k));
   f.p = make_dist_plan(nq, n_local, n_global, k);
   DRT_REQUIRE(ws_bytes >= f.p.total);
   f.s = (hipStream_t)stream;
@@ -1435,7 +1453,16 @@
   f.sel.k = k;
   f.sel.nq = nq;
   f.sel.id_offset = id_offset;
-  f.sel.out_packed = packed;
+  f.sel.out_packed = out.packed;
+  if (!out.packed) {
+    f.sel.out_scores = out.scores;
+    f.sel.out_ids = out.ids;
+    f.sel.ldo = k;
+    f.sel.status = out.status;
+    f.sel.k_cert = out.k_cert;
+    f.sel.one_part = true;
+    f.sel.n_global = n_global;
+  }
   f.sel.global_tau = true;
   f.scan = filter_scan_args(Q, nq, P, d, n_local, nullptr, f.cnt, f.w + f.p.off_keys, f.p.cap);
   return DRT_OK;
@@ -1459,7 +1486,7 @@
                             int32_t k, int64_t id_offset, const float* tau, uint64_t* packed, void* ws,
                             size_t ws_bytes, void* stream) {
   FilterRun f;
-  int rc = filter_setup(f, Q, nq, P, n_local, n_global, d, k, id_offset, tau, packed, ws, ws_bytes, stream);
+  int rc = filter_setup(f, Q, nq, P, n_local, n_global, d, k, id_offset, tau, SelectOut{packed}, ws, ws_bytes, stream);
   if (rc || nq == 0) return rc;
   if (n_local > 0) {
     if ((rc = filter_begin(f, true))) return rc;
@@ -1478,7 +1505,7 @@
   DRT_REQUIRE(starts != nullptr && nchunks >= 1 && starts[0] == 0 && starts[nchunks] == n_local);
   for (int c = 0; c < nchunks; ++c) DRT_REQUIRE(starts[c] <= starts[c + 1]);
   FilterRun f;
-  int rc = filter_setup(f, Q, nq, P, n_local, n_global, d, k, id_offset, tau, packed, ws, ws_bytes, stream);
+  int rc = filter_setup(f, Q, nq, P, n_local, n_global, d, k, id_offset, tau, SelectOut{packed}, ws, ws_bytes, stream);
   if (rc || nq == 0) return rc;
   if (n_local > 0) {
     if ((rc = filter_begin(f, true))) return rc;
@@ -1516,13 +1543,13 @@
   return passes_layout(p.total, p.nq_pad).total;
 }
 
-int drt_ip_topk_filter_passes(const void* Q, int64_t nq, const void* P, int64_t n_local, int64_t n_global,
-                              int32_t d, int32_t k, int64_t id_offset, const float* tau, uint64_t* packed,
+static int filter_passes_impl(const void* Q, int64_t nq, const void* P, int64_t n_local, int64_t n_global,
+                              int32_t d, int32_t k, int64_t id_offset, const float* tau, const SelectOut& out,
                               int32_t npasses, int32_t r, float* tau1_out, uint32_t* pass0_out, void* ws,
                               size_t ws_bytes, void* stream) {
   DRT_REQUIRE(d <= 768 && n_local < ((int64_t)1 << 32) && npasses >= 1 && npasses <= 1024);
   FilterRun f;
-  int rc = filter_setup(f, Q, nq, P, n_local, n_global, d, k, id_offset, tau, packed, ws, ws_bytes, stream);
+  int rc = filter_setup(f, Q, nq, P, n_local, n_global, d, k, id_offset, tau, out, ws, ws_bytes, stream);
   if (rc || nq == 0) return rc;
   const PassesLayout pl = passes_layout(f.p.total, f.p.nq_pad);
   DRT_REQUIRE(ws_bytes >= pl.total);
@@ -1557,6 +1584,26 @@
   return filter_select(f);
 }
 
+int drt_ip_topk_filter_passes(const void* Q, int64_t nq, const void* P, int64_t n_local, int64_t n_global,
+                              int32_t d, int32_t k, int64_t id_offset, const float* tau, uint64_t* packed,
+                              int32_t npasses, int32_t r, float* tau1_out, uint32_t* pass0_out, void* ws,
+                              size_t ws_bytes, void* stream) {
+  DRT_REQUIRE(nq <= 0 || packed != nullptr);
+  return filter_passes_impl(Q, nq, P, n_local, n_global, d, k, id_offset, tau, SelectOut{packed}, npasses, r,
+                            tau1_out, pass0_out, ws, ws_bytes, stream);
+}
+
+int drt_ip_topk_filter_passes_onepart(const void* Q, int64_t nq, const void* P, int64_t n_local, int64_t n_global,
+                                      int32_t d, int32_t k, int32_t k_cert, int64_t id_offset, const float* tau,
+                                      float* out_scores, int64_t* out_ids, int32_t* status, int32_t npasses,
+                                      int32_t r, float* tau1_out, uint32_t* pass0_out, void* ws, size_t ws_bytes,
+                                      void* stream) {
+  DRT_REQUIRE(nq <= 0 || (out_scores && out_ids && status));
+  SelectOut out{nullptr, out_scores, out_ids, status, k_cert};
+  return filter_passes_impl(Q, nq, P, n_local, n_global, d, k, id_offset, tau, out, npasses, r, tau1_out, pass0_out,
+                            ws, ws_bytes, stream);
+}
+
 int drt_ip_topk_dist_filter_lists(const void* Q, int64_t nq, const void* P, int64_t n_local, int64_t n_global,
                                   int32_t d, int32_t k, int64_t id_offset, const uint32_t* lists, int32_t nlists,
                                   float* tau_out, uint64_t* packed, void* ws, size_t ws_bytes, void* stream) {
@@ -1573,7 +1620,7 @@
   DRT_REQUIRE(r > 0 && nlists >= 1 && (int64_t)nlists * r <= kKthChunk);
   DRT_REQUIRE(nlists == 1 || lists_stride >= nq * r);
   FilterRun f;
-  int rc = filter_setup(f, Q, nq, P, n_local, n_global, d, k, id_offset, lists, packed, ws, ws_bytes, stream);
+  int rc = filter_setup(f, Q, nq, P, n_local, n_global, d, k, id_offset, lists, SelectOut{packed}, ws, ws_bytes, stream);
   if (rc || nq == 0) return rc;
   float* tau = tau_out ? tau_out : (float*)(f.w + f.p.off_tau);
   launch_kth_final(nq, lists, (int)nlists, (int)r, lists_stride, (int64_t)r, tau, nullptr,
diff --git a/denseretrievaltoolkits_amd/csrc/search_internal.h b/denseretrievaltoolkits_amd/csrc/search_internal.h
--- a/denseretrievaltoolkits_amd/csrc/search_internal.h
+++ b/denseretrievaltoolkits_amd/csrc/search_internal.h
@@ -38,6 +38,8 @@
   bool global_tau;
   int k_cert;
   const uint32_t* pass0;
+  bool one_part;
+  int64_t n_global;
 };
 
 DRT_INTERNAL int launch_select(const SelectArgs& a, int input, int output, hipStream_t s);
diff --git a/denseretrievaltoolkits_amd/csrc/select.hip b/denseretrievaltoolkits_amd/csrc/select.hip
--- a/denseretrievaltoolkits_amd/csrc/select.hip
+++ b/denseretrievaltoolkits_amd/csrc/select.hip
@@ -1,3 +1,5 @@
+#include <type_traits>
+
 #include "profile.h"
 #include "search_internal.h"
 
@@ -7,8 +9,8 @@
 constexpr int kSelWaves = kSelThreads / 64;
 constexpr int kSelBins = 1024;
 constexpr int kSelBuf = 4096;
-constexpr int kSelKPT = 16;
-constexpr int kSelRegCap = kSelKPT * kSelThreads;
+constexpr int kSelKPTMax = 16;
+constexpr int kSelRegCap = kSelKPTMax * kSelThreads;
 
 template <int INPUT>
 __device__ __forceinline__ uint64_t sel_load(const SelectArgs& a, int64_t q, int64_t j) {
@@ -36,6 +38,16 @@
 #pragma unroll
   for (int i = 1; i < kSelWaves; ++i) r = op(r, scratch[i]);
   return r;
+}
+
+__device__ __forceinline__ uint32_t wave_slot(bool take, uint32_t* ctr) {
+  const uint64_t m = __ballot(take);
+  if (m == 0ull) return 0u;
+  const int leader = __builtin_ctzll(m);
+  uint32_t base = 0;
+  if ((int)(threadIdx.x & 63) == leader) base = atomicAdd(ctr, (uint32_t)__builtin_popcountll(m));
+  base = __shfl(base, leader, 64);
+  return base + __builtin_amdgcn_mbcnt_hi((uint32_t)(m >> 32), __builtin_amdgcn_mbcnt_lo((uint32_t)m, 0u));
 }
 
 template <typename T, int NT, int E, int US>
@@ -149,7 +161,8 @@
 
   bool fast_done = false;
   int nsel = 0;
-  if (c > (int64_t)a.k && c <= kSelRegCap) {
+  auto reg_path = [&](auto kpt_c) -> bool {
+    constexpr int kSelKPT = decltype(kpt_c)::value;
     uint64_t kr[kSelKPT];
     float sc[kSelKPT];
 #pragma unroll
@@ -218,7 +231,7 @@
         if (bn[u] >= b) t = fminf(t, sc[u]);
       t = block_reduce(t, fscr, [](float x, float y) { return fminf(x, y); });
       if (tid == 0) a.tau[q] = t;
-      return;
+      return true;
     }
     const uint32_t cnt_sel = suffix[b];
     const uint32_t c_above = (b + 1 < kSelBins) ? suffix[b + 1] : 0u;
@@ -232,8 +245,11 @@
       __syncthreads();
 #pragma unroll
       for (int u = 0; u < kSelKPT; ++u) {
-        if (bn[u] > b) buf[atomicAdd(&sh_nsel, 1u)] = kr[u];
-        else if (bn[u] == b) side[atomicAdd(&sh_nside, 1u)] = kr[u];
+        const bool up = bn[u] > b, eq = bn[u] == b;
+        const uint32_t pu = wave_slot(up, &sh_nsel);
+        if (up) buf[pu] = kr[u];
+        const uint32_t ps = wave_slot(eq, &sh_nside);
+        if (eq) side[ps] = kr[u];
       }
       __syncthreads();
       const int ns = (int)sh_nside;
@@ -251,12 +267,24 @@
       if (tid == 0) sh_nsel = 0;
       __syncthreads();
 #pragma unroll
-      for (int u = 0; u < kSelKPT; ++u)
-        if (bn[u] >= b) buf[atomicAdd(&sh_nsel, 1u)] = kr[u];
+      for (int u = 0; u < kSelKPT; ++u) {
+        const bool in = bn[u] >= b;
+        const uint32_t pu = wave_slot(in, &sh_nsel);
+        if (in) buf[pu] = kr[u];
+      }
       __syncthreads();
       nsel = (int)sh_nsel;
       fast_done = true;
     }
+    return false;
+  };
+  if (c > (int64_t)a.k && c <= kSelRegCap) {
+    bool done;
+    if (c <= 4 * kSelThreads) done = reg_path(std::integral_constant<int, 4>{});
+    else if (c <= 6 * kSelThreads) done = reg_path(std::integral_constant<int, 6>{});
+    else if (c <= 8 * kSelThreads) done = reg_path(std::integral_constant<int, 8>{});
+    else done = reg_path(std::integral_constant<int, kSelKPTMax>{});
+    if (done) return;
   } else if (c > (int64_t)a.k) {
     float lo = __builtin_inff(), hi = -__builtin_inff();
     for (int64_t j = tid; j < c; j += kSelThreads) {
@@ -435,6 +463,11 @@
   block_bitonic(buf, n2);
 
   const int64_t orow = a.qmap ? (int64_t)a.qmap[q] : q;
+  bool bad = INPUT == SEL_KEYS64 && c_raw > a.cap;
+  if (INPUT == SEL_KEYS64 && a.pass0 && tid == 0) {
+    const uint32_t* t = a.pass0 + q * 4;
+    if (t[2] && (int64_t)t[1] + (c_raw - (int64_t)t[0]) < (int64_t)a.k) bad = true;
+  }
   if (a.out_packed) {
     uint64_t* op = a.out_packed + orow * (int64_t)(a.k + 1);
     for (int j = tid; j < a.k; j += kSelThreads) {
@@ -447,11 +480,6 @@
     }
     if (tid == 0) {
       const uint64_t nval = (uint64_t)(kk_total < a.k ? kk_total : a.k);
-      bool bad = INPUT == SEL_KEYS64 && c_raw > a.cap;
-      if (INPUT == SEL_KEYS64 && a.pass0) {
-        const uint32_t* t = a.pass0 + q * 4;
-        if (t[2] && (int64_t)t[1] + (c_raw - (int64_t)t[0]) < (int64_t)a.k) bad = true;
-      }
       op[a.k] = (nval << 32) | (bad ? 1ull : 0ull) | (c_raw > (int64_t)a.k ? 2ull : 0ull);
     }
     return;
@@ -470,7 +498,10 @@
   }
   if (a.status && tid == 0) {
     int st = 0;
-    if (INPUT == SEL_KEYS64) {
+    if (a.one_part) {
+      const int64_t kq = a.k_cert > 0 ? a.k_cert : a.k;
+      st = (bad || (kk_total < kq && a.n_global >= kq)) ? 1 : 0;
+    } else if (INPUT == SEL_KEYS64) {
       if (c_raw > a.cap) st = 1;
       const int64_t kq = a.k_cert > 0 ? a.k_cert : a.k;
       if (!a.global_tau && c_raw < kq && c_raw < a.n_total) st = 1;
diff --git a/denseretrievaltoolkits_amd/csrc/torch_ops.cpp b/denseretrievaltoolkits_amd/csrc/torch_ops.cpp
--- a/denseretrievaltoolkits_amd/csrc/torch_ops.cpp
+++ b/denseretrievaltoolkits_amd/csrc/torch_ops.cpp
@@ -320,6 +320,24 @@
   return best;
 }
 
+std::tuple<Tensor, Tensor> dist_sample_tau(const Tensor& q_, const Tensor& p_, int64_t n_global, int64_t k) {
+  need(q_, "q", at::kBFloat16, 2);
+  need(p_, "p", at::kBFloat16, 2);
+  const c10::DeviceGuard g(q_.device());
+  const Tensor q = q_.contiguous(), p = p_.contiguous();
+  const int32_t r = drt_ip_topk_sample_rank((int32_t)k);
+  TORCH_CHECK_VALUE(r > 0, "unsupported k=", k);
+  Tensor best = at::empty({q.size(0), r}, q.options().dtype(at::kInt));
+  Tensor tau = at::empty({q.size(0)}, q.options().dtype(at::kFloat));
+  size_t wsb = 0;
+  Tensor ws = dist_ws(q, p.size(0), n_global, k, &wsb);
+  check_rc(drt_ip_topk_dist_sample_tau(q.data_ptr(), q.size(0), p.size(0) ? p.data_ptr() : nullptr, p.size(0),
+                                       n_global, (int32_t)q.size(1), (int32_t)k, (uint32_t*)best.data_ptr<int32_t>(),
+                                       tau.data_ptr<float>(), ws.data_ptr(), wsb, stream_of(q)),
+           "drt_ip_topk_dist_sample_tau");
+  return {best, tau};
+}
+
 Tensor dist_tau(const Tensor& lists_, int64_t k) {
   need(lists_, "lists", at::kInt, 3);
   const c10::DeviceGuard g(lists_.device());
@@ -408,6 +426,33 @@
          (uint64_t*)packed.data_ptr<int64_t>(), (int32_t)npasses, (int32_t)r,
          tau1.has_value() ? tau1->data_ptr<float>() : nullptr,
          pass0.has_value() ? (uint32_t*)pass0->data_ptr<int32_t>() : nullptr);
+}
+
+std::tuple<Tensor, Tensor, Tensor> filter_passes_onepart(const Tensor& q_, const Tensor& p_, int64_t n_global,
+                                                         int64_t k, int64_t k_cert, int64_t id_offset,
+                                                         const Tensor& tau_, int64_t npasses, int64_t r) {
+  need(q_, "q", at::kBFloat16, 2);
+  need(p_, "p", at::kBFloat16, 2);
+  need(tau_, "tau", at::kFloat, 1);
+  const c10::DeviceGuard g(q_.device());
+  const Tensor q = q_.contiguous(), p = p_.contiguous(), tau = tau_.contiguous();
+  const int64_t nq = q.size(0);
+  TORCH_CHECK_VALUE(tau.size(0) == nq, "tau must hold one threshold per query");
+  TORCH_CHECK_VALUE(q.size(1) <= 768, "interleaved filter passes take d <= 768");
+  TORCH_CHECK_VALUE(npasses >= 1 && npasses <= 1024, "npasses must be in [1, 1024]");
+  TORCH_CHECK_VALUE(k_cert >= 1 && k_cert <= k, "k_cert must be in [1, k]");
+  size_t wsb = 0;
+  Tensor ws = dist_ws(q, p.size(0), n_global, k, &wsb, true);
+  Tensor s = at::empty({nq, k}, q.options().dtype(at::kFloat));
+  Tensor i = at::empty({nq, k}, q.options().dtype(at::kLong));
+  Tensor st = at::empty({nq}, q.options().dtype(at::kInt));
+  check_rc(drt_ip_topk_filter_passes_onepart(q.data_ptr(), nq, p.size(0) ? p.data_ptr() : nullptr, p.size(0), n_global,
+                                             (int32_t)q.size(1), (int32_t)k, (int32_t)k_cert, id_offset,
+                                             tau.data_ptr<float>(), s.data_ptr<float>(), i.data_ptr<int64_t>(),
+                                             st.data_ptr<int32_t>(), (int32_t)npasses, (int32_t)r, nullptr, nullptr,
+                                             ws.data_ptr(), wsb, stream_of(q)),
+           "drt_ip_topk_filter_passes_onepart");
+  return {s, i, st};
 }
 
 void filter_lists_into(const Tensor& q_, const Tensor& p_, int64_t n_global, int64_t k, int64_t id_offset,
@@ -783,6 +828,9 @@
   m.def("refine_sort(Tensor cand_scores, Tensor cand_ids, Tensor delta, Tensor cnt, int k) -> (Tensor, Tensor)");
   m.def("topk_merge(Tensor scores, Tensor ids, int k_out) -> (Tensor, Tensor)");
   m.def("dist_sample(Tensor q, Tensor p, int n_global, int k) -> Tensor");
+  m.def("dist_sample_tau(Tensor q, Tensor p, int n_global, int k) -> (Tensor, Tensor)");
+  m.def("filter_passes_onepart(Tensor q, Tensor p, int n_global, int k, int k_cert, int id_offset, Tensor tau, "
+        "int npasses, int r) -> (Tensor, Tensor, Tensor)");
   m.def("dist_tau(Tensor lists, int k) -> Tensor");
   m.def("dist_filter(Tensor q, Tensor p, int n_global, int k, int id_offset, Tensor tau) -> Tensor");
   m.def("dist_filter_lists(Tensor q, Tensor p, int n_global, int k, int id_offset, Tensor lists) -> Tensor");
@@ -829,6 +877,8 @@
   m.impl("refine_sort", &refine_sort);
   m.impl("topk_merge", &topk_merge);
   m.impl("dist_sample", &dist_sample);
+  m.impl("dist_sample_tau", &dist_sample_tau);
+  m.impl("filter_passes_onepart", &filter_passes_onepart);
   m.impl("dist_tau", &dist_tau);
   m.impl("dist_filter", &dist_filter);
   m.impl("dist_filter_lists", &dist_filter_lists);
diff --git a/denseretrievaltoolkits_amd/kernels.py b/denseretrievaltoolkits_amd/kernels.py
--- a/denseretrievaltoolkits_amd/kernels.py
+++ b/denseretrievaltoolkits_amd/kernels.py
@@ -238,6 +238,11 @@
     return ops.load().dist_sample(q, p, n_global, k)
 
 
+def dist_sample_tau(q: torch.Tensor, p: torch.Tensor, n_global: int, k: int):
+    _require_device(q, p)
+    return ops.load().dist_sample_tau(q, p, n_global, k)
+
+
 def dist_tau(lists: torch.Tensor, k: int) -> torch.Tensor:
     _require_device(lists)
     return ops.load().dist_tau(lists, k)
@@ -276,6 +281,12 @@
                        pass0: Optional[torch.Tensor] = None) -> None:
     _require_device(q, p, tau, packed)
     ops.load().filter_passes_into(q, p, n_global, k, id_offset, tau, npasses, r, packed, tau1, pass0)
+
+
+def filter_passes_onepart(q: torch.Tensor, p: torch.Tensor, n_global: int, k: int, id_offset: int,
+                          tau: torch.Tensor, npasses: int, k_cert: int = -1, r: int = -1):
+    _require_device(q, p, tau)
+    return ops.load().filter_passes_onepart(q, p, n_global, k, k_cert if k_cert > 0 else k, id_offset, tau, npasses, r)
 
 
 def dist_filter_lists_into(q: torch.Tensor, p: torch.Tensor, n_global: int, k: int, id_offset: int,
diff --git a/denseretrievaltoolkits_amd/ops.py b/denseretrievaltoolkits_amd/ops.py
--- a/denseretrievaltoolkits_amd/ops.py
+++ b/denseretrievaltoolkits_amd/ops.py
@@ -112,6 +112,17 @@
     def _(q, p, n_global, k, id_offset, tau, starts, packed):
         return None
 
+    @lib.register_fake("drt::dist_sample_tau")
+    def _(q, p, n_global, k):
+        r = int(_native.load().drt_ip_topk_sample_rank(k))
+        return q.new_empty((q.shape[0], r), dtype=torch.int32), q.new_empty((q.shape[0],), dtype=torch.float32)
+
+    @lib.register_fake("drt::filter_passes_onepart")
+    def _(q, p, n_global, k, k_cert, id_offset, tau, npasses, r):
+        nq = q.shape[0]
+        return (q.new_empty((nq, k), dtype=torch.float32), q.new_empty((nq, k), dtype=torch.int64),
+                q.new_empty((nq,), dtype=torch.int32))
+
     @lib.register_fake("drt::filter_passes_into")
     def _(q, p, n_global, k, id_offset, tau, npasses, r, packed, tau1=None, pass0=None):
         return None
diff --git a/denseretrievaltoolkits_amd/search.py b/denseretrievaltoolkits_amd/search.py
--- a/denseretrievaltoolkits_amd/search.py
+++ b/denseretrievaltoolkits_amd/search.py
@@ -138,18 +138,27 @@
                         side: _SideChannel = None):
     sizes = [q.shape[0] for q in qs]
     qg = qs[0] if len(qs) == 1 else torch.cat(qs)
-    best = local.dist_sample(qg, n_global, k)
-    lists = gather(best).contiguous()
-    tau = kernels.dist_tau(lists, k)
+    one = world == 1 and side is None
+    if one:
+        _, tau = kernels.dist_sample_tau(local._queries(qg), local.rows, n_global, k)
+    else:
+        best = local.dist_sample(qg, n_global, k)
+        lists = gather(best).contiguous()
+        tau = kernels.dist_tau(lists, k)
+    merged = None
     kc = kernels.refine_width(k) if stats is not None else k
     lc = kernels.exchange_cap(kc, world) if world > 1 and getattr(local, "exchange_capped", True) else kc
     if chunks is not None and len(chunks) > 1 and qg.shape[1] <= 768:
-        lists = torch.empty((qg.shape[0], lc + 1), dtype=torch.int64, device=qg.device)
-        if TIGHTEN_AFTER_FIRST_PASS and world == 1 and offset == 0 and n_global == local.rows.shape[0]:
-            kernels.filter_passes_into(qg, local.rows, n_global, lc, offset, tau, len(chunks), lists)
+        passes = TIGHTEN_AFTER_FIRST_PASS and world == 1 and offset == 0 and n_global == local.rows.shape[0]
+        if passes and one:
+            merged = kernels.filter_passes_onepart(qg, local.rows, n_global, lc, offset, tau, len(chunks), k_cert=k)
         else:
-            starts = [a for a, _ in chunks] + [chunks[-1][1]]
-            kernels.dist_filter_chunks_into(qg, local.rows, n_global, lc, offset, tau, starts, lists)
+            lists = torch.empty((qg.shape[0], lc + 1), dtype=torch.int64, device=qg.device)
+            if passes:
+                kernels.filter_passes_into(qg, local.rows, n_global, lc, offset, tau, len(chunks), lists)
+            else:
+                starts = [a for a, _ in chunks] + [chunks[-1][1]]
+                kernels.dist_filter_chunks_into(qg, local.rows, n_global, lc, offset, tau, starts, lists)
     elif chunks is not None and len(chunks) > 1:
         lists = torch.empty((len(chunks), qg.shape[0], kc + 1), dtype=torch.int64, device=qg.device)
         for c, (a, b) in enumerate(chunks):
@@ -159,10 +168,13 @@
         kernels.dist_filter_into(qg, local.rows, n_global, lc, offset, tau, lists)
 
     def exchange(gather, all_reduce_sum):
-        allp = gather(lists)
-        if lists.dim() == 3:
-            allp = allp.reshape(-1, qg.shape[0], kc + 1)
-        s, i, st = kernels.merge_packed(allp, kc, n_global, k_cert=k)
+        if merged is not None:
+            s, i, st = merged
+        else:
+            allp = gather(lists)
+            if lists.dim() == 3:
+                allp = allp.reshape(-1, qg.shape[0], kc + 1)
+            s, i, st = kernels.merge_packed(allp, kc, n_global, k_cert=k)
         if stats is not None:
             s, i = kernels.refine(qg, local.rows, offset, s, i, k, stats, tau, st, all_reduce_sum)
         if id_shift:
diff --git a/include/drt.h b/include/drt.h
--- a/include/drt.h
+++ b/include/drt.h
@@ -89,6 +89,9 @@
 int drt_ip_topk_dist_sample(const void* Q, int64_t nq, const void* P, int64_t n_local,
                             int64_t n_global, int32_t d, int32_t k, uint32_t* best, void* ws,
                             size_t ws_bytes, void* stream);
+int drt_ip_topk_dist_sample_tau(const void* Q, int64_t nq, const void* P, int64_t n_local,
+                                int64_t n_global, int32_t d, int32_t k, uint32_t* best, float* tau,
+                                void* ws, size_t ws_bytes, void* stream);
 int drt_ip_topk_dist_tau(const uint32_t* lists, int64_t nq, int32_t nlists, int32_t k, float* tau,
                          void* stream);
 int drt_ip_topk_dist_filter(const void* Q, int64_t nq, const void* P, int64_t n_local,
@@ -107,6 +110,12 @@
                               const float* tau, uint64_t* packed, int32_t npasses, int32_t r,
                               float* tau1_out, uint32_t* pass0_out, void* ws, size_t ws_bytes,
                               void* stream);
+int drt_ip_topk_filter_passes_onepart(const void* Q, int64_t nq, const void* P, int64_t n_local,
+                                      int64_t n_global, int32_t d, int32_t k, int32_t k_cert,
+                                      int64_t id_offset, const float* tau, float* out_scores,
+                                      int64_t* out_ids, int32_t* status, int32_t npasses, int32_t r,
+                                      float* tau1_out, uint32_t* pass0_out, void* ws, size_t ws_bytes,
+                                      void* stream);
 int drt_ip_topk_dist_filter_lists(const void* Q, int64_t nq, const void* P, int64_t n_local,
                                   int64_t n_global, int32_t d, int32_t k, int64_t id_offset,
                                   const uint32_t* lists, int32_t nlists, float* tau_out,
```
